# bdwsq1996/Effi-MVS-plus

Measured on AMD Instinct MI355X. Metric: ref-views/sec (cost-volume hot path: warp + cost volume + 3-D regularisation + cascaded GRU refinement), higher is better.
Workload: dtype f32 (3x3 MFMA convs: products as 3 bf16 partial products hi*hi+hi*lo+lo*hi, f32 accumulate; all else f32); 1 GPU; cfg3: DTU-shaped 1600x1184, N=5 views (S=4 sources), 3-stage cascade ndepths=48,8,8, GRU iters 3,3,3, seeded-random weights, features of the stock FPN resident in HBM; parallelism=single GPU, views_in_flight=3, arithmetic=split

## Files before the change

### effi_mvs_plus_amd/_lib.py

```python
from __future__ import annotations

import ctypes as C
import os
import threading

_HERE = os.path.dirname(os.path.abspath(__file__))
LIB_PATH = os.environ.get("EFFI_MVS_LIB") or os.path.join(_HERE, "libeffimvs_hip.so")
HEADER_PATH = os.path.join(os.path.dirname(_HERE), "include", "effi_mvs_hip.h")

_vp, _i, _l, _f = C.c_void_p, C.c_int, C.c_long, C.c_float

SIGNATURES = {
    "effi_version": [],
    "effi_set_workspace": [_i, _vp, _l],
    "effi_set_option": [C.c_char_p, _l],
    "effi_fusion_dynamic_filter_f32": [_vp, _vp, _vp, _vp, _i, _i, _i, _vp, _i, _i, _f, _i, _f, _f, _i, _vp, _vp, _vp, _vp, _vp, _vp,
                                       _vp, _vp],
    "effi_fusion_dtu_filter_f32": [_vp, _vp, _vp, _vp, _i, _i, _i, _vp, _f, _f, _i, _i, _f, _f, _vp, _vp, _vp, _vp, _vp, _vp, _vp],
    "effi_fusion_vis_filter_f32": [_vp, _vp, _i, _i, _i, _i, _f, _f, _i, _i, _vp, _vp],
    "effi_fusion_points_f32": [_i, _vp, _l, _vp, _vp, _i, _i, _i, _vp, _vp, _vp],
    "effi_fusion_dtu_reproject_f32": [_vp, _vp, _vp, _vp, _i, _i, _i, _i, _f, _f, _vp, _vp, _vp, _vp],
    "effi_compose_rel_proj_f32": [_vp, _i, _vp, _vp],
    "effi_rel_proj_f32": [_vp, _vp, _vp, _vp],
    "effi_planar_to_nhwc_f32": [_vp, _vp, _i, _i, _i, _vp],
    "effi_homo_warp_f32": [_vp, _vp, _vp, _l, _l, _i, _i, _i, _i, _vp, _vp],
    "effi_warpcorr_views_f32": [_vp, _vp, _i, _vp, _vp, _l, _l, _i, _i, _i, _i, _vp, _vp, _vp],
    "effi_warpcorr_views_tbl_f32": [_vp, _i, _vp, _vp, _l, _l, _i, _i, _i, _i, _vp, _vp, _vp],
    "effi_warpcorr_views_x3_f32": [_vp, _vp, _i, _vp, _vp, _l, _l, _i, _i, _i, _i, _vp, _vp, _i, _vp],
    "effi_warpcorr_views_x3_tbl_f32": [_vp, _i, _vp, _vp, _l, _l, _i, _i, _i, _i, _vp, _vp, _i, _vp],
    "effi_warpcorr_dyn_tbl_f32": [_vp, _i, _vp, _vp, _vp, _vp, _i, _i, _i, _i, _i, _vp, _vp, _vp],
    "effi_view_table_set": [_vp, _vp, _i, _vp],
    "effi_pixelwise_net_f32": [_vp, _vp, _i, _i, _i, _vp, _vp],
    "effi_view_aggregate_f32": [_vp, _vp, _i, _i, _i, _vp, _vp],
    "effi_warpcorr_dyn_f32": [_vp, _vp, _i, _vp, _vp, _vp, _vp, _i, _i, _i, _i, _i, _vp, _vp, _vp],
    "effi_conv3d_k3_f32": [_vp, _vp, _i, _vp, _vp, _i, _i, _i, _i, _i, _i, _i, _vp, _vp, _vp],
    "effi_deconv3d_k3s2_bf16x3_f32": [_vp, _i, _vp, _vp, _i, _i, _i, _i, _i, _vp, _vp, _vp],
    "effi_conv3d_k3s2_mfma_f32": [_vp, _i, _vp, _vp, _i, _i, _i, _i, _i, _vp, _vp],
    "effi_conv3d_k3s1_mfma_f32": [_vp, _i, _vp, _vp, _i, _i, _i, _i, _i, _vp, _vp],
    "effi_deconv3d_k3_f32": [_vp, _i, _vp, _vp, _i, _i, _i, _i, _i, _i, _vp, _vp, _vp],
    "effi_softmax_regress_conf_f32": [_vp, _vp, _l, _l, _i, _i, _vp, _vp, _vp, _i, _vp, _vp],
    "effi_vol_lookup1d_f32": [_vp, _l, _l, _i, _vp, _l, _l, _l, _i, _vp, _vp, _l, _i, _i, _vp, _vp],
    "effi_bilinear_sampler1d_f32": [_vp, _i, _i, _i, _vp, _l, _vp, _vp, _vp],
    "effi_getcost_conv1x1_f32": [_vp, _vp, _i, _i, _vp, _vp, _l, _l, _i, _vp, _l, _l, _i, _vp, _vp, _l, _i, _i, _i, _vp, _vp, _i,
                                 _i, _vp, _vp],
    "effi_getcost_f32": [_vp, _vp, _i, _i, _vp, _vp, _l, _l, _i, _vp, _l, _l, _i, _vp, _vp, _l, _i, _i, _i, _vp, _vp],
    "effi_conv2d_f32": [_vp, _vp, _i, _vp, _vp, _i, _i, _i, _i, _i, _i, _vp, _vp, _vp, _i, _vp, _vp, _vp],
    "effi_conv3d_k3s1_roll_bf16x3_f32": [_vp, _vp, _i, _vp, _vp, _i, _i, _i, _i, _i, _vp, _vp],
    "effi_conv3d_k3s1_bf16x3_f32": [_vp, _vp, _i, _vp, _vp, _i, _i, _i, _i, _i, _vp, _vp],
    "effi_vol_lookup1d_pair_f32": [_vp, _vp, _l, _l, _i, _vp, _l, _l, _l, _i, _vp, _vp, _l, _i, _i, _vp, _vp, _vp],
    "effi_conv3d_k3_pair_f32": [_vp, _vp, _vp, _vp, _vp, _vp, _vp, _vp, _i, _i, _i, _i, _i, _i, _i, _vp],
    "effi_conv3d_k3s1_roll_bf16x3_pair_f32": [_vp, _vp, _vp, _vp, _vp, _vp, _vp, _vp, _vp, _i, _i, _i, _i, _i, _i, _vp],
    "effi_csp_gen_roll_bf16x3_pair_f32": [_vp, _i, _i, _i] + [_vp] * 16 + [_vp],
    "effi_debug_poison_lds": [C.c_uint, _vp, _vp],
    "effi_debug_pk_war_probe": [_vp, _i, _i, _i, _vp],
    "effi_deconv3d_k3_pair_f32": [_vp, _vp, _vp, _vp, _vp, _vp, _vp, _vp, _i, _i, _i, _i, _i, _i, _i, _vp],
    "effi_homo_warp_bwd_f32": [_vp, _vp, _l, _l, _i, _i, _i, _i, _vp, _vp, _vp],
    "effi_warpcorr_views_bwd_f32": [_vp, _vp, _i, _vp, _vp, _l, _l, _i, _i, _i, _i, _vp, _vp, _vp, _vp],
    "effi_image_prepare_u8_f32": [_vp, _i, _i, _i, _i, _i, _vp, _vp],
    "effi_resize_linear_f32": [_vp, _i, _i, _i, _i, _i, _vp, _vp],
    "effi_encoder_inputs_f32": [_vp, _vp, _i, _vp, _vp, _l, _l, _i, _vp, _l, _l, _i, _vp, _vp, _l, _i, _i, _i, _vp, _vp, _vp, _vp,
                                _i, _vp, _vp, _vp],
    "effi_encoder_inputs_bf16x3_f32": [_vp, _vp, _i, _vp, _vp, _l, _l, _i, _vp, _l, _l, _i, _vp, _vp, _l, _i, _i, _i, _vp, _vp, _vp, _vp,
                                       _i, _vp, _vp, _vp],
    "effi_conv2d_k3_bf16x3_pair_f32": [_vp, _vp, _i, _vp, _vp, _vp, _vp, _vp, _i, _vp, _vp, _vp, _i, _i, _i, _i, _vp],
    "effi_conv2d_k3_k1_up2x_bf16x3_f32": [_vp, _vp, _i, _vp, _vp, _i, _vp, _vp, _vp, _vp, _i, _i, _i, _vp, _vp, _vp],
    "effi_conv2d_k3_k1_bf16x3_f32": [_vp, _vp, _i, _vp, _vp, _i, _i, _vp, _i, _vp, _vp, _i, _i, _i, _i, _vp, _vp],
    "effi_conv2d_k3_bf16x3_f32": [_vp, _vp, _i, _vp, _vp, _i, _i, _i, _i, _i, _vp, _vp, _vp, _i, _vp, _vp, _vp],
    "effi_conv2d_k5s2_f32": [_vp, _i, _vp, _vp, _i, _i, _i, _i, _vp, _vp],
    "effi_conv2d_k5s2_bf16x3_f32": [_vp, _i, _vp, _vp, _i, _i, _i, _i, _vp, _vp],
    "effi_conv3d_k3s2_bf16x3_f32": [_vp, _i, _vp, _vp, _i, _i, _i, _i, _i, _vp, _vp],
    "effi_conv2d_c1k7_relu_f32": [_vp, _vp, _vp, _i, _i, _i, _vp, _vp],
    "effi_conv2d_c1k7_relu_bf16x3_f32": [_vp, _vp, _vp, _i, _i, _i, _vp, _vp],
    "effi_convex_upsample2x_f32": [_vp, _vp, _vp, _i, _i, _i, _vp, _vp, _vp, _vp],
    "effi_compose_rel_proj_stages_f32": [_vp, _i, _i, _vp, _vp],
    "effi_split_tanh_relu_stages_f32": [_vp, _vp, _vp, _vp, _vp, _vp, _i, _vp],
    "effi_split_tanh_relu_f32": [_vp, _i, _i, _i, _vp, _vp, _vp],
    "effi_depth_to_inv_f32": [_vp, _vp, _i, _i, _vp, _vp],
    "effi_stage1_hypotheses_f32": [_vp, _i, _i, _vp, _vp, _vp],
    "effi_upsample_nearest_f32": [_vp, _i, _i, _i, _i, _vp, _vp],
    "effi_head_update_f32": [_vp, _vp, _vp, _vp, _i, _i, _i, _vp, _vp, _vp],
    "effi_conv2d_k3_twice_bf16x3_f32": [_vp, _i, _vp, _vp, _vp, _vp, _i, _i, _i, _vp, _vp],
    "effi_encoder_tail_bf16x3_f32": [_vp, _vp, _i, _vp, _vp, _vp, _vp, _vp, _vp, _i, _vp, _i, _vp, _vp, _i, _i, _i, _vp, _vp],
    "effi_sr_geometry": [_i, _i, _vp, _vp],
    "effi_sr_clear_border": [_vp, _vp, _vp, _vp, _vp, _vp, _i, _vp],
    "effi_sr_from_planar_f32": [_vp, _i, _i, _i, _vp, _i, _i, _vp],
    "effi_split_tanh_relu_stages_sr_f32": [_vp, _vp, _vp, _vp, _vp, _vp, _vp, _vp, _vp, _vp, _vp, _i, _vp],
    "effi_encoder_inputs_bf16x3_sr": [_vp, _vp, _i, _vp, _vp, _l, _l, _i, _vp, _l, _l, _i, _vp, _vp, _l, _i, _i, _i, _vp, _vp, _vp, _vp,
                                      _i, _vp, _vp, _i, _i, _vp],
    "effi_encoder_pair_gen_bf16x3_sr": [_vp, _vp, _i, _vp, _vp, _l, _l, _i, _vp, _l, _l, _i, _vp, _vp, _l, _i, _i, _i, _vp, _vp, _vp, _vp,
                                        _i, _vp, _vp, _vp, _vp, _vp, _vp, _i, _i, _i, _i, _vp],
    "effi_gru_zr_q_fused_bf16x3_sr": [_vp, _vp, _vp, _vp, _vp, _vp, _vp, _i, _i, _i, _i, _i, _vp, _vp, _vp],
    "effi_conv2d_k3_bf16x3_sr": [_vp, _vp, _i, _vp, _vp, _i, _i, _i, _i, _i, _i, _i, _vp, _vp, _vp, _vp, _vp],
    "effi_conv2d_k3_bf16x3_pair_sr": [_vp, _vp, _i, _vp, _vp, _vp, _vp, _vp, _i, _vp, _vp, _vp, _i, _i, _i, _i, _i, _i, _vp],
    "effi_conv2d_k3_k1_bf16x3_sr": [_vp, _vp, _i, _vp, _vp, _i, _i, _vp, _i, _vp, _vp, _i, _i, _i, _i, _i, _i, _vp, _vp, _vp],
    "effi_conv2d_k3_k1_up2x_bf16x3_sr": [_vp, _vp, _i, _vp, _vp, _i, _vp, _vp, _vp, _vp, _i, _i, _i, _i, _i, _vp, _vp, _vp],
    "effi_conv_wgrad_f32": [_vp, _vp, _i, _i, _i, _i, _i, _i, _i, _i, _i, _i, _i, _i, _i, _i, _vp, _vp],
    "effi_channel_sum_f32": [_vp, _i, _i, _l, _vp, _vp, _i, _vp],
    "effi_conv2d_k5s2_dgrad_f32": [_vp, _vp, _i, _i, _i, _i, _vp, _vp],
    "effi_bn_moment_f32": [_vp, _i, _i, _l, _vp, _i, _vp, _vp, _i, _vp],
    "effi_bn_train_fwd_f32": [_vp, _i, _i, _l, _vp, _vp, _f, _f, _vp, _vp, _vp, _i, _vp, _vp, _vp, _vp, _i, _vp],
    "effi_pack_conv2d_mfma_f32": [_vp, _vp, _i, _i, _i, _i, _vp, _vp, _vp],
    "effi_pack_conv2d_k5s2_dgrad_f32": [_vp, _i, _i, _i, _i, _vp, _vp, _vp],
    "effi_bn_apply_f32": [_vp, _i, _i, _l, _vp, _vp, _vp, _vp, _i, _vp, _vp],
    "effi_bn_bwd_f32": [_vp, _vp, _vp, _i, _i, _l, _vp, _vp, _vp, _i, _vp, _vp, _vp, _vp, _i, _vp],
    "effi_pointwise_f32": [_i, _vp, _vp, _vp, _vp, _f, _f, _l, _l, _i, _vp, _vp, _vp, _vp],
    "effi_vol_lookup1d_bwd_f32": [_vp, _l, _l, _i, _vp, _l, _l, _l, _i, _vp, _vp, _l, _i, _i, _vp, _vp],
    "effi_getcost_bwd_f32": [_vp, _vp, _i, _i, _vp, _vp, _l, _l, _i, _vp, _l, _l, _i, _vp, _vp, _l, _i, _i, _i, _vp, _vp],
    "effi_softargmin_bwd_f32": [_vp, _vp, _l, _l, _i, _i, _vp, _vp, _vp],
    "effi_view_aggregate_bwd_f32": [_vp, _vp, _i, _i, _i, _vp, _vp, _vp, _vp],
    "effi_convex_upsample2x_bwd_f32": [_vp, _vp, _i, _i, _vp, _vp, _vp, _vp, _vp],
    "effi_warpcorr_dyn_bwd_f32": [_vp, _vp, _i, _vp, _vp, _vp, _vp, _i, _i, _i, _i, _i, _vp, _vp, _vp, _vp, _vp, _vp],
}

BF16X3_ENTRIES = ("effi_conv2d_k3_bf16x3_pair_f32", "effi_conv2d_k3_bf16x3_f32", "effi_conv2d_k3_k1_bf16x3_f32",
                  "effi_conv2d_k3_k1_up2x_bf16x3_f32", "effi_conv3d_k3s1_bf16x3_f32", "effi_conv3d_k3s1_roll_bf16x3_f32",
                  "effi_conv3d_k3s1_roll_bf16x3_pair_f32", "effi_csp_gen_roll_bf16x3_pair_f32", "effi_deconv3d_k3s2_bf16x3_f32", "effi_encoder_tail_bf16x3_f32", "effi_conv2d_k3_twice_bf16x3_f32",
                  "effi_conv2d_k5s2_bf16x3_f32", "effi_conv3d_k3s2_bf16x3_f32",
                  "effi_conv2d_k3_bf16x3_sr", "effi_conv2d_k3_bf16x3_pair_sr", "effi_conv2d_k3_k1_bf16x3_sr", "effi_conv2d_k3_k1_up2x_bf16x3_sr",
                  "effi_encoder_pair_gen_bf16x3_sr", "effi_gru_zr_q_fused_bf16x3_sr")
for _n in BF16X3_ENTRIES:
    SIGNATURES[_n + "_bf16"] = SIGNATURES[_n]

NON_STATUS_SYMBOLS = ("effi_error_string", "effi_workspace_bytes", "effi_get_workspace", "effi_get_option", "effi_option_unset")

_lock = threading.Lock()
_lib = None


class EffiLibraryError(RuntimeError):
    pass


def lib():
    global _lib
    if _lib is not None:
        return _lib
    with _lock:
        if _lib is not None:
            return _lib
        if not os.path.exists(LIB_PATH):
            raise EffiLibraryError(
                f"{LIB_PATH} not found: build the gfx950 kernels first "
                "(python -c 'import __graft_entry__ as g; g.build()' or make -C effi_mvs_plus_amd/csrc). "
                "There is no CPU / eager fallback for the cost-volume path.")
        handle = C.CDLL(LIB_PATH)
        for name, argtypes in SIGNATURES.items():
            fn = getattr(handle, name)
            fn.argtypes = argtypes
            fn.restype = _i
        handle.effi_error_string.argtypes = [_i]
        handle.effi_error_string.restype = C.c_char_p
        handle.effi_workspace_bytes.argtypes = []
# ... 24 lines not shown
```

### effi_mvs_plus_amd/csrc/common.hpp

```cpp
#pragma once
#include <hip/hip_runtime.h>
#include "../../include/effi_mvs_hip.h"

#define EFFI_LAUNCH_CHECK()                                   \
    do {                                                      \
        if (hipPeekAtLastError() != hipSuccess) return EFFI_ERR_LAUNCH; \
    } while (0)

const float* effi_zero_page();

enum EffiOption {
    EFFI_OPT_WARP_LDS_KB,
    EFFI_OPT_DYN_FORM,
    EFFI_OPT_DYN_SETUP_EXACT,
    EFFI_OPT_DYN_XCHG,
    EFFI_OPT_PIXNET_MFMA,
    EFFI_OPT_FORCE_MR,
    EFFI_OPT_MR4_MIN, EFFI_OPT_MR4_NT2_MAX, EFFI_OPT_MR2_MIN,
    EFFI_OPT_WIDE_TILES,
    EFFI_OPT_ROLL_MR, EFFI_OPT_ROLL_ZT, EFFI_OPT_ROLL_RP,
    EFFI_OPT_DECONV_MR,
    EFFI_OPT_SR_WAVES,
    EFFI_OPT_ENC_GEN_MR3,
    EFFI_OPT_C3_LEAN,
// ... 64 lines not shown
__device__ __forceinline__ float effi_sigmoid_split(float x) {
#ifdef EFFI_EXACT_EPILOGUES
    return effi_sigmoid(x);
#else
    const float r = effi_rcp_refined(1.0f + effi_exp_fast(fminf(-x, 60.0f)));
    return (x != x) ? x : r;
#endif
}
__device__ __forceinline__ float effi_tanh_split(float x) {
#ifdef EFFI_EXACT_EPILOGUES
    return tanhf(x);
#else
    const float r = 1.0f - 2.0f * effi_rcp_refined(1.0f + effi_exp_fast(fminf(2.0f * x, 60.0f)));
    return (x != x) ? x : r;
#endif
}

__device__ __forceinline__ float effi_inv_to_depth(float inv, float lo, float hi) {
    const float max_depth = 1.0f / lo, min_depth = 1.0f / hi;
    const float min_disp = 1.0f / max_depth, max_disp = 1.0f / min_depth;
    float s = min_disp + (max_disp - min_disp) * inv;
    s = fmaxf(s, 1e-4f);
    return 1.0f / s;
}

__device__ __forceinline__ float effi_depth_to_inv(float depth, float lo, float hi) {
    const float max_depth = 1.0f / lo, min_depth = 1.0f / hi;
    const float min_disp = 1.0f / max_depth, max_disp = 1.0f / min_depth;
    const float den = (max_disp - min_disp) + 1e-10f;
    const float s_ = 1.0f / depth;
    return (s_ - min_disp) / den;
}

__device__ __forceinline__ float effi_lk_rcp(float b) {
#ifdef EFFI_EXACT_LOOKUP
    return 1.0f / b;
#else
    const float r0 = __builtin_amdgcn_rcpf(b);
    return fmaf(fmaf(-b, r0, 1.0f), r0, r0);
#endif
}
__device__ __forceinline__ float effi_lk_div(float a, float b, float rb) {
#ifdef EFFI_EXACT_LOOKUP
    (void)rb;
    return a / b;
#else
    const float q = a * rb;
    return fmaf(fmaf(-q, b, a), rb, q);
#endif
}

__device__ __forceinline__ void lookup1d_index(int Dp, float q_depth, float dmin, float dmax, int& x0, float& w0, float& w1) {
    const float scaled = effi_lk_rcp(q_depth);
    const float min_disp = effi_lk_rcp(dmax), max_disp = effi_lk_rcp(dmin);
    const float den = (max_disp - min_disp) + 1e-10f;
    const float disp = effi_lk_div(scaled - min_disp, den, effi_lk_rcp(den));
    const float dm1 = (float)(Dp - 1);
    const float t = disp * dm1;
    const float g = effi_lk_div(2.0f * t, dm1, effi_lk_rcp(dm1)) - 1.0f;
    float ix = ((g + 1.0f) * 0.5f) * dm1;
    ix = fminf(fmaxf(ix, -2.0f), dm1 + 2.0f);
    const float x0f = floorf(ix);
    x0 = (int)x0f;
    w1 = ix - x0f;
    w0 = (x0f + 1.0f) - ix;
}
// ... 212 lines not shown
```

### effi_mvs_plus_amd/csrc/conv2d_sr.hip

```cpp
#include "conv2d_x3.hpp"

namespace {

int fill_sr(Conv2dArgs& a, const void* const* srcs, const int* src_channels, int n_src, const void* wpack_bf16, const float* bias,
            int cout, int h, int w, int hp, int wp) {
    if (!srcs || !src_channels || n_src < 1 || n_src > EFFI_MAX_SRC || !wpack_bf16 || !bias) return EFFI_ERR_BADARG;
    if (cout < 1 || h < 1 || w < 1) return EFFI_ERR_BADARG;
    const bool wide_possible = w >= 512 || effi_option(EFFI_OPT_WIDE_TILES) == 1;
    if (hp < ((h + 15) & ~15) + 2 || wp < (wide_possible ? ((w + 63) & ~63) : ((w + 15) & ~15)) + 2) return EFFI_ERR_BADARG;
    if ((long)hp * wp * 4 >= (1L << 31)) return EFFI_ERR_UNSUPPORTED;
    a.cin = 0;
    for (int i = 0; i < EFFI_MAX_SRC; ++i) {
        a.src[i] = reinterpret_cast<const float*>((i < n_src) ? srcs[i] : srcs[0]);
        a.ch[i] = (i < n_src) ? src_channels[i] : 0;
        if (i < n_src && (!srcs[i] || src_channels[i] < 1)) return EFFI_ERR_BADARG;
        if (i < n_src && (src_channels[i] & 15)) return EFFI_ERR_UNSUPPORTED;
        if (i < n_src && (reinterpret_cast<uintptr_t>(srcs[i]) & 15)) return EFFI_ERR_BADARG;
        a.cin += a.ch[i];
    }
    if ((long)cout * hp * wp >= (1L << 31)) return EFFI_ERR_UNSUPPORTED;
    a.kgroups = (a.cin + 3) / 4;
    a.zeros = nullptr;
    a.wpack = reinterpret_cast<const float*>(wpack_bf16);
    a.bias = bias;
// ... 118 lines not shown
}

extern "C" int EFFI_FN(effi_conv2d_k3_k1_bf16x3_sr)(const void* const* srcs, const int* src_channels, int n_src, const void* wpack_bf16,
                                                    const float* bias, int cout1, int relu1, const float* extra, int c_extra,
                                                    const void* w2pack_bf16, const float* bias2, int cout2, int relu, int h, int w,
                                                    int hp, int wp, float* out, void* out_sr, effi_stream_t stream) {
    if (!w2pack_bf16 || !bias2 || (!out && !out_sr) || (out && out_sr)) return EFFI_ERR_BADARG;
    if (cout1 < 1 || cout2 < 1 || c_extra < 0 || (c_extra > 0 && !extra)) return EFFI_ERR_BADARG;
    if (cout1 > 96 || c_extra > 16 || cout2 > 96) return EFFI_ERR_UNSUPPORTED;
    if (out_sr && ((cout2 & 15) || (reinterpret_cast<uintptr_t>(out_sr) & 15))) return EFFI_ERR_BADARG;
    Conv2dArgs a;
    const int rc = fill_sr(a, srcs, src_channels, n_src, wpack_bf16, bias, cout1, h, w, hp, wp);
    if (rc != EFFI_OK) return rc;
    a.kgroups = relu1 ? 1 : 0;
    a.act = relu ? EFFI_ACT_RELU : EFFI_ACT_NONE;
    a.hd = c_extra;
    a.aux0 = c_extra ? extra : bias2;
    a.aux1 = reinterpret_cast<const float*>(w2pack_bf16);
    a.disp_range = bias2;
    a.n_range = cout2;
    a.out0 = out;
    a.out_sr = reinterpret_cast<unsigned short*>(out_sr);
    hipStream_t st = effi_s(stream);
    switch ((cout1 + 15) / 16) {
        case 1: return launch_bf16x3<1, EFFI_EPI_K1, false, true>(a, st);
        case 2: return launch_bf16x3<2, EFFI_EPI_K1, false, true>(a, st);
        case 3: return launch_bf16x3<3, EFFI_EPI_K1, false, true>(a, st);
        case 4: return launch_bf16x3<4, EFFI_EPI_K1, false, true>(a, st);
        case 6: return launch_bf16x3<6, EFFI_EPI_K1, false, true>(a, st);
        default: return EFFI_ERR_UNSUPPORTED;
    }
}

extern "C" int EFFI_FN(effi_conv2d_k3_k1_up2x_bf16x3_sr)(const void* const* srcs, const int* src_channels, int n_src,
                                                         const void* wpack_bf16, const float* bias, int cout1, const void* w2pack_bf16,
                                                         const float* bias2, const float* inv_depth, const float* disp_range,
                                                         int n_range, int h, int w, int hp, int wp, float* out_depth,
                                                         float* out_depth_inv, effi_stream_t stream) {
    if (!w2pack_bf16 || !bias2 || !inv_depth || !disp_range || n_range < 2 || !out_depth) return EFFI_ERR_BADARG;
    if (cout1 < 1 || cout1 > 96) return EFFI_ERR_UNSUPPORTED;
    Conv2dArgs a;
    const int rc = fill_sr(a, srcs, src_channels, n_src, wpack_bf16, bias, cout1, h, w, hp, wp);
    if (rc != EFFI_OK) return rc;
    a.kgroups = 1;
    a.hd = 0;
    a.aux0 = inv_depth;
    a.aux1 = reinterpret_cast<const float*>(w2pack_bf16);
    a.disp_range = bias2;
    a.n_range = 36;
    a.out0 = out_depth;
    a.out1 = out_depth_inv;
    a.zin = n_range;
    a.xptr0 = disp_range;
    hipStream_t st = effi_s(stream);
    switch ((cout1 + 15) / 16) {
        case 2: return launch_bf16x3<2, EFFI_EPI_K1UP, false, true>(a, st);
        case 4: return launch_bf16x3<4, EFFI_EPI_K1UP, false, true>(a, st);
        case 6: return launch_bf16x3<6, EFFI_EPI_K1UP, false, true>(a, st);
        default: return EFFI_ERR_UNSUPPORTED;
    }
}

#include "gru_fused.hpp"
```

### effi_mvs_plus_amd/csrc/conv2d_x3.hpp

```cpp
#pragma once
#include "common.hpp"

#ifdef EFFI_BF16_ONLY
#define EFFI_FN(name) name##_bf16
#else
#define EFFI_FN(name) name
#endif

#ifndef EFFI_ABL
#define EFFI_ABL 0
#endif
#ifndef EFFI_PIPE_FRAGS
#define EFFI_PIPE_FRAGS 0
#endif

#ifndef EFFI_EPI_BATCH
#define EFFI_EPI_BATCH 1
#endif
#ifndef EFFI_EPI_EARLY_MAX
#define EFFI_EPI_EARLY_MAX 16
#endif
#ifndef EFFI_B_EARLY
#define EFFI_B_EARLY 0
#endif
// ... 139 lines not shown
        for (int r = 0; r < 4; ++r) dst[(long)r * hw] = effi_sigmoid_split(v[r]) * (is_z ? 1.0f : hv[r]);
    } else if (EPI == EFFI_EPI_GRU_Q) {
        if (nvalid <= 0) return;
        if (SR && a.aux_q4) {
            const long oq = ((long)(co0 >> 2) * hw + pix) * 4;
            const f32x4 h4 = *reinterpret_cast<const f32x4*>(a.aux0 + oq), z4 = *reinterpret_cast<const f32x4*>(a.aux1 + oq);
            f32x4 g;
#pragma unroll
            for (int r = 0; r < 4; ++r) g[r] = (1.0f - z4[r]) * h4[r] + z4[r] * effi_tanh_split(v[r]);
            *reinterpret_cast<f32x4*>(a.out0 + oq) = g;
            effi_sr_store4(a.out_sr, a.sr_hp, a.sr_wp, co0, y, x, g);
            return;
        }
        const long o = (long)co0 * hw + pix;
        float hv[4], zv[4];
#pragma unroll
        for (int r = 0; r < 4; ++r) {
            hv[r] = a.aux0[o + (long)r * hw];
            zv[r] = a.aux1[o + (long)r * hw];
        }
        f32x4 g;
#pragma unroll
        for (int r = 0; r < 4; ++r) g[r] = (1.0f - zv[r]) * hv[r] + zv[r] * effi_tanh_split(v[r]);
#pragma unroll
        for (int r = 0; r < 4; ++r) a.out0[o + (long)r * hw] = g[r];
        if (SR) effi_sr_store4(a.out_sr, a.sr_hp, a.sr_wp, co0, y, x, g);
    }
}

typedef __bf16 bf16x8 __attribute__((ext_vector_type(8)));

#define EFFI_EPI_K1 6
#define EFFI_EPI_K1UP 8
typedef __bf16 bf16x2 __attribute__((ext_vector_type(2)));
typedef float f32x2 __attribute__((ext_vector_type(2)));

__device__ __forceinline__ void split_octet(const f32x4 (&pa)[8], int px, bf16x8& hi, bf16x8& lo) {
#pragma unroll
    for (int e = 0; e < 8; e += 2) {
        const f32x2 x = {pa[e][px], pa[e + 1][px]};
        const bf16x2 h2 = __builtin_convertvector(x, bf16x2);
        const f32x2 hf = __builtin_convertvector(h2, f32x2);
        const bf16x2 l2 = __builtin_convertvector(x - hf, bf16x2);
        hi[e] = h2[0];
        hi[e + 1] = h2[1];
        lo[e] = l2[0];
        lo[e + 1] = l2[1];
    }
}

template <int NT, int MR, int EPI, bool ZB, bool WIDE, bool SR = false, int NW = 4, bool GEN = false>
__device__ __forceinline__ void conv2d_k3_bf16x3_tile(const Conv2dArgs a, int tiles_x, int ntiles, int bid, int nbid, int bidy,
                                                      const EncGenArgs* gp = nullptr, int gmode = 0) {
    constexpr int NTHR = NW * 64;
    static_assert(!GEN || SR, "generated inputs use the split-resident LDS image");
    static_assert(NW == 4 || (SR && NW == 8), "eight waves: split-resident kernels only");
    constexpr int TR = WIDE ? NW : NW * MR, TW = WIDE ? 16 * MR : 16;
    constexpr int AR = TR + 2, AW = SR ? TW + 2 : TW + 8, AQ = AW / 4, XOFF = SR ? 0 : 3, XLEFT = 4, CCH = 16, NKS = 5;
    constexpr int MROW = WIDE ? 0 : AW * 8, MCOL = WIDE ? 16 * 8 : 0;
    constexpr int APIX = AR * AW, NITEMS = (APIX / 4) * 2;
    constexpr int APIXP = SR ? ((APIX + 15) & ~15) : APIX;
    constexpr int NPART = kHiOnly ? 1 : 2;
    constexpr int NUA = SR ? (NPART * 2 * APIXP + NTHR - 1) / NTHR : 1;
    constexpr int NBF = NKS * NT * 2 * 64;
    constexpr int NB4 = (NBF + NTHR - 1) / NTHR;
    static_assert(SR || NITEMS <= 256, "one staging item per thread");
    static_assert(!(SR && ZB), "split-resident maps are 2-D");
    static_assert(EPI != EFFI_EPI_HEAD && EPI != EFFI_EPI_ADD_UP2, "epilogue not instantiated for the split-precision kernel");
    static_assert((EPI != EFFI_EPI_K1 && EPI != EFFI_EPI_K1UP) || !ZB, "the fused 1x1 epilogue is 2-D only");
    __shared__ __attribute__((aligned(16))) unsigned short lds_ah[SR ? NUA * NTHR * 8 : APIX * CCH];
    __shared__ __attribute__((aligned(16))) unsigned short lds_al[SR ? 8 : APIX * CCH];
    __shared__ __attribute__((aligned(16))) unsigned short lds_b[NB4 * NTHR * 8];
    const unsigned short* const lds_al_rd = SR ? lds_ah + 2 * APIXP * 8 : lds_al;
    constexpr int IW7 = (AW + 7 + 1) & ~1, IH7 = AR + 7;
    __shared__ float lds_inv[GEN ? IH7 * IW7 : 1];

    const int tid = threadIdx.x, lane = tid & 63, wv = tid >> 6;
    const int li = lane & 15, lk = lane >> 4;
    const int h = a.h, w = a.w;
    const long hw = (long)h * w;
    const int tile = effi_xcd_remap(bid, nbid);
    if (tile >= ntiles) return;
    const int ty_ = tile / tiles_x;
    const int x0 = (tile - ty_ * tiles_x) * TW, y0 = ty_ * TR;
    const int zpl = ZB ? bidy : 0;

    const bool stager = tid < NITEMS;
    const int pq = stager ? tid % (APIX / 4) : 0, soct = stager ? tid / (APIX / 4) : 0;
    const int srow = pq / AQ, sqx = pq - srow * AQ;
    const int sgy = y0 - 1 + srow, sgx = x0 - XLEFT + 4 * sqx;
    const bool s_in = stager & (sgy >= 0) & (sgy < h) & (sgx >= 0) & (sgx < w);
    const int s_off = sgy * w + sgx;
    const int s_lds = (soct * APIX + srow * AW + 4 * sqx) * 8;
    const int s_nv = w - sgx;
    const bool s_part = s_nv < 4;

    f32x4 pa[SR ? NUA : 8];
    const int cin_eff = ZB ? 3 * a.cin : a.cin;
    const int nchunks = (cin_eff + CCH - 1) / CCH;
    const unsigned short* wbf = reinterpret_cast<const unsigned short*>(a.wpack);
    int goff[NUA];
    if (SR && !GEN) {
#pragma unroll
        for (int j = 0; j < NUA; ++j) {
            const int u = tid + j * NTHR;
            const int part = u / (2 * APIXP), r_ = u - part * (2 * APIXP);
            const int oct = r_ / APIXP, p = r_ - oct * APIXP;
            const int row = p / AW, col = p - row * AW;
            const bool valid = (part < NPART) & (p < APIX);
            goff[j] = valid ? ((oct * 2 + part) * a.sr_hp + (y0 + row)) * a.sr_wp + (x0 + col) : 0;
        }
    }
    auto prefetch = [&](int ch) {
        if constexpr (GEN) {
            (void)ch;
        } else if constexpr (SR) {
            const int cb = ch * CCH;
            const int c1 = cb - a.ch[0], c2 = c1 - a.ch[1];
            const float* src = (c1 < 0) ? a.src[0] : (c2 < 0 ? a.src[1] : a.src[2]);
            const int cl = (c1 < 0) ? cb : (c2 < 0 ? c1 : c2);
            const f32x4* base = reinterpret_cast<const f32x4*>(src) + (long)(cl >> 2) * ((long)a.sr_hp * a.sr_wp);
#pragma unroll
            for (int j = 0; j < NUA; ++j) pa[j] = (EFFI_ABL & 1) ? f32x4{0.0f, 0.0f, 0.0f, 0.0f} : base[goff[j]];
        } else {
        int cb = ch * CCH + soct * 8;
        const int emax = min(cin_eff - cb, 8) - 1;
        bool in = s_in & (emax >= 0);
        long zoff = 0;
        if (ZB) {
            const int dz = (cb >= a.cin) + (cb >= 2 * a.cin);
            cb -= dz * a.cin;
            const int zz = zpl + dz - 1;
            in &= (zz >= 0) & (zz < a.zcount);
            zoff = (long)zz * hw;
        }
        const int c1 = cb - a.ch[0], c2 = c1 - a.ch[1];
        const float* src = (c1 < 0) ? a.src[0] : (c2 < 0 ? a.src[1] : a.src[2]);
        const int cl = (c1 < 0) ? cb : (c2 < 0 ? c1 : c2);
        const float* base = in ? src + ((long)cl * a.cstride + zoff + s_off) : a.zeros;
        const long step = in ? a.cstride : 0;
        const float* q = base;
        if (ZB && in && s_part) {
// ... 167 lines not shown

    constexpr bool kBatchT = SR && EFFI_EPI_BATCH != 0 && !(EFFI_ABL & 24) &&
                             (EPI == EFFI_EPI_PLAIN || EPI == EFFI_EPI_GRU_ZR || EPI == EFFI_EPI_GRU_Q);
    constexpr int NZ = (EPI == EFFI_EPI_GRU_ZR) ? NT / 2 : 0;
    constexpr int NH = !kBatchT ? 0 : (EPI == EFFI_EPI_GRU_ZR ? NT - NZ : (EPI == EFFI_EPI_GRU_Q ? NT : 0));
    constexpr int NZQ = (kBatchT && EPI == EFFI_EPI_GRU_Q) ? NT : 0;
    constexpr bool kStateEarly = MR * (NH + NZQ) * 4 <= EFFI_EPI_EARLY_MAX;
    const bool ebatch = kBatchT && (EPI == EFFI_EPI_PLAIN || a.aux_q4);
    f32x4 eb[kBatchT ? NT : 1], eh[MR][NH > 0 ? NH : 1], ez[MR][NZQ > 0 ? NZQ : 1];
    unsigned eqb[MR];
    bool einside[MR];
    auto epi_issue_bias = [&]() {
        if (!ebatch) return;
#pragma unroll
        for (int n = 0; n < NT; ++n) eb[n] = *reinterpret_cast<const f32x4*>(a.bias + n * 16 + 4 * lk);
#pragma unroll
        for (int m = 0; m < MR; ++m) {
            const int x = x0 + li + (WIDE ? 16 * m : 0), y = y0 + (WIDE ? wv : wv * MR + m);
            einside[m] = (y < h) & (x < w);
            eqb[m] = ((unsigned)lk * (unsigned)hw + (einside[m] ? (unsigned)(y * w + x) : 0u)) * 4u;
        }
    };
    auto epi_issue_state = [&]() {
        if (!ebatch) return;
#pragma unroll
        for (int m = 0; m < MR; ++m) {
#pragma unroll
            for (int j = 0; j < NH; ++j) eh[m][j] = *reinterpret_cast<const f32x4*>(a.aux0 + (size_t)(eqb[m] + (unsigned)j * 16u * (unsigned)hw));
#pragma unroll
            for (int j = 0; j < NZQ; ++j) ez[m][j] = *reinterpret_cast<const f32x4*>(a.aux1 + (size_t)(eqb[m] + (unsigned)j * 16u * (unsigned)hw));
        }
    };

    constexpr bool kK1 = (EPI == EFFI_EPI_K1 || EPI == EFFI_EPI_K1UP) && !(EFFI_ABL & 24) && EFFI_EPI_BATCH != 0;
    f32x4 kb[kK1 ? NT : 1], kex[kK1 ? MR : 1];
    if constexpr (kK1) {
#pragma unroll
        for (int n = 0; n < NT; ++n) kb[n] = *reinterpret_cast<const f32x4*>(a.bias + n * 16 + 4 * lk);
#pragma unroll
        for (int m = 0; m < MR; ++m) kex[m] = f32x4{0.0f, 0.0f, 0.0f, 0.0f};
        if (EPI == EFFI_EPI_K1 && a.hd > 0) {
#pragma unroll
            for (int m = 0; m < MR; ++m) {
                const int x = x0 + li + (WIDE ? 16 * m : 0), y = y0 + (WIDE ? wv : wv * MR + m);
                const unsigned pix = ((y < h) & (x < w)) ? (unsigned)(y * w + x) : 0u;
#pragma unroll
                for (int r = 0; r < 4; ++r) {
                    const int c = 4 * lk + r;
                    const float t_ = a.aux0[(size_t)((unsigned)min(c, a.hd - 1) * (unsigned)hw + pix)];
                    kex[m][r] = (c < a.hd) ? t_ : 0.0f;
                }
            }
        }
    }

    constexpr bool kBiasQ = !kBatchT && !kK1 && !(EFFI_ABL & 24) && EFFI_EPI_BATCH != 0;
    f32x4 gb[kBiasQ ? NT : 1];
    if constexpr (kBiasQ) {
#pragma unroll
        for (int n = 0; n < NT; ++n) gb[n] = *reinterpret_cast<const f32x4*>(a.bias + n * 16 + 4 * lk);
    }

    prefetch(0);
    epi_issue_bias();
    if (kStateEarly) epi_issue_state();
    stash(0);
    __syncthreads();
// ... 58 lines not shown
                    }
                }
                if (PIPE) {
                    __builtin_amdgcn_sched_barrier(0);
                    if (s_ + 1 < NKS) load_b(s_ + 1, n);
                }
            }
        }
        if (ch + 1 < nchunks) {
            __syncthreads();
            stash(ch + 1);
            __syncthreads();
        }
    }

    if (EFFI_ABL & 24) {
#pragma unroll
        for (int m = 0; m < MR; ++m) {
            const int x = x0 + li + (WIDE ? 16 * m : 0), y = y0 + (WIDE ? wv : wv * MR + m);
            if (y >= h || x >= w) continue;
#pragma unroll
            for (int n = 0; n < NT; ++n)
#pragma unroll
                for (int r = 0; r < 4; ++r) {
                    if (EFFI_ABL & 16) {
                        if (acc[m][n][r] == 1.2345e38f) a.out0[0] = 1.0f;
                    } else if (n * 16 + 4 * lk + r < min(a.cout, a.hd > 0 ? a.hd : a.cout)) {
                        a.out0[(long)(n * 16 + 4 * lk + r) * hw + (long)y * w + x] = acc[m][n][r];
                    }
                }
        }
        return;
    }
    if (EPI == EFFI_EPI_K1 || EPI == EFFI_EPI_K1UP) {
        const unsigned short* w2 = reinterpret_cast<const unsigned short*>(a.aux1);
        const int nt2 = (a.n_range + 15) >> 4;
        const bool relu1 = a.kgroups != 0;
        bf16x4 xh[MR][NT + 1], xl[MR][NT + 1];
        bool inside[MR];
        long pixm[MR];
        f32x4 ex[MR];
#pragma unroll
        for (int m = 0; m < MR; ++m) {
            const int x = x0 + li + (WIDE ? 16 * m : 0);
            const int y = y0 + (WIDE ? wv : wv * MR + m);
            inside[m] = (y < h) & (x < w);
            pixm[m] = inside[m] ? (long)y * w + x : 0;
            if constexpr (kK1) {
                ex[m] = kex[m];
            } else {
#pragma unroll
                for (int r = 0; r < 4; ++r) {
                    const int c = 4 * lk + r;
                    ex[m][r] = (c < a.hd) ? a.aux0[(long)c * hw + pixm[m]] : 0.0f;
                }
            }
        }
#pragma unroll
        for (int m = 0; m < MR; ++m) {
#pragma unroll
            for (int n = 0; n <= NT; ++n) {
                f32x4 vf;
#pragma unroll
                for (int r = 0; r < 4; ++r)
                    vf[r] = (n < NT) ? acc[m][n][r] + (kK1 ? kb[n < NT ? n : 0][r] : a.bias[n * 16 + 4 * lk + r]) : (inside[m] ? ex[m][r] : 0.0f);
                if (relu1 && n < NT) {
#pragma unroll
                    for (int r = 0; r < 4; ++r) vf[r] = fmaxf(vf[r], 0.0f);
                }
                xh[m][n] = __builtin_convertvector(vf, bf16x4);
                xl[m][n] = __builtin_convertvector(vf - __builtin_convertvector(xh[m][n], f32x4), bf16x4);
            }
        }
        if constexpr (EPI == EFFI_EPI_K1UP) {
            f32x4 om[MR][3];
#pragma unroll
            for (int t = 0; t < 3; ++t) {
                bf16x4 wh[NT + 1], wl[NT + 1];
#pragma unroll
// ... 32 lines not shown
                    const int yy = y + k / 3 - 1, xx = x + k % 3 - 1;
                    const bool ok = (yy >= 0) & (yy < h) & (xx >= 0) & (xx < w);
                    nbv[k] = ok ? a.aux0[ok ? (long)yy * w + xx : 0] : 0.0f;
                }
                float mx = v[0];
#pragma unroll
                for (int k = 1; k < 9; ++k) mx = fmaxf(mx, v[k]);
                float e[9], sm = 0.0f;
#pragma unroll
                for (int k = 0; k < 9; ++k) {
#ifdef EFFI_EXACT_EPILOGUES
                    e[k] = expf(v[k] - mx);
#else
                    e[k] = effi_exp_fast(v[k] - mx);
#endif
                    sm = sm + e[k];
                }
                float ac = 0.0f;
#ifdef EFFI_EXACT_EPILOGUES
#pragma unroll
                for (int k = 0; k < 9; ++k) ac = ac + (e[k] / sm) * nbv[k];
#else
                const float rsm = effi_rcp_refined(sm);
#pragma unroll
                for (int k = 0; k < 9; ++k) ac = ac + (e[k] * rsm) * nbv[k];
#endif
                const long o = (long)(2 * y + (lk >> 1)) * W2 + 2 * x + (lk & 1);
                const float dep = effi_inv_to_depth(ac, lo, hi);
                a.out0[o] = dep;
                if (a.out1) a.out1[o] = effi_depth_to_inv(dep, lo, hi);
            }
            return;
        }
        for (int t = 0; t < nt2; ++t) {
            bf16x4 wh[NT + 1], wl[NT + 1];
#pragma unroll
            for (int n = 0; n <= NT; ++n) {
                const long f = ((long)(t * (NT + 1) + n) * 2) * 64 + lane;
                wh[n] = *reinterpret_cast<const bf16x4*>(w2 + f * 4);
                wl[n] = *reinterpret_cast<const bf16x4*>(w2 + (f + 64) * 4);
            }
            const int co = t * 16 + 4 * lk;
            float b2[4];
#pragma unroll
            for (int r = 0; r < 4; ++r) b2[r] = a.disp_range[co + r];
#pragma unroll
            for (int m = 0; m < MR; ++m) {
                f32x4 o = {0.0f, 0.0f, 0.0f, 0.0f};
#pragma unroll
                for (int n = 0; n <= NT; ++n) {
                    o = __builtin_amdgcn_mfma_f32_16x16x16bf16_1k(wh[n], xh[m][n], o, 0, 0, 0);
                    if (!kHiOnly) {
                        o = __builtin_amdgcn_mfma_f32_16x16x16bf16_1k(wl[n], xh[m][n], o, 0, 0, 0);
                        o = __builtin_amdgcn_mfma_f32_16x16x16bf16_1k(wh[n], xl[m][n], o, 0, 0, 0);
                    }
                }
                if (inside[m]) {
                    f32x4 vo;
#pragma unroll
                    for (int r = 0; r < 4; ++r) {
                        float v = o[r] + b2[r];
                        if (a.act == EFFI_ACT_RELU) v = fmaxf(v, 0.0f);
                        vo[r] = v;
                    }
                    if (SR && a.out_sr) {
                        effi_sr_store4(a.out_sr, a.sr_hp, a.sr_wp, co, y0 + (WIDE ? wv : wv * MR + m), x0 + li + (WIDE ? 16 * m : 0), vo);
                    } else {
#pragma unroll
                        for (int r = 0; r < 4; ++r)
                            if (co + r < a.n_range) a.out0[(long)(co + r) * hw + pixm[m]] = vo[r];
                    }
                }
            }
        }
        return;
    }
    if constexpr (kBatchT) if (ebatch) {
        if (!kStateEarly) epi_issue_state();
        const unsigned plane = (unsigned)a.sr_hp * (unsigned)a.sr_wp;
#pragma unroll
        for (int m = 0; m < MR; ++m) {
            if (!einside[m]) continue;
            const int x = x0 + li + (WIDE ? 16 * m : 0), y = y0 + (WIDE ? wv : wv * MR + m);
            const unsigned ub = (unsigned)lk * plane + (unsigned)(y + 1) * (unsigned)a.sr_wp + (unsigned)(x + 1);
#pragma unroll
            for (int n = 0; n < NT; ++n) {
                f32x4 v;
#pragma unroll
                for (int r = 0; r < 4; ++r) v[r] = acc[m][n][r] + eb[n][r];
// ... 11 lines not shown
#pragma unroll
                        for (int r = 0; r < 4; ++r) dst[(long)r * a.ostride] = v[r];
                    }
                } else if constexpr (EPI == EFFI_EPI_GRU_ZR) {
                    f32x4 g;
                    if (n < NZ) {
#pragma unroll
                        for (int r = 0; r < 4; ++r) g[r] = effi_sigmoid_split(v[r]) * 1.0f;
                        *reinterpret_cast<f32x4*>(a.out0 + (size_t)(eqb[m] + (unsigned)n * 16u * (unsigned)hw)) = g;
                    } else {
#pragma unroll
                        for (int r = 0; r < 4; ++r) g[r] = effi_sigmoid_split(v[r]) * eh[m][n >= NZ ? n - NZ : 0][r];
                        effi_sr_store4_at(a.out_sr, ub + (unsigned)(4 * (n - NZ)) * plane, lk & 1, g);
                    }
                } else {
                    f32x4 g;
#pragma unroll
                    for (int r = 0; r < 4; ++r) g[r] = (1.0f - ez[m][n][r]) * eh[m][n][r] + ez[m][n][r] * effi_tanh_split(v[r]);
                    *reinterpret_cast<f32x4*>(a.out0 + (size_t)(eqb[m] + (unsigned)n * 16u * (unsigned)hw)) = g;
                    effi_sr_store4_at(a.out_sr, ub + (unsigned)(4 * n) * plane, lk & 1, g);
                }
            }
        }
        return;
    }
#pragma unroll
    for (int m = 0; m < MR; ++m) {
        const int x = x0 + li + (WIDE ? 16 * m : 0);
        const int y = y0 + (WIDE ? wv : wv * MR + m);
        if (y >= h || x >= w) continue;
        const long pix = (long)y * w + x;
#pragma unroll
        for (int n = 0; n < NT; ++n)
            conv_epilogue_store_t<((EPI == EFFI_EPI_K1 || EPI == EFFI_EPI_K1UP) ? EFFI_EPI_PLAIN : EPI), SR>(a, acc[m][n], n * 16 + 4 * lk, pix, hw, zpl, y, x,
                                                                                                          kBiasQ ? &gb[n] : nullptr);
    }
}

template <int NT, int MR, int EPI, bool ZB = false, bool WIDE = false, bool SR = false, int NW = 4>
__global__ __launch_bounds__(NW * 64) void conv2d_k3_bf16x3_kernel(const Conv2dArgs a, int tiles_x, int ntiles) {
#ifdef EFFI_STAGGER
    if (SR && gridDim.x > 512) {
        const int slot = (blockIdx.x >> 8) % 3;
        for (int i = 0; i < slot * EFFI_STAGGER; ++i) __builtin_amdgcn_s_sleep(127);
    }
#endif
    conv2d_k3_bf16x3_tile<NT, MR, EPI, ZB, WIDE, SR, NW>(a, tiles_x, ntiles, blockIdx.x, gridDim.x, blockIdx.y);
}

template <int NT, int MR, bool WIDE, bool SR = false, int NW = 4>
__global__ __launch_bounds__(NW * 64) void conv2d_k3_bf16x3_pair_kernel(const Conv2dArgs a0, const Conv2dArgs a1, int tiles_x, int ntiles) {
    if (blockIdx.y == 0) conv2d_k3_bf16x3_tile<NT, MR, EFFI_EPI_PLAIN, false, WIDE, SR, NW>(a0, tiles_x, ntiles, blockIdx.x, gridDim.x, 0);
    else conv2d_k3_bf16x3_tile<NT, MR, EFFI_EPI_PLAIN, false, WIDE, SR, NW>(a1, tiles_x, ntiles, blockIdx.x, gridDim.x, 0);
}

template <int NT, int MR, bool WIDE>
__global__ __launch_bounds__(256) void conv2d_k3_bf16x3_encgen_pair_kernel(const Conv2dArgs a0, const Conv2dArgs a1, const EncGenArgs g,
                                                                           int tiles_x, int ntiles) {
    conv2d_k3_bf16x3_tile<NT, MR, EFFI_EPI_PLAIN, false, WIDE, true, 4, true>(blockIdx.y == 0 ? a0 : a1, tiles_x, ntiles, blockIdx.x, gridDim.x, 0, &g,
                                                                             (int)blockIdx.y);
}

static long effi_opt_or(int id, long dflt) {
    const long v = effi_option(id);
    return v == EFFI_OPT_UNSET ? dflt : v;
}
static long effi_mr4_min() { return effi_opt_or(EFFI_OPT_MR4_MIN, 400); }
// ... 8 lines not shown
    if (t4 >= effi_mr4_min() && !(NT == 2 && t4 >= effi_mr4_nt2_max())) mr = 4;
    else if (t2 >= effi_mr2_min()) mr = 2;
    else mr = 1;
    const long force = effi_opt_or(EFFI_OPT_FORCE_MR, 0);
    if (force) mr = (int)force;
    const long wide_env = effi_opt_or(EFFI_OPT_WIDE_TILES, -1);
    const bool wide = wide_env >= 0 ? wide_env != 0 : (mr == 4 && a.w >= 512 && !ZB);
    if (wide) {
        const int tiles_x = effi_cdiv(a.w, 16 * mr), ntiles = tiles_x * effi_cdiv(a.h, 4);
        const dim3 grid(ntiles, (unsigned)planes);
        if (mr == 4) hipLaunchKernelGGL((conv2d_k3_bf16x3_kernel<NT, 4, EPI, ZB, true, SR>), grid, dim3(256), 0, st, a, tiles_x, ntiles);
        else if (mr == 2) hipLaunchKernelGGL((conv2d_k3_bf16x3_kernel<NT, 2, EPI, ZB, true, SR>), grid, dim3(256), 0, st, a, tiles_x, ntiles);
        else hipLaunchKernelGGL((conv2d_k3_bf16x3_kernel<NT, 1, EPI, ZB, true, SR>), grid, dim3(256), 0, st, a, tiles_x, ntiles);
        return hipPeekAtLastError() == hipSuccess ? EFFI_OK : EFFI_ERR_LAUNCH;
    }
    if constexpr (SR) {
        const long srw = effi_option(EFFI_OPT_SR_WAVES);
        if ((srw == 8 && mr <= 2) || (srw == EFFI_OPT_UNSET && mr == 1 && NT >= 6)) {
            const int tiles_x = (int)cols, ntiles = tiles_x * effi_cdiv(a.h, 8 * mr);
            const dim3 grid(ntiles, 1);
            if (mr == 2) hipLaunchKernelGGL((conv2d_k3_bf16x3_kernel<NT, 2, EPI, false, false, true, 8>), grid, dim3(512), 0, st, a, tiles_x, ntiles);
            else hipLaunchKernelGGL((conv2d_k3_bf16x3_kernel<NT, 1, EPI, false, false, true, 8>), grid, dim3(512), 0, st, a, tiles_x, ntiles);
            return hipPeekAtLastError() == hipSuccess ? EFFI_OK : EFFI_ERR_LAUNCH;
        }
    }
    const int tiles_x = (int)cols, ntiles = tiles_x * effi_cdiv(a.h, 4 * mr);
    const dim3 grid(ntiles, (unsigned)planes);
    if (mr == 4) hipLaunchKernelGGL((conv2d_k3_bf16x3_kernel<NT, 4, EPI, ZB, false, SR>), grid, dim3(256), 0, st, a, tiles_x, ntiles);
    else if (mr == 2) hipLaunchKernelGGL((conv2d_k3_bf16x3_kernel<NT, 2, EPI, ZB, false, SR>), grid, dim3(256), 0, st, a, tiles_x, ntiles);
    else hipLaunchKernelGGL((conv2d_k3_bf16x3_kernel<NT, 1, EPI, ZB, false, SR>), grid, dim3(256), 0, st, a, tiles_x, ntiles);
    return hipPeekAtLastError() == hipSuccess ? EFFI_OK : EFFI_ERR_LAUNCH;
}

template <int EPI, bool SR = false>
static int dispatch_bf16x3(const Conv2dArgs& a, int nt, hipStream_t st) {
    switch (nt) {
        case 1: return launch_bf16x3<1, EPI, false, SR>(a, st);
        case 2: return launch_bf16x3<2, EPI, false, SR>(a, st);
        case 3: return launch_bf16x3<3, EPI, false, SR>(a, st);
        case 4: return launch_bf16x3<4, EPI, false, SR>(a, st);
        case 6: return launch_bf16x3<6, EPI, false, SR>(a, st);
        default: return EFFI_ERR_UNSUPPORTED;
    }
}

template <int NT, bool SR = false>
static int launch_bf16x3_pair(const Conv2dArgs& a0, const Conv2dArgs& a1, hipStream_t st) {
    const long cols = effi_cdiv(a0.w, 16);
    const long t4 = cols * effi_cdiv(a0.h, 16) * 2, t2 = cols * effi_cdiv(a0.h, 8) * 2;
    int mr;
    if (t4 >= effi_mr4_min() && !(NT == 2 && t4 >= effi_mr4_nt2_max())) mr = 4;
    else if (t2 >= effi_mr2_min()) mr = 2;
    else mr = 1;
    const long force = effi_opt_or(EFFI_OPT_FORCE_MR, 0);
    if (force) mr = (int)force;
    if (mr == 4 && a0.w >= 512) {
        const int tiles_x = effi_cdiv(a0.w, 64), ntiles = tiles_x * effi_cdiv(a0.h, 4);
        hipLaunchKernelGGL((conv2d_k3_bf16x3_pair_kernel<NT, 4, true, SR>), dim3(ntiles, 2), dim3(256), 0, st, a0, a1, tiles_x, ntiles);
        return hipPeekAtLastError() == hipSuccess ? EFFI_OK : EFFI_ERR_LAUNCH;
    }
    if constexpr (SR) {
        if (effi_option(EFFI_OPT_SR_WAVES) == 8 && mr <= 2) {
            const int tiles_x = (int)cols, ntiles = tiles_x * effi_cdiv(a0.h, 8 * mr);
            const dim3 grid(ntiles, 2);
            if (mr == 2) hipLaunchKernelGGL((conv2d_k3_bf16x3_pair_kernel<NT, 2, false, true, 8>), grid, dim3(512), 0, st, a0, a1, tiles_x, ntiles);
            else hipLaunchKernelGGL((conv2d_k3_bf16x3_pair_kernel<NT, 1, false, true, 8>), grid, dim3(512), 0, st, a0, a1, tiles_x, ntiles);
// ... 33 lines not shown
```

### effi_mvs_plus_amd/csrc/proj.hip

```cpp
#include "common.hpp"

namespace {

__device__ void compose_k_rt(const float* pair, double P[4][4]) {
    const float* E = pair;
    const float* K = pair + 16;
    for (int r = 0; r < 3; ++r)
        for (int c = 0; c < 4; ++c) {
            double s = 0.0;
            for (int k = 0; k < 3; ++k) s += (double)K[r * 4 + k] * (double)E[k * 4 + c];
            P[r][c] = s;
        }
    for (int c = 0; c < 4; ++c) P[3][c] = (double)E[12 + c];
}

__device__ void load4x4(const float* m, double P[4][4]) {
    for (int r = 0; r < 4; ++r)
        for (int c = 0; c < 4; ++c) P[r][c] = (double)m[r * 4 + c];
}

__device__ void invert4x4(const double A[4][4], double inv[4][4]) {
    double M[4][8];
    for (int r = 0; r < 4; ++r)
        for (int c = 0; c < 4; ++c) {
// ... 15 lines not shown
            if (r == col) continue;
            const double f = M[r][col];
            for (int c = 0; c < 8; ++c) M[r][c] -= f * M[col][c];
        }
    }
    for (int r = 0; r < 4; ++r)
        for (int c = 0; c < 4; ++c) inv[r][c] = M[r][c + 4];
}

__device__ void write_rt(const double S[4][4], const double Rinv[4][4], float* rt) {
    double M[3][4];
    for (int r = 0; r < 3; ++r)
        for (int c = 0; c < 4; ++c) {
            double s = 0.0;
            for (int k = 0; k < 4; ++k) s += S[r][k] * Rinv[k][c];
            M[r][c] = s;
        }
    for (int r = 0; r < 3; ++r)
        for (int c = 0; c < 3; ++c) rt[r * 3 + c] = (float)M[r][c];
    for (int r = 0; r < 3; ++r) rt[9 + r] = (float)M[r][3];
}

__global__ void compose_rel_proj_kernel(const float* __restrict__ pairs, int n_views, float* __restrict__ rt) {
    const int v = blockIdx.x * blockDim.x + threadIdx.x;
    if (v >= n_views - 1) return;
    double R[4][4], Rinv[4][4], S[4][4];
    compose_k_rt(pairs, R);
    invert4x4(R, Rinv);
    compose_k_rt(pairs + (long)(v + 1) * 32, S);
    write_rt(S, Rinv, rt + v * 12);
}

struct PairList { const float* p[4]; };
__global__ void compose_rel_proj_stages_kernel(PairList pl, int n_views, float* __restrict__ rt_all) {
    const int v = threadIdx.x;
    if (v >= n_views - 1) return;
    const float* pairs = pl.p[0];
#pragma unroll
    for (int j = 1; j < 4; ++j)
        if ((int)blockIdx.x == j) pairs = pl.p[j];
    double R[4][4], Rinv[4][4], S[4][4];
    compose_k_rt(pairs, R);
    invert4x4(R, Rinv);
    compose_k_rt(pairs + (long)(v + 1) * 32, S);
    write_rt(S, Rinv, rt_all + ((long)blockIdx.x * (n_views - 1) + v) * 12);
}

__global__ void rel_proj_kernel(const float* __restrict__ src, const float* __restrict__ ref, float* __restrict__ rt) {
    if (threadIdx.x != 0 || blockIdx.x != 0) return;
    double R[4][4], Rinv[4][4], S[4][4];
    load4x4(ref, R);
    invert4x4(R, Rinv);
    load4x4(src, S);
    write_rt(S, Rinv, rt);
}

}

extern "C" int effi_compose_rel_proj_f32(const float* pairs, int n_views, float* rt_out, effi_stream_t stream) {
    if (!pairs || !rt_out || n_views < 2 || n_views > EFFI_MAX_VIEWS + 1) return EFFI_ERR_BADARG;
    hipLaunchKernelGGL(compose_rel_proj_kernel, dim3(1), dim3(64), 0, effi_s(stream), pairs, n_views, rt_out);
    EFFI_LAUNCH_CHECK();
    return EFFI_OK;
}

extern "C" int effi_compose_rel_proj_stages_f32(const float* const* pairs, int n_stages, int n_views, float* rt_out,
                                                effi_stream_t stream) {
    if (!pairs || !rt_out || n_stages < 1 || n_stages > 4 || n_views < 2 || n_views > EFFI_MAX_VIEWS + 1) return EFFI_ERR_BADARG;
    PairList pl;
    for (int k = 0; k < 4; ++k) {
        pl.p[k] = pairs[k < n_stages ? k : 0];
        if (!pl.p[k]) return EFFI_ERR_BADARG;
    }
    hipLaunchKernelGGL(compose_rel_proj_stages_kernel, dim3(n_stages), dim3(64), 0, effi_s(stream), pl, n_views, rt_out);
    EFFI_LAUNCH_CHECK();
    return EFFI_OK;
}

extern "C" int effi_rel_proj_f32(const float* src_proj, const float* ref_proj, float* rt_out, effi_stream_t stream) {
    if (!src_proj || !ref_proj || !rt_out) return EFFI_ERR_BADARG;
    hipLaunchKernelGGL(rel_proj_kernel, dim3(1), dim3(64), 0, effi_s(stream), src_proj, ref_proj, rt_out);
    EFFI_LAUNCH_CHECK();
    return EFFI_OK;
}
```

### effi_mvs_plus_amd/csrc/volume_ops.hip

```cpp
#include <cstdint>
#include "common.hpp"

namespace {

constexpr int TPB = 256;

__global__ __launch_bounds__(TPB) void planar_to_nhwc_kernel(EffiPtrList srcs, EffiOutList dsts, int C, int HW) {
    extern __shared__ __attribute__((aligned(16))) float tile[];
    const float* __restrict__ src = srcs.p[blockIdx.y];
    float* __restrict__ dst = dsts.p[blockIdx.y];
    const long p0 = (long)blockIdx.x * 64;
    const int n = C * 64;
    for (int e = threadIdx.x; e < n; e += TPB) {
        const int c = e >> 6, p = e & 63;
        const long gp = p0 + p;
        tile[c * 65 + p] = (gp < HW) ? src[(long)c * HW + gp] : 0.0f;
    }
    __syncthreads();
    for (int e = threadIdx.x; e < n; e += TPB) {
        const int p = e / C, c = e - p * C;
        const long gp = p0 + p;
        if (gp < HW) dst[gp * C + c] = tile[c * 65 + p];
    }
}
// ... 38 lines not shown
    for (int j = 1; j < 4; ++j)
        if (k == j) { ctx = a.ctx[j]; hidden = a.hidden[j]; inp = a.inp[j]; nh = a.nh[j]; n = a.n[j]; b0 = a.first[j]; }
    const long i = 4 * ((long)(blockIdx.x - b0) * TPB + threadIdx.x);
    if (a.vec4) {
        if (i >= n) return;
        const float4 v = *reinterpret_cast<const float4*>(ctx + i);
        if (i < nh) *reinterpret_cast<float4*>(hidden + i) = make_float4(tanhf(v.x), tanhf(v.y), tanhf(v.z), tanhf(v.w));
        else *reinterpret_cast<float4*>(inp + (i - nh)) = make_float4(fmaxf(v.x, 0.0f), fmaxf(v.y, 0.0f), fmaxf(v.z, 0.0f), fmaxf(v.w, 0.0f));
        return;
    }
#pragma unroll
    for (int e = 0; e < 4; ++e) {
        if (i + e >= n) break;
        const float v = ctx[i + e];
        if (i + e < nh) hidden[i + e] = tanhf(v);
        else inp[i + e - nh] = fmaxf(v, 0.0f);
    }
}

__global__ void depth_to_inv_kernel(const float* __restrict__ depth, const float* __restrict__ disp_range,
                                    int n_range, int n, float* __restrict__ inv) {
    const float lo = disp_range[0], hi = disp_range[n_range - 1];
    const float max_depth = 1.0f / lo, min_depth = 1.0f / hi;
    const float min_disp = 1.0f / max_depth, max_disp = 1.0f / min_depth;
    const float den = (max_disp - min_disp) + 1e-10f;
    for (int i = blockIdx.x * TPB + threadIdx.x; i < n; i += gridDim.x * TPB) {
        const float s = 1.0f / depth[i];
        inv[i] = (s - min_disp) / den;
    }
}

__global__ void stage1_hypotheses_kernel(const float* __restrict__ disp_range, int n_range, int D,
                                         float* __restrict__ depths, float* __restrict__ intervals) {
    const float lo = disp_range[0], hi = disp_range[n_range - 1];
    const float step = (hi - lo) / (float)(D - 1);
    for (int d = threadIdx.x; d < D; d += blockDim.x) {
        const float s = lo + (float)d * step;
        depths[d] = 1.0f / s;
    }
    if (threadIdx.x < 3) {
        const float base = (hi - lo) / (float)n_range;
        const float ratio = (threadIdx.x == 0) ? 4.0f : (threadIdx.x == 1 ? 2.0f : 1.0f);
        intervals[threadIdx.x] = base * ratio;
    } else if (threadIdx.x == 3) {
        intervals[3] = 1.0f / hi;
    } else if (threadIdx.x == 4) {
        intervals[4] = 1.0f / lo;
    }
}

__global__ void upsample_nearest_kernel(const float* __restrict__ in, int C, int h, int w, int f,
                                        float* __restrict__ out) {
    const int W = w * f, H = h * f;
    const long n = (long)C * H * W;
    for (long i = (long)blockIdx.x * TPB + threadIdx.x; i < n; i += (long)gridDim.x * TPB) {
        const int x = (int)(i % W);
        const long t = i / W;
        const int y = (int)(t % H);
        const int c = (int)(t / H);
        out[i] = in[((long)c * h + y / f) * w + x / f];
    }
}

__global__ __launch_bounds__(TPB) void head_update_kernel(const float* __restrict__ s9, const float* __restrict__ bias2,
                                                          const float* __restrict__ inv, const float* __restrict__ disp_range,
                                                          int n_range, int h, int w, float* __restrict__ out_inv,
                                                          float* __restrict__ out_depth) {
    const int wq = w >> 2;
    const long q = (long)blockIdx.x * TPB + threadIdx.x;
    if (q >= (long)h * wq) return;
    const int y = (int)(q / wq), x = (int)(q - (long)y * wq) * 4;
    const long hw = (long)h * w;
    float acc[4] = {0.0f, 0.0f, 0.0f, 0.0f};
#pragma unroll
    for (int ky = 0; ky < 3; ++ky) {
        const int yy = y + ky - 1;
        if (yy < 0 || yy >= h) continue;
        const float* row = s9 + (long)yy * w + x;
#pragma unroll
        for (int kx = 0; kx < 3; ++kx) {
            const float* pl = row + (long)(ky * 3 + kx) * hw;
// ... 20 lines not shown
    *reinterpret_cast<float4*>(out_depth + pix) = d;
}

__global__ void view_aggregate_kernel(const float* __restrict__ sim_views, const float* __restrict__ weights,
                                      int S, int D, int hw, float* __restrict__ out) {
    const int p = blockIdx.x * TPB + threadIdx.x;
    if (p >= hw) return;
    const int d0 = blockIdx.y * 8;
    if (!weights) {
        for (int d = d0; d < min(D, d0 + 8); ++d) {
            float acc = 0.0f;
            for (int v = 0; v < S; ++v) acc = acc + sim_views[((long)v * D + d) * hw + p];
            out[(long)d * hw + p] = acc / (float)S;
        }
        return;
    }
    float wv[EFFI_MAX_VIEWS];
    float wsum = 0.0f;
#pragma unroll
    for (int v = 0; v < EFFI_MAX_VIEWS; ++v) {
        wv[v] = (v < S) ? weights[(long)v * hw + p] : 0.0f;
        if (v < S) wsum = wsum + wv[v];
    }
    const float den = wsum + 1e-6f;
    for (int d = d0; d < min(D, d0 + 8); ++d) {
        float acc = 0.0f;
#pragma unroll
        for (int v = 0; v < EFFI_MAX_VIEWS; ++v)
            if (v < S) acc = acc + sim_views[((long)v * D + d) * hw + p] * wv[v];
        out[(long)d * hw + p] = acc / den;
    }
}

__global__ void softmax_regress_conf_kernel(const float* __restrict__ logits, const float* __restrict__ depth,
                                            long dds, long dps, int D, int hw,
                                            float* __restrict__ out_depth, float* __restrict__ out_conf,
                                            const float* __restrict__ disp_range, int n_range, float* __restrict__ out_dinv) {
    const int p = blockIdx.x * blockDim.x + threadIdx.x;
    if (p >= hw) return;
    float m = -INFINITY;
    for (int d = 0; d < D; ++d) m = fmaxf(m, logits[(long)d * hw + p]);
    float sum = 0.0f;
    for (int d = 0; d < D; ++d) sum = sum + expf(logits[(long)d * hw + p] - m);
    float dep = 0.0f, idxf = 0.0f;
    for (int d = 0; d < D; ++d) {
        const float pr = expf(logits[(long)d * hw + p] - m) / sum;
        dep = dep + pr * depth[d * dds + p * dps];
        idxf = idxf + pr * (float)d;
    }
    int idx = (int)idxf;
    idx = max(0, min(D - 1, idx));
    float s4 = 0.0f;
    for (int k = idx - 1; k <= idx + 2; ++k) {
        const float pr = (k >= 0 && k < D) ? expf(logits[(long)k * hw + p] - m) / sum : 0.0f;
        s4 = s4 + pr;
    }
    out_depth[p] = dep;
    out_conf[p] = 4.0f * (s4 / 4.0f);
    if (out_dinv) out_dinv[p] = effi_depth_to_inv(dep, disp_range[0], disp_range[n_range - 1]);
}

template <int DT>
__global__ __launch_bounds__(64) void softmax_regress_conf_reg_kernel(const float* __restrict__ logits, const float* __restrict__ depth,
                                                                      long dds, long dps, int hw, float* __restrict__ out_depth,
                                                                      float* __restrict__ out_conf, const float* __restrict__ disp_range,
                                                                      int n_range, float* __restrict__ out_dinv) {
    const int p = blockIdx.x * 64 + threadIdx.x;
    if (p >= hw) return;
    float e[DT], dv[DT];
#pragma unroll
    for (int d = 0; d < DT; ++d) e[d] = logits[(long)d * hw + p];
#pragma unroll
    for (int d = 0; d < DT; ++d) dv[d] = depth[d * dds + p * dps];
    float m = -INFINITY;
#pragma unroll
    for (int d = 0; d < DT; ++d) m = fmaxf(m, e[d]);
    float sum = 0.0f;
#pragma unroll
    for (int d = 0; d < DT; ++d) {
        e[d] = expf(e[d] - m);
        sum = sum + e[d];
    }
    float dep = 0.0f, idxf = 0.0f;
#pragma unroll
    for (int d = 0; d < DT; ++d) {
        e[d] = e[d] / sum;
        dep = dep + e[d] * dv[d];
        idxf = idxf + e[d] * (float)d;
    }
    int idx = (int)idxf;
    idx = max(0, min(DT - 1, idx));
    float s4 = 0.0f;
#pragma unroll
    for (int d = 0; d < DT; ++d) {
        const bool in = (d >= idx - 1) & (d <= idx + 2);
        s4 = in ? s4 + e[d] : s4;
    }
    out_depth[p] = dep;
    out_conf[p] = 4.0f * (s4 / 4.0f);
    if (out_dinv) out_dinv[p] = effi_depth_to_inv(dep, disp_range[0], disp_range[n_range - 1]);
}

__device__ __forceinline__ float lookup1d(const float* __restrict__ vol, long dstride, int Dp,
                                          float q_depth, float dmin, float dmax) {
    int x0;
    float w0, w1;
    lookup1d_index(Dp, q_depth, dmin, dmax, x0, w0, w1);
    return lookup1d_fetch(vol, dstride, Dp, x0, w0, w1);
}

__global__ void bilinear_sampler1d_kernel(const float* __restrict__ img, int C, int W, const float* __restrict__ coords, long nq,
                                          long total, float* __restrict__ out, float* __restrict__ mask) {
    const long i = (long)blockIdx.x * TPB + threadIdx.x;
    if (i >= total) return;
    const long n = i / nq, q = i - n * nq;
    const float xp = coords[2 * i], yp = coords[2 * i + 1];
    const float wm1 = (float)(W - 1);
    const float g = 2.0f * xp / wm1 - 1.0f;
    float ix = ((g + 1.0f) / 2.0f) * wm1;
    ix = fminf(fmaxf(ix, -2.0f), wm1 + 2.0f);
    const float x0f = floorf(ix);
    const int x0 = (int)x0f;
    const float w1 = ix - x0f, w0 = (x0f + 1.0f) - ix;
    const float* row = img + n * (long)C * W;
    for (int c = 0; c < C; ++c) out[(n * C + c) * nq + q] = lookup1d_fetch(row + (long)c * W, 1, W, x0, w0, w1);
    if (mask) mask[i] = ((g > -1.0f) & (yp > -1.0f) & (g < 1.0f) & (yp < 1.0f)) ? 1.0f : 0.0f;
}

__global__ void vol_lookup1d_kernel(const float* __restrict__ vol, long vds, long vps, int Dp,
                                    const float* __restrict__ query, long qds, long qys, long qxs, int nq,
                                    const float* __restrict__ dmin, const float* __restrict__ dmax, long rps,
                                    int h, int w, float* __restrict__ out, const float* __restrict__ vol_b,
                                    float* __restrict__ out_b) {
// ... 222 lines not shown
}

extern "C" int effi_upsample_nearest_f32(const float* in, int C, int h, int w, int f, float* out,
                                         effi_stream_t stream) {
    if (!in || !out || C < 1 || h < 1 || w < 1 || f < 1) return EFFI_ERR_BADARG;
    const long n = (long)C * h * f * w * f;
    hipLaunchKernelGGL(upsample_nearest_kernel, dim3(min(effi_cdiv(n, TPB), 8192)), dim3(TPB), 0, effi_s(stream),
                       in, C, h, w, f, out);
    EFFI_LAUNCH_CHECK();
    return EFFI_OK;
}

extern "C" int effi_head_update_f32(const float* partial9, const float* bias2, const float* inv_depth, const float* disp_range,
                                    int n_range, int h, int w, float* out_inv, float* out_depth, effi_stream_t stream) {
    if (!partial9 || !bias2 || !inv_depth || !disp_range || n_range < 2 || !out_inv || !out_depth || h < 1 || w < 1)
        return EFFI_ERR_BADARG;
    if (w & 3) return EFFI_ERR_UNSUPPORTED;
    const long n = (long)h * (w >> 2);
    hipLaunchKernelGGL(head_update_kernel, dim3((unsigned)effi_cdiv(n, TPB)), dim3(TPB), 0, effi_s(stream), partial9, bias2, inv_depth,
                       disp_range, n_range, h, w, out_inv, out_depth);
    EFFI_LAUNCH_CHECK();
    return EFFI_OK;
}

extern "C" int effi_view_aggregate_f32(const float* sim_views, const float* weights, int S, int D, int hw,
                                       float* out, effi_stream_t stream) {
    if (!sim_views || !out || S < 1 || S > EFFI_MAX_VIEWS || D < 1 || hw < 1) return EFFI_ERR_BADARG;
    hipLaunchKernelGGL(view_aggregate_kernel, dim3(effi_cdiv(hw, TPB), effi_cdiv(D, 8)), dim3(TPB), 0, effi_s(stream),
                       sim_views, weights, S, D, hw, out);
    EFFI_LAUNCH_CHECK();
    return EFFI_OK;
}

extern "C" int effi_softmax_regress_conf_f32(const float* logits, const float* depth, long dds, long dps, int D,
                                             int hw, float* out_depth, float* out_conf, const float* disp_range, int n_range,
                                             float* out_depth_inv, effi_stream_t stream) {
    if (!logits || !depth || !out_depth || !out_conf || D < 1 || hw < 1) return EFFI_ERR_BADARG;
    if (out_depth_inv && (!disp_range || n_range < 2)) return EFFI_ERR_BADARG;
    const dim3 grid(effi_cdiv(hw, 64));
    hipStream_t st = effi_s(stream);
#define EFFI_SM(DT)                                                                                                      \
    hipLaunchKernelGGL(softmax_regress_conf_reg_kernel<DT>, grid, dim3(64), 0, st, logits, depth, dds, dps, hw, out_depth, \
                       out_conf, disp_range, n_range, out_depth_inv)
    switch (D) {
        case 8: EFFI_SM(8); break;
        case 16: EFFI_SM(16); break;
        case 32: EFFI_SM(32); break;
        case 48: EFFI_SM(48); break;
        case 64: EFFI_SM(64); break;
        case 96: EFFI_SM(96); break;
        default:
            hipLaunchKernelGGL(softmax_regress_conf_kernel, grid, dim3(64), 0, st, logits, depth, dds, dps, D, hw, out_depth, out_conf,
                               disp_range, n_range, out_depth_inv);
    }
#undef EFFI_SM
    EFFI_LAUNCH_CHECK();
    return EFFI_OK;
}

extern "C" int effi_vol_lookup1d_f32(const float* vol, long vds, long vps, int Dp, const float* query, long qds,
                                     long qys, long qxs, int nq, const float* dmin, const float* dmax, long rps,
                                     int h, int w, float* out, effi_stream_t stream) {
    if (!vol || !query || !dmin || !dmax || !out || Dp < 2 || nq < 1 || h < 1 || w < 1) return EFFI_ERR_BADARG;
    hipLaunchKernelGGL(vol_lookup1d_kernel, dim3(effi_cdiv((long)h * w, TPB)), dim3(TPB), 0, effi_s(stream), vol, vds,
                       vps, Dp, query, qds, qys, qxs, nq, dmin, dmax, rps, h, w, out, nullptr, nullptr);
    EFFI_LAUNCH_CHECK();
    return EFFI_OK;
}

extern "C" int effi_bilinear_sampler1d_f32(const float* img, int N, int C, int W, const float* coords, long nq, float* out,
                                           float* mask, effi_stream_t stream) {
    if (!img || !coords || !out || N < 1 || C < 1 || W < 1 || nq < 1) return EFFI_ERR_BADARG;
    const long total = (long)N * nq;
    hipLaunchKernelGGL(bilinear_sampler1d_kernel, dim3(effi_cdiv(total, TPB)), dim3(TPB), 0, effi_s(stream), img, C, W, coords, nq,
                       total, out, mask);
    EFFI_LAUNCH_CHECK();
    return EFFI_OK;
}

extern "C" int effi_vol_lookup1d_pair_f32(const float* vol_a, const float* vol_b, long vds, long vps, int Dp, const float* query,
                                          long qds, long qys, long qxs, int nq, const float* dmin, const float* dmax, long rps,
                                          int h, int w, float* out_a, float* out_b, effi_stream_t stream) {
    if (!vol_a || !vol_b || !query || !dmin || !dmax || !out_a || !out_b || Dp < 2 || nq < 1 || h < 1 || w < 1) return EFFI_ERR_BADARG;
    hipLaunchKernelGGL(vol_lookup1d_kernel, dim3(effi_cdiv((long)h * w, TPB), 2), dim3(TPB), 0, effi_s(stream), vol_a, vds,
                       vps, Dp, query, qds, qys, qxs, nq, dmin, dmax, rps, h, w, out_a, vol_b, out_b);
    EFFI_LAUNCH_CHECK();
    return EFFI_OK;
}

extern "C" int effi_getcost_f32(const float* inv_depth, const float* disp_range, int n_range, int input_is_depth,
// ... 77 lines not shown
                                       int w, const float* weight_c1, const float* bias_c1, const float* weight_d1,
                                       const float* bias_d1, int cout, float* out_c1, float* out_d1, effi_stream_t stream) {
    return encoder_inputs_launch(false, inv_depth, disp_range, n_range, interval, cur_vol, cds, cps, Dcur, reg_vol, rds, rps, Dreg, dmin,
                                 dmax, range_ps, nq, h, w, weight_c1, bias_c1, weight_d1, bias_d1, cout, out_c1, out_d1, stream);
}

extern "C" int effi_encoder_inputs_bf16x3_f32(const float* inv_depth, const float* disp_range, int n_range, const float* interval,
                                              const float* cur_vol, long cds, long cps, int Dcur, const float* reg_vol, long rds,
                                              long rps, int Dreg, const float* dmin, const float* dmax, long range_ps, int nq, int h,
                                              int w, const float* weight_c1, const float* bias_c1, const float* weight_d1,
                                              const float* bias_d1, int cout, float* out_c1, float* out_d1, effi_stream_t stream) {
    return encoder_inputs_launch(true, inv_depth, disp_range, n_range, interval, cur_vol, cds, cps, Dcur, reg_vol, rds, rps, Dreg, dmin,
                                 dmax, range_ps, nq, h, w, weight_c1, bias_c1, weight_d1, bias_d1, cout, out_c1, out_d1, stream);
}

extern "C" int effi_encoder_inputs_bf16x3_sr(const float* inv_depth, const float* disp_range, int n_range, const float* interval,
                                             const float* cur_vol, long cds, long cps, int Dcur, const float* reg_vol, long rds,
                                             long rps, int Dreg, const float* dmin, const float* dmax, long range_ps, int nq, int h,
                                             int w, const float* weight_c1, const float* bias_c1, const float* weight_d1,
                                             const float* bias_d1, int cout, void* sr_c1, void* sr_d1, int hp, int wp,
                                             effi_stream_t stream) {
    if (!sr_c1 || !sr_d1) return EFFI_ERR_BADARG;
    return encoder_inputs_launch(true, inv_depth, disp_range, n_range, interval, cur_vol, cds, cps, Dcur, reg_vol, rds, rps, Dreg, dmin,
                                 dmax, range_ps, nq, h, w, weight_c1, bias_c1, weight_d1, bias_d1, cout, nullptr, nullptr, stream,
                                 sr_c1, sr_d1, hp, wp);
}

namespace {
struct SrMaps {
    unsigned short* base[4];
    int planes[4], h[4], w[4], hp[4], wp[4];
    int first[5];
};
__global__ __launch_bounds__(TPB) void sr_clear_border_kernel(SrMaps a) {
    int k = 0;
#pragma unroll
    for (int j = 1; j < 4; ++j) k += ((int)blockIdx.x >= a.first[j]) ? 1 : 0;
    unsigned short* base = a.base[0];
    int planes = a.planes[0], h = a.h[0], w = a.w[0], hp = a.hp[0], wp = a.wp[0], b0 = a.first[0];
#pragma unroll
    for (int j = 1; j < 4; ++j)
        if (k == j) { base = a.base[j]; planes = a.planes[j]; h = a.h[j]; w = a.w[j]; hp = a.hp[j]; wp = a.wp[j]; b0 = a.first[j]; }
    const int rowpart = (hp - h) * wp, per_plane = rowpart + h * (wp - w);
    const long i = (long)(blockIdx.x - b0) * TPB + threadIdx.x;
    if (i >= (long)planes * per_plane) return;
    const int pl = (int)(i / per_plane), r = (int)(i - (long)pl * per_plane);
    int y, x;
    if (r < rowpart) {
        const int ry = r / wp;
        x = r - ry * wp;
        y = ry == 0 ? 0 : h + ry;
    } else {
        const int q = r - rowpart, ry = q / (wp - w), cx = q - ry * (wp - w);
        y = 1 + ry;
        x = cx == 0 ? 0 : w + cx;
    }
    *reinterpret_cast<float4*>(base + (((long)pl * hp + y) * wp + x) * 8) = make_float4(0.0f, 0.0f, 0.0f, 0.0f);
}

__global__ __launch_bounds__(TPB) void sr_from_planar_kernel(const float* __restrict__ in, int C, int h, int w, unsigned short* __restrict__ sr,
                                                             int hp, int wp) {
    const long hw = (long)h * w, i = (long)blockIdx.x * TPB + threadIdx.x;
    if (i >= (long)(C >> 3) * hw) return;
    const int o = (int)(i / hw);
    const long p = i - (long)o * hw;
    const int y = (int)(p / w), x = (int)(p - (long)y * w);
    float v[8];
#pragma unroll
    for (int e = 0; e < 8; ++e) v[e] = in[(long)(8 * o + e) * hw + p];
    effi_sr_store8(sr, hp, wp, 8 * o, y, x, v);
}

struct SplitStagesSr {
    const float* ctx[4];
    float* hidden[4];
    float* inp[4];
    unsigned short* hidden_sr[4];
    int hd[4], cd[4], h[4], w[4], hp[4], wp[4], q4[4];
    int first[5];
};
__global__ __launch_bounds__(TPB) void split_tanh_relu_stages_sr_kernel(SplitStagesSr a) {
    int k = 0;
#pragma unroll
    for (int j = 1; j < 4; ++j) k += ((int)blockIdx.x >= a.first[j]) ? 1 : 0;
    const float* __restrict__ ctx = a.ctx[0];
    float* __restrict__ hidden = a.hidden[0];
    float* __restrict__ inp = a.inp[0];
    unsigned short* __restrict__ hsr = a.hidden_sr[0];
    int hd = a.hd[0], cd = a.cd[0], h = a.h[0], w = a.w[0], hp = a.hp[0], wp = a.wp[0], b0 = a.first[0], q4 = a.q4[0];
#pragma unroll
    for (int j = 1; j < 4; ++j)
        if (k == j) {
            ctx = a.ctx[j]; hidden = a.hidden[j]; inp = a.inp[j]; hsr = a.hidden_sr[j];
            hd = a.hd[j]; cd = a.cd[j]; h = a.h[j]; w = a.w[j]; hp = a.hp[j]; wp = a.wp[j]; b0 = a.first[j]; q4 = a.q4[j];
        }
    const long hw = (long)h * w, n_h = (long)(hd >> 3) * hw, n_i = (long)(cd >> 2) * hw;
    const long i = (long)(blockIdx.x - b0) * TPB + threadIdx.x;
    if (i < n_h) {
        const int o = (int)(i / hw);
        const long p = i - (long)o * hw;
        const int y = (int)(p / w), x = (int)(p - (long)y * w);
        float v[8];
#pragma unroll
        for (int e = 0; e < 8; ++e) v[e] = tanhf(ctx[(long)(8 * o + e) * hw + p]);
        if (q4) {
            *reinterpret_cast<float4*>(hidden + ((long)(2 * o) * hw + p) * 4) = make_float4(v[0], v[1], v[2], v[3]);
            *reinterpret_cast<float4*>(hidden + ((long)(2 * o + 1) * hw + p) * 4) = make_float4(v[4], v[5], v[6], v[7]);
        } else {
#pragma unroll
            for (int e = 0; e < 8; ++e) hidden[(long)(8 * o + e) * hw + p] = v[e];
        }
        effi_sr_store8(hsr, hp, wp, 8 * o, y, x, v);
    } else if (i < n_h + n_i) {
        const long q = i - n_h;
        const int c4 = (int)(q / hw);
        const long p = q - (long)c4 * hw;
#pragma unroll
        for (int e = 0; e < 4; ++e) inp[(long)(4 * c4 + e) * hw + p] = fmaxf(ctx[(long)(hd + 4 * c4 + e) * hw + p], 0.0f);
    }
}
}

extern "C" int effi_sr_geometry(int h, int w, int* hp, int* wp) {
    if (h < 1 || w < 1 || !hp || !wp) return EFFI_ERR_BADARG;
    *hp = ((h + 15) & ~15) + 2;
    *wp = (w >= 512 ? ((w + 63) & ~63) : ((w + 15) & ~15)) + 2;
    return EFFI_OK;
}

extern "C" int effi_sr_clear_border(void* const* maps, const int* planes, const int* h, const int* w, const int* hp, const int* wp,
                                    int n_groups, effi_stream_t stream) {
    if (!maps || !planes || !h || !w || !hp || !wp || n_groups < 1 || n_groups > 4) return EFFI_ERR_BADARG;
    SrMaps a;
    int blocks = 0;
    for (int k = 0; k < 4; ++k) {
        const int j = k < n_groups ? k : 0;
        if (!maps[j] || planes[j] < 1 || h[j] < 1 || w[j] < 1 || hp[j] < h[j] + 2 || wp[j] < w[j] + 2 || (reinterpret_cast<uintptr_t>(maps[j]) & 15))
            return EFFI_ERR_BADARG;
        a.base[k] = reinterpret_cast<unsigned short*>(maps[j]);
        a.planes[k] = planes[j]; a.h[k] = h[j]; a.w[k] = w[j]; a.hp[k] = hp[j]; a.wp[k] = wp[j];
        a.first[k] = blocks;
        if (k < n_groups) blocks += effi_cdiv((long)planes[j] * ((long)(hp[j] - h[j]) * wp[j] + (long)h[j] * (wp[j] - w[j])), TPB);
    }
    a.first[4] = blocks;
    hipLaunchKernelGGL(sr_clear_border_kernel, dim3(blocks), dim3(TPB), 0, effi_s(stream), a);
    EFFI_LAUNCH_CHECK();
    return EFFI_OK;
}

extern "C" int effi_sr_from_planar_f32(const float* in, int channels, int h, int w, void* sr, int hp, int wp, effi_stream_t stream) {
    if (!in || !sr || channels < 8 || (channels & 7) || h < 1 || w < 1 || hp < h + 2 || wp < w + 2 || (reinterpret_cast<uintptr_t>(sr) & 15))
        return EFFI_ERR_BADARG;
    hipLaunchKernelGGL(sr_from_planar_kernel, dim3(effi_cdiv((long)(channels >> 3) * h * w, TPB)), dim3(TPB), 0, effi_s(stream), in,
                       channels, h, w, reinterpret_cast<unsigned short*>(sr), hp, wp);
    EFFI_LAUNCH_CHECK();
    return EFFI_OK;
}

extern "C" int effi_split_tanh_relu_stages_sr_f32(const float* const* ctx, const int* hd, const int* cd, const int* h, const int* w,
                                                  float* const* hidden, void* const* hidden_sr, const int* hp, const int* wp,
                                                  float* const* inp, const int* hidden_q4, int n_stages, effi_stream_t stream) {
    if (!ctx || !hd || !cd || !h || !w || !hidden || !hidden_sr || !hp || !wp || !inp || n_stages < 1 || n_stages > 4) return EFFI_ERR_BADARG;
    SplitStagesSr a;
    int blocks = 0;
    for (int k = 0; k < 4; ++k) {
        const int j = k < n_stages ? k : 0;
        if (!ctx[j] || !hidden[j] || !hidden_sr[j] || !inp[j] || hd[j] < 8 || cd[j] < 4 || h[j] < 1 || w[j] < 1) return EFFI_ERR_BADARG;
        if ((hd[j] & 7) || (cd[j] & 3)) return EFFI_ERR_UNSUPPORTED;
        if (hp[j] < h[j] + 2 || wp[j] < w[j] + 2 || (reinterpret_cast<uintptr_t>(hidden_sr[j]) & 15)) return EFFI_ERR_BADARG;
        a.ctx[k] = ctx[j]; a.hidden[k] = hidden[j]; a.inp[k] = inp[j]; a.hidden_sr[k] = reinterpret_cast<unsigned short*>(hidden_sr[j]);
        a.hd[k] = hd[j]; a.cd[k] = cd[j]; a.h[k] = h[j]; a.w[k] = w[j]; a.hp[k] = hp[j]; a.wp[k] = wp[j];
        a.q4[k] = hidden_q4 ? hidden_q4[j] : 0;
        if (a.q4[k] && (reinterpret_cast<uintptr_t>(hidden[j]) & 15)) return EFFI_ERR_BADARG;
        a.first[k] = blocks;
        if (k < n_stages) blocks += effi_cdiv((long)h[j] * w[j] * ((hd[j] >> 3) + (cd[j] >> 2)), TPB);
    }
    a.first[4] = blocks;
    hipLaunchKernelGGL(split_tanh_relu_stages_sr_kernel, dim3(blocks), dim3(TPB), 0, effi_s(stream), a);
    EFFI_LAUNCH_CHECK();
    return EFFI_OK;
}

namespace {
template <int COUT>
__global__ __launch_bounds__(TPB) void conv2d_c1k7_relu_x3_kernel(const float* __restrict__ in, const float* __restrict__ wgt,
                                                                  const float* __restrict__ bias, int h, int w, float* __restrict__ out) {
    effi_c1k7_relu_tile_x3<COUT>(in, wgt, bias, h, w, out, blockIdx.x, blockIdx.y);
}
}

extern "C" int effi_conv2d_c1k7_relu_bf16x3_f32(const float* in, const float* weight, const float* bias, int cout, int h, int w,
                                                float* out, effi_stream_t stream) {
    if (!in || !weight || !bias || !out || h < 1 || w < 1) return EFFI_ERR_BADARG;
    const dim3 grid(effi_cdiv(w, EFFI_C1K7_TX), effi_cdiv(h, EFFI_C1K7_TY));
    hipStream_t st = effi_s(stream);
    switch (cout) {
        case 16: hipLaunchKernelGGL(conv2d_c1k7_relu_x3_kernel<16>, grid, dim3(TPB), 0, st, in, weight, bias, h, w, out); break;
        case 32: hipLaunchKernelGGL(conv2d_c1k7_relu_x3_kernel<32>, grid, dim3(TPB), 0, st, in, weight, bias, h, w, out); break;
        case 48: hipLaunchKernelGGL(conv2d_c1k7_relu_x3_kernel<48>, grid, dim3(TPB), 0, st, in, weight, bias, h, w, out); break;
        default: return EFFI_ERR_UNSUPPORTED;
    }
    EFFI_LAUNCH_CHECK();
    return EFFI_OK;
}

extern "C" int effi_convex_upsample2x_f32(const float* inv_depth, const float* mask, const float* disp_range,
                                          int n_range, int h, int w, float* out_inv, float* out_depth,
                                          float* out_depth_inv, effi_stream_t stream) {
    if (!inv_depth || !mask || (!out_inv && !out_depth) || h < 1 || w < 1) return EFFI_ERR_BADARG;
    if (out_depth && (!disp_range || n_range < 2)) return EFFI_ERR_BADARG;
    if (out_depth_inv && !out_depth) return EFFI_ERR_BADARG;
    hipLaunchKernelGGL(convex_upsample2x_kernel, dim3(effi_cdiv((long)h * w, TPB)), dim3(TPB), 0, effi_s(stream),
                       inv_depth, mask, disp_range, n_range, h, w, out_inv, out_depth, out_depth_inv);
// ... 4 lines not shown
```

### effi_mvs_plus_amd/models/Effi_MVS_plus.py

```python
from __future__ import annotations

from functools import partial

import torch
import torch.nn as nn

from .. import ops, packing
from .module import (ConvBnReLU, CostRegNet_2_sample_FPN3D_Fast, P_1to8_FeatureNet_Fast, _require_eval,
                     cost_up_small, mvs_loss)
from .update import BasicUpdateBlock

Align_Corners_Range = False


def _stack(ts):
    return ts[0].unsqueeze(0) if len(ts) == 1 else torch.stack(ts)


def disp_to_depth(disp, min_depth, max_depth):
    lo, hi = 1 / max_depth, 1 / min_depth
    scaled = (lo + (hi - lo) * disp).clamp(min=1e-4)
    return scaled, 1 / scaled


# ... 218 lines not shown
        self.cdim = 32
        self.feat_ratio = [2, 2, 2]
        self.G = 1
        self.cost_dim_stage = [32, 16, 8]
        self.feature_in_channel = [8, 16, 32, 64]
        self.context_in_channel = [4, 8, 16, 32]
        if list(depth_interals_ratio) != [4, 2, 1] or not inverse or not stage_channel:
            raise NotImplementedError("Effi_MVS_plus: HIP path covers the shipped configuration "
                                      "(depth_interals_ratio=[4,2,1], inverse=True, stage_channel=True)")

        self.PixelwiseNet = PixelwiseNet2d()
        self.feature = P_1to8_FeatureNet_Fast(base_channels=4, in_channel=self.feature_in_channel,
                                              out_channel=self.cost_dim_stage, stage_channel=self.stage_channel)
        self.feature.channels_last_outputs = True
        self.cnet_depth = P_1to8_FeatureNet_Fast(base_channels=4, in_channel=self.context_in_channel,
                                                 out_channel=self.context_feature, stage_channel=self.stage_channel)
        blocks = [BasicUpdateBlock(hidden_dim=self.hdim_stage[s], cost_dim=self.G * self.CostNum,
                                   ratio=self.feat_ratio[s], context_dim=self.cdim_stage[s], UpMask=True,
                                   Inverse=self.inverse, cost_num=self.cost_num) for s in range(3)]
        self.update_block_depth1, self.update_block_depth2, self.update_block_depth3 = blocks
        self.update_block = nn.ModuleList(blocks)
        self.depthnet = DepthNet()
        self.CSP_R1 = cost_up_small(in_channels=self.G, base_channels=8)
        self.CSP_R2 = cost_up_small(in_channels=self.G, base_channels=8)
        self.CSP_R = nn.ModuleList([self.CSP_R1, self.CSP_R2])
        self.CSP_C1 = cost_up_small(in_channels=self.G, base_channels=8)
        self.CSP_C2 = cost_up_small(in_channels=self.G, base_channels=8)
        self.CSP_C = nn.ModuleList([self.CSP_C1, self.CSP_C2])
        self.cost_regularization = CostRegNet_2_sample_FPN3D_Fast(in_channels=self.G, base_channels=8)

    def _hot_single(self, feats, ctx, pairs, disp_range, want_intermediates=False):
        D1 = self.depth_stage_nums[0]
        ops.mark("begin")
        hyp, misc = ops.stage1_hypotheses(disp_range, D1)
        g_min, g_max = misc[3:4], misc[4:5]
        preds, inter = [], {}
        conf = None
        weights = reg_vol = cur_vol = None
        lo_prev, hi_prev = g_min, g_max

        keys = ["stage{}".format(s + 1) for s in range(self.num_stage)]
        if self.num_stage <= 4:
            rts = ops.compose_rel_proj_stages([pairs[k].contiguous() for k in keys])
        else:
            rts = [ops.compose_rel_proj(pairs[k]) for k in keys]

        table = feats if isinstance(feats, ops.ViewTable) else None

        def geometry(s):
            if table is not None:
                return (), rts[s], table.shapes[s]
            maps = [f[keys[s]] for f in feats]
            return ops.to_nhwc(maps), rts[s], maps[0].shape

        sr_maps = None
        use_sr = (ops.uses_sr() and self.num_stage <= 4 and self.CostNum == 3
                  and all(hd in (16, 32, 48) for hd in self.hdim_stage[:self.num_stage])
                  and all(ctx[k].shape[-1] % 4 == 0 for k in keys))

        state_q4 = [False] * self.num_stage

        def all_states():
            nonlocal sr_maps, state_q4
            cs = [ctx[k].contiguous() for k in keys]
            if use_sr:
                nm = BasicUpdateBlock.N_SR_MAPS
                sr_maps = [ops.sr_alloc(nm, self.hdim_stage[s], cs[s].shape[1], cs[s].shape[2], cs[s].device, clear=False)
                           for s in range(self.num_stage)]
                ops.sr_clear_border(sr_maps)
                state_q4 = [self.update_block[s].state_q4_ok(not want_intermediates) and ops.uses_sr(cs[s].shape[1] * cs[s].shape[2])
                            for s in range(self.num_stage)]
                return dict(enumerate(ops.split_tanh_relu_stages_sr(cs, self.hdim_stage[:self.num_stage], self.cdim_stage[:self.num_stage],
                                                                    [m[-1] for m in sr_maps], q4=state_q4)))
            if self.num_stage <= 4:
                return dict(enumerate(ops.split_tanh_relu_stages(cs, self.hdim_stage[:self.num_stage], self.cdim_stage[:self.num_stage])))
            return {s: ops.split_tanh_relu(cs[s], self.hdim_stage[s], self.cdim_stage[s]) for s in range(self.num_stage)}

        geo = {0: geometry(0)}
        with ops.Branch() as prep_branch:
            st = all_states()
            for s in range(1, self.num_stage):
                geo[s] = geometry(s)
        prep_joined = False
        tail_branch = None
        inv_next = None
        for s in range(self.num_stage):
            if s > 0:
                ops.mark("stage{}".format(s))
            nhwc, rt, (_, h, w) = geo[s]
            if s == 0:
                if table is not None:
                    sim_views, entropy = ops.warpcorr_views_tbl(table, 0, rt, hyp, D1, x3=bool(ops.option("warp_x3")))
                else:
                    sim_views, entropy = ops.warpcorr_views(nhwc[0], nhwc[1:], rt, hyp, D1, x3=bool(ops.option("warp_x3")))
                weights = self.PixelwiseNet.run(entropy)
                cur_vol = ops.view_aggregate(sim_views, weights)
                reg_vol = self.cost_regularization.run(cur_vol.unsqueeze(0))[0][0]
                depth, c, inv_next = ops.softmax_regress_conf(reg_vol, hyp, disp_range)
                with ops.Branch() as tail_branch:
                    conf = ops.upsample_nearest(c.unsqueeze(0), 4)[0]
                preds.append(depth)
                lo_cur, hi_cur = g_min, g_max
            else:
                D = self.depth_stage_nums[s]
                if table is not None:
                    sim, samples = ops.warpcorr_dyn_tbl(table, s, rt, preds[-1], misc[s:s + 1], weights, D)
                else:
                    sim, samples = ops.warpcorr_dyn(nhwc[0], nhwc[1:], rt, preds[-1], misc[s:s + 1], weights, D)
                x = sim.unsqueeze(0)
                csp_r, csp_c = self.CSP_R[s - 1], self.CSP_C[s - 1]
                if cur_vol.shape == reg_vol.shape and cur_vol.dim() == 3 and cost_up_small.pairable(csp_r, csp_c, x, w // 2):
                    prior, prior_c = ops.vol_lookup1d_pair(reg_vol, cur_vol, samples, lo_prev, hi_prev, h // 2, w // 2)
                    (reg_new, _), (cur_new, _) = cost_up_small.run_pair(csp_r, csp_c, x, prior.unsqueeze(0), prior_c.unsqueeze(0))
                    reg_vol, cur_vol = reg_new[0], cur_new[0]
                else:
                    with ops.Branch() as br:
                        prior_c = ops.vol_lookup1d(cur_vol, samples, lo_prev, hi_prev, h // 2, w // 2)
                        cur_new = csp_c.run(x, prior_c.unsqueeze(0))[0][0]
                    prior = ops.vol_lookup1d(reg_vol, samples, lo_prev, hi_prev, h // 2, w // 2)
                    reg_vol = csp_r.run(x, prior.unsqueeze(0))[0][0]
                    br.join(cur_new)
                    cur_vol = cur_new
                lo_cur, hi_cur = samples[D - 1], samples[0]
            if want_intermediates:
                inter["view_weights"] = weights
                inter["reg_volume{}".format(s + 1)] = reg_vol
                inter["cur_volume{}".format(s + 1)] = cur_vol
            if not prep_joined:
                prep_branch.join(*[t_ for k in st for t_ in st[k]], *[t_ for k in range(1, self.num_stage) for t_ in (list(geo[k][0]) + [geo[k][1]])])
                prep_joined = True
            hidden, inp = st[s]
            inv_cur = (inv_next if inv_next is not None else ops.depth_to_inv(preds[-1], disp_range)).unsqueeze(0)
            cur_c, reg_c, lo_c, hi_c, itv = cur_vol, reg_vol, lo_cur, hi_cur, misc[s:s + 1]
# ... 89 lines not shown
```

### effi_mvs_plus_amd/models/update.py

```python
from __future__ import annotations

import functools

import torch
import torch.nn as nn

from .. import ops, packing
from .module import _require_eval


def _pack(cache, conv, scale=1.0):
    return cache.get([conv.weight, conv.bias], lambda: packing.pack_conv2d(conv.weight, conv.bias, scale))


def _unbatched(t):
    return [t[i].contiguous() for i in range(t.shape[0])]


def _stack(ts):
    return ts[0].unsqueeze(0) if len(ts) == 1 else torch.stack(ts)


class DepthHead(nn.Module):

# ... 187 lines not shown
        w, b = _pack(self._m2, self.mask[2], scale=0.25)
        return ops.conv2d([hid], w, b, self.mask[2].out_channels, 1, act=ops.ACT_NONE)

    def mask_upsample_fusable(self, net):
        c1, c2 = self.mask[0].out_channels, self.mask[2].out_channels
        return (ops.uses_split() and net.shape[-1] % 4 == 0 and c1 in (32, 64, 96) and c2 == 36
                and self.mask[0].in_channels % 8 == 0)

    def run_mask_upsample(self, net, inv_depth, disp_range):
        w, b = _pack(self._m0, self.mask[0])
        c1 = self.mask[0].out_channels
        w2, b2 = self._m2u.get([self.mask[2].weight, self.mask[2].bias],
                               lambda: packing.pack_mask_taps_per_lane(self.mask[2].weight, self.mask[2].bias, c1, scale=0.25))
        return ops.conv2d_k3_k1_up2x([net], w.wx, b, c1, w2, b2, inv_depth, disp_range)

    N_SR_MAPS = 5

    def _sr_structure_ok(self, hd):
        e = self.encoder
        cmix, cd = e.convd.out_channels, e.convc.in_channels - e.convd.out_channels
        c1m = self.mask[0].out_channels
        return (hd in (16, 32, 48) and e.convd1.in_channels == 1 and cmix <= 48 and 0 <= cd <= 16 and e.convc.out_channels == hd
                and self.depth_head.conv1.out_channels == hd and self.depth_head.conv1.in_channels == hd
                and self.depth_head.conv2.out_channels == 1 and (not self.UpMask or (c1m in (32, 64, 96) and self.mask[2].out_channels == 36)))

    def sr_fusable(self, net, lookup):
        return (ops.uses_sr(net.shape[-1] * net.shape[-2]) and net.shape[-1] % 4 == 0 and getattr(lookup, "encoder_inputs_sr", None) is not None
                and self._sr_structure_ok(net.shape[0]))

    def state_q4_ok(self, fuse_upsample):
        return (bool(ops.option("state_q4")) and fuse_upsample and self.UpMask and not ops.option("gru_fused")
                and self._sr_structure_ok(self.depth_head.conv1.in_channels))

    def run_fused_sr(self, net, lookup, inv_depth, context, seq_len, disp_range, fuse_upsample=False, maps=None, net_sr_ready=False,
                     net_owned=False, net_q4=False):
        hd = net.shape[0]
        h, w = net.shape[-2:]
        dev = net.device
        if maps is None:
            maps = ops.sr_alloc(self.N_SR_MAPS, hd, h, w, dev)
        A, B, Cm, Dm, Hm = maps
        if net_q4 and not (net_sr_ready and net_owned and self.state_q4_ok(fuse_upsample)):
            raise ValueError("run_fused_sr: a Q4 state needs net_sr_ready, net_owned and the fused mask head")
        q4 = net_q4
        if not net_sr_ready:
            ops.sr_from_planar(net, out=Hm)
        gru_fused = hd <= 16 * ops.option("gru_fused")
        zh_buf = torch.empty(9 if gru_fused else max(hd, 9), h, w, device=dev, dtype=torch.float32)
        z_buf, head_buf = (None if gru_fused else zh_buf[:hd]), zh_buf[:9]
        h_own = net if net_owned else None
        e = self.encoder
        wc1, bc1 = e.convc1_raw()
        w7, b7 = e.conv7_packed()
        wd2, bd2 = _pack(e._caches["d2"], e.convd2)
        wc2, bc2 = _pack(e._caches["c2"], e.convc2)
        wd, bd = _pack(e._caches["d"], e.convd)
        cmix, cd = e.convd.out_channels, context.shape[0]
        wca, bca = e._caches["c_after"].get([e.convc.weight, e.convc.bias],
                                            lambda: packing.pack_conv1x1_after(e.convc.weight, e.convc.bias, cmix, cd))
        wzr, bzr = self.depth_gru._packed_zr()
        wq, bq = _pack(self.depth_gru._cq, self.depth_gru.convq)
        dh = self.depth_head
        wh1, bh1 = _pack(dh._c1, dh.conv1)
        wh2, bh2 = dh._c2t.get([dh.conv2.weight], lambda: packing.pack_head_taps(dh.conv2.weight, hd))
        inv_list, mask_list, depth_list = [], [], []
        gen_pair = ops.option("enc_gen") != 0 and getattr(lookup, "encoder_pair_sr", None) is not None
        H_first = Hm
        h_pp = [None, net if net_owned else None]
        for i in range(seq_len):
            if gen_pair:
                lookup.encoder_pair_sr(inv_depth, wc1, bc1, w7, b7, hd, wc2.wx, bc2, Cm, wd2.wx, bd2, Dm)
            else:
                lookup.encoder_inputs_sr(inv_depth, wc1, bc1, w7, b7, hd, A, B)
                ops.conv2d_k3_pair_sr([A], wc2.wx, bc2, Cm, [B], wd2.wx, bd2, Dm, hd, act=ops.ACT_RELU)
            ops.conv2d_k3_k1_sr([Cm, Dm], wd.wx, bd, cmix, context, wca, bca, hd, relu=True, out_sr=A)
            if gru_fused:
                h_next = h_pp[i % 2]
                if h_next is None or h_next.data_ptr() == net.data_ptr():
                    h_next = h_pp[i % 2] = torch.empty(hd, h, w, device=dev, dtype=torch.float32)
                H_next = B if Hm is not B else H_first
                net, _ = ops.gru_zr_q_fused_sr(Hm, A, net, wzr.wx, bzr, wq.wx, bq, h_next, H_next)
                Hm = H_next
            else:
                z, _ = ops.conv2d_k3_sr([Hm, A], wzr.wx, bzr, 2 * hd, epilogue=ops.EPI_GRU_ZR, aux0=net, out0=z_buf, out_sr=B, q4=q4)
                if h_own is None:
                    h_own = torch.empty(hd, h, w, device=dev, dtype=torch.float32)
                net, _ = ops.conv2d_k3_sr([B, A], wq.wx, bq, hd, epilogue=ops.EPI_GRU_Q, aux0=net, aux1=z, out0=h_own, out_sr=Hm, q4=q4)
            want_mask = self.UpMask and i == seq_len - 1
            fused_up = want_mask and fuse_upsample
            if want_mask and not fused_up:
                with ops.Branch() as br:
                    mask = self.run_mask(net)
            part = ops.conv2d_k3_k1_sr([Hm], wh1.wx, bh1, hd, None, wh2, bh2, 9, relu=False, relu1=True, out=head_buf)
            inv_depth, depth = ops.head_update(part, dh.conv2.bias, inv_depth, disp_range)
            if fused_up:
                wm, bm = _pack(self._m0, self.mask[0])
                c1 = self.mask[0].out_channels
                w2, b2 = self._m2u.get([self.mask[2].weight, self.mask[2].bias],
                                       lambda: packing.pack_mask_taps_per_lane(self.mask[2].weight, self.mask[2].bias, c1, scale=0.25))
                mask = ops.conv2d_k3_k1_up2x_sr([Hm], wm.wx, bm, c1, w2, b2, inv_depth, disp_range)
            elif want_mask:
                br.join(mask)
            inv_list.append(inv_depth)
            depth_list.append(depth)
            mask_list.append(mask if want_mask else inv_depth)
        return net, mask_list, inv_list, depth_list

    def run_fused(self, net, lookup, inv_depth, context, seq_len, disp_range, fuse_upsample=False, sr_maps=None, net_sr_ready=False,
                  net_owned=False, net_q4=False):
        if self.sr_fusable(net, lookup):
            return self.run_fused_sr(net, lookup, inv_depth, context, seq_len, disp_range, fuse_upsample, sr_maps, net_sr_ready, net_owned, net_q4)
        if net_q4:
            raise ValueError("run_fused: a Q4 state was passed but the block does not take the split-resident path")
        hd = net.shape[0]
        h, w = net.shape[-2:]
        dev = net.device
        mk = lambda c: torch.empty(c, h, w, device=dev, dtype=torch.float32)
        bufs = {"cor1": mk(hd), "cor2": mk(hd), "dfm1": mk(hd), "dfm2": mk(hd)}
        bufs["enc"] = bufs["cor1"]
        bufs["enc_tail"] = bufs["dfm2"]
        z_buf, rh_buf, head_buf, cost_buf = bufs["dfm1"], bufs["cor2"], bufs["dfm2"], None
        h_bufs = [mk(hd), mk(hd)]
        inv_list, mask_list, depth_list = [], [], []
        fuse_c1 = getattr(lookup, "conv1x1", None) is not None and hd % 8 == 0
        fuse_in = fuse_c1 and getattr(lookup, "encoder_inputs", None) is not None and hd in (16, 32, 48)
        for i in range(seq_len):
            if fuse_c1:
# ... 67 lines not shown
```

### effi_mvs_plus_amd/ops.py

```python
from __future__ import annotations

import ctypes as C
import functools
import os
import threading

import weakref

import torch

from . import _lib
from ._lib import EffiLibraryError, check

ACT_NONE, ACT_RELU, ACT_SIGMOID, ACT_TANH = 0, 1, 2, 3
EPI_PLAIN, EPI_GRU_ZR, EPI_GRU_Q, EPI_HEAD, EPI_ADD_UP2, EPI_NHWC = 0, 1, 2, 3, 4, 5
EPI_ADD_SHUF2, EPI_NHWC_ADD_SHUF2 = 9, 10
MAX_VIEWS = 12


class KernelProfile:

    def __init__(self, keys=None):
        self.keys = None if keys is None else set(keys)
        self.records = []
# ... 21 lines not shown
            d["flops"] += work.get("flops", 0.0)
            d["bytes"] += work.get("bytes", 0.0)
        return out


_PROF = None

PRECISIONS = ("split", "fp32", "bf16")
_PRECISION = os.environ.get("EFFI_MVS_PRECISION", "split")
if _PRECISION not in PRECISIONS:
    raise ValueError(f"EFFI_MVS_PRECISION must be one of {PRECISIONS}, got {_PRECISION!r}")


def set_precision(mode):
    global _PRECISION
    if mode not in PRECISIONS:
        raise ValueError(f"precision must be one of {PRECISIONS}, got {mode!r}")
    _PRECISION = mode


def get_precision():
    return _PRECISION


def uses_split():
    return _PRECISION in ("split", "bf16")


def _x3(name):
    return getattr(_lib.lib(), name + "_bf16" if _PRECISION == "bf16" else name)


_PY_OPTION_DEFAULTS = {"warp_x3": 0, "state_q4": 1, "c1k7_mfma": 1, "k5s2_split": 1, "roll": 1, "conv3d_unaligned_split": 1, "conv3d_s2_split": 1, "fpn_conv0_fused": 1,
                       "fpn_split_head": 1, "csp_pair": 1, "head_taps": 1, "enc_tail": 0, "enc_gen": 1, "reduce_chunk": 2048, "gru_fused": 0, "csp_gen": 0}
_PY_OPTS = {k: int(os.environ.get("EFFI_" + k.upper(), v)) for k, v in _PY_OPTION_DEFAULTS.items()}
LIB_OPTIONS = ("warp_lds_kb", "dyn_form", "dyn_setup_exact", "dyn_xchg", "pixnet_mfma", "force_mr", "mr4_min", "mr4_nt2_max", "mr2_min",
               "wide_tiles", "roll_mr", "roll_zt", "roll_rp", "deconv_mr", "sr_waves", "enc_gen_mr3", "c3_lean", "dyn_win")


def option(name):
    return _PY_OPTS[name]


def get_option(name):
    if name in _PY_OPTS:
        return _PY_OPTS[name]
    if name not in LIB_OPTIONS:
        raise KeyError(name)
    L = _lib.lib()
    v = L.effi_get_option(name.encode())
    return None if v == L.effi_option_unset() else int(v)


def set_option(name, value):
    before = get_option(name)
    if name in _PY_OPTS:
        _PY_OPTS[name] = _PY_OPTION_DEFAULTS[name] if value is None else int(value)
    else:
        L = _lib.lib()
        check(L.effi_set_option(name.encode(), L.effi_option_unset() if value is None else int(value)), "effi_set_option")
    return before


class options:

    def __init__(self, **kw):
        self.kw, self.before = kw, {}
# ... 164 lines not shown
        _MARKS.append((name, ev))


def _stream():
    return C.c_void_p(torch._C._cuda_getCurrentRawStream(torch._C._cuda_getDevice()))


def _ptr_array(tensors):
    return (C.c_void_p * len(tensors))(*[t.data_ptr() for t in tensors])


def _int_array(vals):
    return (C.c_int * len(vals))(*vals)


def compose_rel_proj(pairs: torch.Tensor) -> torch.Tensor:
    _t(pairs, "pairs")
    n = pairs.shape[0]
    rt = torch.empty(n - 1, 12, device=pairs.device, dtype=torch.float32)
    check(_lib.lib().effi_compose_rel_proj_f32(_p(pairs), n, _p(rt), _stream()), "effi_compose_rel_proj_f32")
    return rt


def compose_rel_proj_stages(pairs_list):
    for p_ in pairs_list:
        _t(p_, "pairs")
    n = pairs_list[0].shape[0]
    if len(pairs_list) > 4 or any(p_.shape[0] != n for p_ in pairs_list):
        raise ValueError("compose_rel_proj_stages: up to 4 stages with the same number of views")
    rt = torch.empty(len(pairs_list), n - 1, 12, device=pairs_list[0].device, dtype=torch.float32)
    check(_lib.lib().effi_compose_rel_proj_stages_f32(_ptr_array(pairs_list), len(pairs_list), n, _p(rt), _stream()),
          "effi_compose_rel_proj_stages_f32")
    return [rt[k] for k in range(len(pairs_list))]


def rel_proj(src_proj: torch.Tensor, ref_proj: torch.Tensor) -> torch.Tensor:
    _t(src_proj, "src_proj"), _t(ref_proj, "ref_proj")
    rt = torch.empty(12, device=src_proj.device, dtype=torch.float32)
    check(_lib.lib().effi_rel_proj_f32(_p(src_proj), _p(ref_proj), _p(rt), _stream()), "effi_rel_proj_f32")
    return rt


def to_nhwc(feats):
    out, todo_src, todo_dst = [None] * len(feats), [], []
    for i, f in enumerate(feats):
        _t(f, "feature", contiguous=False)
        C_, h, w = f.shape
        if f.permute(1, 2, 0).is_contiguous() and C_ > 1:
            out[i] = f.permute(1, 2, 0)
        else:
            if not f.is_contiguous():
                raise ValueError("feature map must be planar-contiguous or channels-last")
            d = torch.empty(h, w, C_, device=f.device, dtype=torch.float32)
            out[i] = d
            todo_src.append(f)
            todo_dst.append(d)
    if todo_src:
        C_, h, w = todo_src[0].shape
        for k in range(0, len(todo_src), MAX_VIEWS + 1):
            s, d = todo_src[k:k + MAX_VIEWS + 1], todo_dst[k:k + MAX_VIEWS + 1]
            check(_lib.lib().effi_planar_to_nhwc_f32(_ptr_array(s), _ptr_array(d), len(s), C_, h * w, _stream()),
                  "effi_planar_to_nhwc_f32")
    return out


def _depth_strides(depth: torch.Tensor, D, h, w):
# ... 389 lines not shown
    work = lambda: {"flops": 0.0, "bytes": 4.0 * h * w * (1 + V + 1 + 1 + (3 if want_points else 0)) + 3.0 * h * w}
    check(_call("fusion_dtu_filter", work, _lib.lib().effi_fusion_dtu_filter_f32, _p(ref_depth), _p(src_depths), _p(ref_cam), _p(src_cams),
                V, h, w, _p(conf), float(conf_threshold), float(conf_keep), int(s), int(e), float(dist_base), float(diff_base), _p(scratch),
                _p(out["depth"]), _p(out["photo_mask"]), _p(out["geo_mask"]), _p(out["mask"]), _p(out["points"]), _stream()),
          "effi_fusion_dtu_filter_f32")
    return out


def image_prepare(img_u8, dst_h, dst_w, out=None):
    if not isinstance(img_u8, torch.Tensor) or img_u8.dtype != torch.uint8 or not img_u8.is_contiguous():
        raise TypeError("image_prepare: contiguous uint8 tensor [h,w,c] expected")
    if img_u8.dim() == 2:
        img_u8 = img_u8.unsqueeze(-1)
    if not img_u8.is_cuda:
        raise _lib.EffiLibraryError("effi_image_prepare_u8_f32 needs a tensor on the GPU (there is no CPU fallback)")
    h, w, c = img_u8.shape
    if out is None:
        out = torch.empty(c, dst_h, dst_w, device=img_u8.device, dtype=torch.float32)
    work = lambda: {"flops": 0.0, "bytes": 1.0 * h * w * c + 4.0 * c * dst_h * dst_w}
    check(_call("image_prepare", work, _lib.lib().effi_image_prepare_u8_f32, C.c_void_p(img_u8.data_ptr()), h, w, c, dst_h, dst_w,
                _p(out), _stream()), "effi_image_prepare_u8_f32")
    return out


def resize_planar(x, dst_h, dst_w, out=None):
    _t(x, "image")
    c, h, w = x.shape
    if out is None:
        out = torch.empty(c, dst_h, dst_w, device=x.device, dtype=torch.float32)
    check(_lib.lib().effi_resize_linear_f32(_p(x), c, h, w, dst_h, dst_w, _p(out), _stream()), "effi_resize_linear_f32")
    return out


def softmax_regress_conf(logits, depth, disp_range=None):
    D, h, w = logits.shape
    _t(logits, "logits"), _t(depth, "depth", contiguous=False)
    depth, dds, dps = _depth_strides(depth, D, h, w)
    od = torch.empty(h, w, device=logits.device, dtype=torch.float32)
    oc = torch.empty(h, w, device=logits.device, dtype=torch.float32)
    oi, n_range = None, 0
    if disp_range is not None:
        _t(disp_range, "disp_range")
        oi, n_range = torch.empty(h, w, device=logits.device, dtype=torch.float32), disp_range.numel()
    check(_lib.lib().effi_softmax_regress_conf_f32(_p(logits), _p(depth), dds, dps, D, h * w, _p(od), _p(oc), _p(disp_range), n_range,
                                                    _p(oi), _stream()), "effi_softmax_regress_conf_f32")
    return (od, oc) if disp_range is None else (od, oc, oi)


def _vol_strides(vol, h, w):
    _t(vol, "volume", contiguous=False)
    if vol.dim() == 3:
        if not vol.is_contiguous():
            vol = vol.contiguous()
        return vol, h * w, 1, vol.shape[0]
    if vol.dim() == 4 and vol.shape[0] == h * w:
        return vol, vol.stride(3), vol.stride(0), vol.shape[3]
    raise ValueError(f"unsupported volume shape {tuple(vol.shape)}")


def _range_ptr(r, h, w):
    _t(r, "range", contiguous=False)
    if r.numel() == 1:
        return r.reshape(1), 0
    if r.numel() == h * w:
        return r.reshape(h, w).contiguous(), 1
    raise ValueError(f"depth range with {r.numel()} elements does not match {h}x{w}")


def vol_lookup1d(vol, query, dmin, dmax, h, w):
    vol, vds, vps, Dp = _vol_strides(vol, h, w)
    _t(query, "query")
    nq, qh, qw = query.shape
    if (qh, qw) == (h, w):
        qys, qxs = qw, 1
    elif (qh // 2, qw // 2) == (h, w):
        qys, qxs = 2 * qw, 2
# ... 280 lines not shown
        self.t, self.channels, self.h, self.w = t, channels, h, w
        self.hp, self.wp = t.shape[2], t.shape[3]

    def parts(self):
        v = self.t[:, :, 1:self.h + 1, 1:self.w + 1, :].float()
        v = v.permute(1, 0, 4, 2, 3).reshape(2, self.channels, self.h, self.w)
        return v[0], v[1]


def sr_alloc(n_maps, channels, h, w, device, clear=True):
    if channels % 8:
        raise ValueError("SR maps hold whole octets of channels")
    hp, wp = sr_geometry(h, w)
    block = torch.empty(n_maps, channels // 8, 2, hp, wp, 8, device=device, dtype=torch.bfloat16)
    maps = [SRMap(block[i], channels, h, w) for i in range(n_maps)]
    if clear:
        sr_clear_border([maps])
    return maps


def _sr(m, name):
    if not isinstance(m, SRMap):
        raise TypeError(f"{name}: expected an SRMap")
    t_ = m.t
    if not t_.is_cuda:
        raise EffiLibraryError(f"{name}: CPU tensor passed to the HIP path (no CPU fallback exists)")
    if t_.device.index != torch._C._cuda_getDevice():
        raise EffiLibraryError(f"{name}: map lives on cuda:{t_.device.index} but the current device is cuda:{torch._C._cuda_getDevice()}")
    if t_.dtype != torch.bfloat16 or not t_.is_contiguous():
        raise ValueError(f"{name}: SR maps are contiguous bf16 tensors")
    return m


def sr_clear_border(groups):
    if not 1 <= len(groups) <= 4:
        raise ValueError("sr_clear_border: 1..4 groups")
    firsts = [_sr(g[0], "SR map") for g in groups]
    planes = [2 * (g[0].channels // 8) * len(g) for g in groups]
    for g in groups:
        step = g[0].t.numel() * 2
        if any(m.t.data_ptr() != g[0].t.data_ptr() + i * step for i, m in enumerate(g)):
            raise ValueError("sr_clear_border: a group must be consecutive maps of one sr_alloc block")
    check(_lib.lib().effi_sr_clear_border(_ptr_array([m.t for m in firsts]), _int_array(planes), _int_array([m.h for m in firsts]),
                                           _int_array([m.w for m in firsts]), _int_array([m.hp for m in firsts]),
                                           _int_array([m.wp for m in firsts]), len(groups), _stream()), "effi_sr_clear_border")


def sr_from_planar(x, out=None):
    _t(x, "map")
    Cc, h, w = x.shape
    if out is None:
        out = sr_alloc(1, Cc, h, w, x.device)[0]
    check(_lib.lib().effi_sr_from_planar_f32(_p(x), Cc, h, w, _p(_sr(out, "SR map").t), out.hp, out.wp, _stream()), "effi_sr_from_planar_f32")
    return out


def split_tanh_relu_stages_sr(ctxs, hds, cds, hidden_srs, q4=None):
    outs = []
    for c_, hd, cd, m in zip(ctxs, hds, cds, hidden_srs):
        _t(c_, "context"), _sr(m, "hidden SR map")
        _, h, w = c_.shape
        if (m.channels, m.h, m.w) != (hd, h, w):
            raise ValueError("split_tanh_relu_stages_sr: SR map does not match the hidden state")
        outs.append((torch.empty(hd, h, w, device=c_.device, dtype=torch.float32),
                     torch.empty(cd, h, w, device=c_.device, dtype=torch.float32)))
    if len(ctxs) > 4:
        raise ValueError("split_tanh_relu_stages_sr: up to 4 stages")
    check(_lib.lib().effi_split_tanh_relu_stages_sr_f32(
        _ptr_array(ctxs), _int_array(list(hds)), _int_array(list(cds)), _int_array([c_.shape[1] for c_ in ctxs]),
        _int_array([c_.shape[2] for c_ in ctxs]), _ptr_array([o[0] for o in outs]), _ptr_array([m.t for m in hidden_srs]),
        _int_array([m.hp for m in hidden_srs]), _int_array([m.wp for m in hidden_srs]), _ptr_array([o[1] for o in outs]),
        _int_array([int(bool(v)) for v in (q4 if q4 is not None else [0] * len(ctxs))]), len(ctxs),
        _stream()), "effi_split_tanh_relu_stages_sr_f32")
    return outs


def encoder_inputs_sr(x, disp_range, interval, cur_vol, reg_vol, dmin, dmax, nq, h, w, weight_c1, bias_c1, weight_d1, bias_d1, cout,
                      out_c1, out_d1):
    _t(x, "inv_depth"), _t(interval, "interval"), _t(disp_range, "disp_range")
    for t_ in (weight_c1, bias_c1, weight_d1, bias_d1):
        _t(t_, "encoder weights")
    _sr(out_c1, "out_c1"), _sr(out_d1, "out_d1")
    cur_vol, cds, cps, Dc = _vol_strides(cur_vol, h, w)
    reg_vol, rds, rps, Dr = _vol_strides(reg_vol, h, w)
    dmin_t, gps = _range_ptr(dmin, h, w)
    dmax_t, gps2 = _range_ptr(dmax, h, w)
    if gps != gps2:
        raise ValueError("depth_min / depth_max must both be global or both per-pixel")
    if (out_c1.channels, out_c1.h, out_c1.w) != (cout, h, w) or (out_d1.channels, out_d1.h, out_d1.w) != (cout, h, w):
        raise ValueError("encoder_inputs_sr: output maps must be [cout,h,w]")
    work = lambda: {"flops": 2.0 * h * w * (2 * nq + 49) * cout, "bytes": 4.0 * h * w * (2 * cout + 1 + Dc + Dr)}
    check(_call("encoder_inputs", work, _lib.lib().effi_encoder_inputs_bf16x3_sr, _p(x), _p(disp_range), disp_range.numel(),
                _p(interval), _p(cur_vol), cds, cps, Dc, _p(reg_vol), rds, rps, Dr, _p(dmin_t), _p(dmax_t), gps, nq, h, w,
                _p(weight_c1), _p(bias_c1), _p(weight_d1), _p(bias_d1), cout, _p(out_c1.t), _p(out_d1.t), out_c1.hp, out_c1.wp,
                _stream()), "effi_encoder_inputs_bf16x3_sr")
    return out_c1, out_d1


def encoder_pair_gen_sr(x, disp_range, interval, cur_vol, reg_vol, dmin, dmax, nq, h, w, weight_c1, bias_c1, weight_d1, bias_d1, hd,
                        wpack_c2, bias_c2, out_c2, wpack_d2, bias_d2, out_d2, cout, act=ACT_RELU):
# ... 83 lines not shown
def conv2d_k3_pair_sr(srcs_a, wpack_a, bias_a, out_a, srcs_b, wpack_b, bias_b, out_b, cout, act=ACT_NONE):
    g = _sr_srcs(list(srcs_a) + list(srcs_b) + [out_a, out_b])
    h, w = g.h, g.w
    cin = sum(m.channels for m in srcs_a) + sum(m.channels for m in srcs_b)
    work = lambda: {"flops": 2.0 * h * w * cin * cout * 9, "bytes": 4.0 * h * w * (cin + 2 * cout)}
    check(_call(f"conv2d_k3x3_pair_nt{(cout + 15) // 16}", work, _x3("effi_conv2d_k3_bf16x3_pair_sr"), _ptr_array([m.t for m in srcs_a]),
                _int_array([m.channels for m in srcs_a]), len(srcs_a), _p(wpack_a), _p(bias_a), _p(out_a.t),
                _ptr_array([m.t for m in srcs_b]), _int_array([m.channels for m in srcs_b]), len(srcs_b), _p(wpack_b), _p(bias_b),
                _p(out_b.t), cout, h, w, g.hp, g.wp, act, _stream()), "effi_conv2d_k3_bf16x3_pair_sr")
    return out_a, out_b


def conv2d_k3_k1_sr(srcs, wpack, bias, cout1, extra, w2pack, bias2, cout2, relu=True, relu1=False, out=None, out_sr=None):
    g = _sr_srcs(srcs)
    h, w = g.h, g.w
    c_extra = 0
    if extra is not None:
        _t(extra, "extra channels")
        c_extra = extra.shape[0]
    if out_sr is None and out is None:
        out = torch.empty(cout2, h, w, device=g.t.device, dtype=torch.float32)
    if out_sr is not None:
        _sr(out_sr, "out_sr")
        if (out_sr.channels, out_sr.h, out_sr.w) != (cout2, h, w):
            raise ValueError("conv2d_k3_k1_sr: output map does not match")
    cin = sum(m.channels for m in srcs)
    work = lambda: {"flops": 2.0 * h * w * (cin * cout1 * 9 + (cout1 + c_extra) * cout2),
                    "bytes": 4.0 * h * w * (cin + c_extra + cout2)}
    check(_call(f"conv2d_k3k1_nt{(cout1 + 15) // 16}", work, _x3("effi_conv2d_k3_k1_bf16x3_sr"), _ptr_array([m.t for m in srcs]),
                _int_array([m.channels for m in srcs]), len(srcs), _p(wpack), _p(bias), cout1, int(relu1), _p(extra), c_extra,
                _p(w2pack), _p(bias2), cout2, int(relu), h, w, g.hp, g.wp, _p(None if out_sr is not None else out),
                _p(out_sr.t if out_sr is not None else None), _stream()), "effi_conv2d_k3_k1_bf16x3_sr")
    return out_sr if out_sr is not None else out


def conv2d_k3_k1_up2x_sr(srcs, wpack, bias, cout1, w2pack, bias2, inv_depth, disp_range, want_depth_inv=True):
    g = _sr_srcs(srcs)
    _t(inv_depth, "inv_depth"), _t(disp_range, "disp_range")
    h, w = g.h, g.w
    dev = g.t.device
    out_depth = torch.empty(2 * h, 2 * w, device=dev, dtype=torch.float32)
    out_dinv = torch.empty(2 * h, 2 * w, device=dev, dtype=torch.float32) if want_depth_inv else None
    cin = sum(m.channels for m in srcs)
    work = lambda: {"flops": 2.0 * h * w * (cin * cout1 * 9 + cout1 * 36), "bytes": 4.0 * h * w * (cin + 1 + 8)}
    check(_call(f"conv2d_k3k1up_nt{(cout1 + 15) // 16}", work, _x3("effi_conv2d_k3_k1_up2x_bf16x3_sr"), _ptr_array([m.t for m in srcs]),
                _int_array([m.channels for m in srcs]), len(srcs), _p(wpack), _p(bias), cout1, _p(w2pack), _p(bias2), _p(inv_depth),
                _p(disp_range), disp_range.numel(), h, w, g.hp, g.wp, _p(out_depth), _p(out_dinv), _stream()),
          "effi_conv2d_k3_k1_up2x_bf16x3_sr")
    return out_depth, out_dinv


def conv2d_k3_k1_x3(srcs, wpack, bias, cout1, extra, w2pack, bias2, cout2, relu=True, out=None, relu1=False):
    for s in srcs:
        _t(s, "conv2d input")
    h, w = srcs[0].shape[-2:]
    c_extra = 0
    if extra is not None:
        _t(extra, "extra channels")
        c_extra = extra.shape[0]
    if out is None:
        out = torch.empty(cout2, h, w, device=srcs[0].device, dtype=torch.float32)
    cin = sum(s.shape[0] for s in srcs)
    work = lambda: {"flops": 2.0 * h * w * (cin * cout1 * 9 + (cout1 + c_extra) * cout2),
                    "bytes": 4.0 * h * w * (cin + c_extra + cout2)}
    check(_call(f"conv2d_k3k1_nt{(cout1 + 15) // 16}", work, _x3("effi_conv2d_k3_k1_bf16x3_f32"), _ptr_array(srcs),
                _int_array([s.shape[0] for s in srcs]), len(srcs), _p(wpack), _p(bias), cout1, int(relu1), _p(extra), c_extra,
# ... 404 lines not shown
```

### include/effi_mvs_hip.h

```cpp
#ifndef EFFI_MVS_HIP_H
#define EFFI_MVS_HIP_H

#ifdef __cplusplus
extern "C" {
#endif

#define EFFI_OK               0
#define EFFI_ERR_BADARG      -1
#define EFFI_ERR_UNSUPPORTED -2
#define EFFI_ERR_LAUNCH      -3
#define EFFI_ERR_WORKSPACE   -4

#define EFFI_MAX_VIEWS 12
#define EFFI_MAX_SRC    3
#define EFFI_VIEW_TABLE_ROW (EFFI_MAX_VIEWS + 2)
#define EFFI_VIEW_TABLE_MAX 64

typedef void* effi_stream_t;

#define EFFI_ACT_NONE    0
#define EFFI_ACT_RELU    1
#define EFFI_ACT_SIGMOID 2
#define EFFI_ACT_TANH    3
#define EFFI_EPI_PLAIN   0
#define EFFI_EPI_GRU_ZR  1
#define EFFI_EPI_GRU_Q   2
#define EFFI_EPI_Q4      0x100
#define EFFI_EPI_HEAD    3
#define EFFI_EPI_NHWC    5
#define EFFI_EPI_ADD_SHUF2 9
#define EFFI_EPI_NHWC_ADD_SHUF2 10
#define EFFI_EPI_ADD_UP2 4

int effi_version(void);
const char* effi_error_string(int code);

#define EFFI_MAX_DEVICES 64
long effi_workspace_bytes(void);
int effi_set_workspace(int device, void* workspace, long bytes);
const void* effi_get_workspace(int device);

int effi_compose_rel_proj_f32(const float* pairs, int n_views, float* rt_out, effi_stream_t stream);
int effi_compose_rel_proj_stages_f32(const float* const* pairs, int n_stages, int n_views, float* rt_out,
                                     effi_stream_t stream);
int effi_rel_proj_f32(const float* src_proj, const float* ref_proj, float* rt_out, effi_stream_t stream);

int effi_planar_to_nhwc_f32(const float* const* srcs, float* const* dsts, int n, int C, int HW,
                            effi_stream_t stream);

int effi_homo_warp_f32(const float* src_nhwc, const float* rt, const float* depth, long depth_dstride,
                       long depth_pstride, int C, int h, int w, int D, float* out, effi_stream_t stream);

int effi_warpcorr_views_f32(const float* ref_nhwc, const float* const* src_nhwc, int S, const float* rt,
                            const float* depth, long depth_dstride, long depth_pstride,
                            int C, int h, int w, int D, float* sim_views, float* entropy,
                            effi_stream_t stream);

int effi_warpcorr_views_tbl_f32(const float* const* view_table_dev, int S, const float* rt, const float* depth,
                                long depth_dstride, long depth_pstride, int C, int h, int w, int D, float* sim_views,
                                float* entropy, effi_stream_t stream);
int effi_view_table_set(const void** table_dev, const void* const* ptrs, int n, effi_stream_t stream);

int effi_pixelwise_net_f32(const float* entropy, const float* params, int n, int h, int w, float* weight,
                           effi_stream_t stream);

int effi_view_aggregate_f32(const float* sim_views, const float* weights, int S, int D, int hw, float* out,
                            effi_stream_t stream);

int effi_warpcorr_dyn_f32(const float* ref_nhwc, const float* const* src_nhwc, int S, const float* rt,
                          const float* cur_depth, const float* interval, const float* view_w, int vw_shift,
                          int C, int h, int w, int D, float* sim, float* samples, effi_stream_t stream);

int effi_warpcorr_dyn_tbl_f32(const float* const* view_table_dev, int S, const float* rt, const float* cur_depth,
                              const float* interval, const float* view_w, int vw_shift, int C, int h, int w, int D,
                              float* sim, float* samples, effi_stream_t stream);

int effi_conv3d_k3_f32(const float* const* srcs, const int* src_channels, int n_src,
                       const float* weight, const float* bias, int cout,
// ... 10 lines not shown
int effi_conv2d_k3_bf16x3_pair_f32(const float* const* srcs_a, const int* src_channels_a, int n_src_a, const void* wpack_a,
                                   const float* bias_a, float* out_a, const float* const* srcs_b,
                                   const int* src_channels_b, int n_src_b, const void* wpack_b, const float* bias_b,
                                   float* out_b, int cout, int h, int w, int act, effi_stream_t stream);
int effi_conv2d_k5s2_bf16x3_f32(const float* in, int cin, const void* wpack_bf16, const float* bias, int cout, int hin, int win,
                                int act, float* out, effi_stream_t stream);
int effi_conv3d_k3s2_bf16x3_f32(const float* in, int cin, const void* wpack_bf16, const float* bias, int cout, int D, int h, int w,
                                int relu, float* out, effi_stream_t stream);
int effi_conv2d_k3_twice_bf16x3_f32(const float* in, int cin, const void* w1_bf16, const float* bias1, const void* w2_bf16,
                                    const float* bias2, int cout, int h, int w, float* out, effi_stream_t stream);
int effi_encoder_tail_bf16x3_f32(const float* cor1, const float* dfm1, int hd, const void* wc2_bf16, const float* bias_c2,
                                 const void* wd2_bf16, const float* bias_d2, const void* wd_bf16, const float* bias_d, int cmix,
                                 const float* extra, int c_extra, const void* w2pack_bf16, const float* bias2, int cout2, int h,
                                 int w, float* out, effi_stream_t stream);
int effi_conv2d_k3_k1_up2x_bf16x3_f32(const float* const* srcs, const int* src_channels, int n_src, const void* wpack_bf16,
                                      const float* bias, int cout1, const void* w2pack_bf16, const float* bias2,
                                      const float* inv_depth, const float* disp_range, int n_range, int h, int w,
                                      float* out_depth, float* out_depth_inv, effi_stream_t stream);
int effi_conv3d_k3s1_bf16x3_f32(const float* const* srcs, const int* src_channels, int n_src, const void* wpack_bf16,
                                const float* bias, int cout, int D, int h, int w, int relu, float* out,
                                effi_stream_t stream);
int effi_conv3d_k3s1_roll_bf16x3_f32(const float* const* srcs, const int* src_channels, int n_src, const void* wpack_bf16,
                                     const float* bias, int cout, int D, int h, int w, int relu, float* out,
                                     effi_stream_t stream);
int effi_deconv3d_k3_f32(const float* in, int cin, const float* weight, const float* bias, int cout,
                         int D, int h, int w, int sz, int relu, const float* skip,
                         float* out, effi_stream_t stream);
int effi_deconv3d_k3s2_bf16x3_f32(const float* in, int cin, const void* wpack_bf16, const float* bias, int cout,
                                  int D, int h, int w, int relu, const float* skip, float* out, effi_stream_t stream);

int effi_softmax_regress_conf_f32(const float* logits, const float* depth, long depth_dstride,
                                  long depth_pstride, int D, int hw, float* out_depth, float* out_conf,
                                  const float* disp_range, int n_range, float* out_depth_inv, effi_stream_t stream);

int effi_vol_lookup1d_f32(const float* vol, long vol_dstride, long vol_pstride, int Dp,
                          const float* query, long q_dstride, long q_ystride, long q_xstride, int nq,
                          const float* dmin, const float* dmax, long range_pstride,
                          int h, int w, float* out, effi_stream_t stream);

int effi_bilinear_sampler1d_f32(const float* img, int N, int C, int W, const float* coords, long nq, float* out, float* mask,
                                effi_stream_t stream);

int effi_getcost_f32(const float* inv_depth, const float* disp_range, int n_range, int input_is_depth,
                     const float* interval,
                     const float* cur_vol, long cur_dstride, long cur_pstride, int Dcur,
                     const float* reg_vol, long reg_dstride, long reg_pstride, int Dreg,
                     const float* dmin, const float* dmax, long range_pstride, int nq,
                     int h, int w, float* cost, effi_stream_t stream);

int effi_getcost_conv1x1_f32(const float* inv_depth, const float* disp_range, int n_range, int input_is_depth,
                             const float* interval,
                             const float* cur_vol, long cur_dstride, long cur_pstride, int Dcur,
                             const float* reg_vol, long reg_dstride, long reg_pstride, int Dreg,
                             const float* dmin, const float* dmax, long range_pstride, int nq,
                             int h, int w, const float* weight, const float* bias, int cout, int relu,
                             float* out, effi_stream_t stream);

int effi_encoder_inputs_f32(const float* inv_depth, const float* disp_range, int n_range, const float* interval,
                            const float* cur_vol, long cur_dstride, long cur_pstride, int Dcur,
                            const float* reg_vol, long reg_dstride, long reg_pstride, int Dreg,
                            const float* dmin, const float* dmax, long range_pstride, int nq, int h, int w,
                            const float* weight_c1, const float* bias_c1, const float* weight_d1, const float* bias_d1,
                            int cout, float* out_c1, float* out_d1, effi_stream_t stream);
int effi_encoder_inputs_bf16x3_f32(const float* inv_depth, const float* disp_range, int n_range, const float* interval,
                            const float* cur_vol, long cur_dstride, long cur_pstride, int Dcur,
                            const float* reg_vol, long reg_dstride, long reg_pstride, int Dreg,
// ... 175 lines not shown
int effi_conv3d_k3s1_bf16x3_f32_bf16(const float* const* srcs, const int* src_channels, int n_src, const void* wpack_bf16,
                                const float* bias, int cout, int D, int h, int w, int relu, float* out,
                                effi_stream_t stream);
int effi_conv3d_k3s1_roll_bf16x3_f32_bf16(const float* const* srcs, const int* src_channels, int n_src, const void* wpack_bf16,
                                     const float* bias, int cout, int D, int h, int w, int relu, float* out,
                                     effi_stream_t stream);
int effi_conv3d_k3s1_roll_bf16x3_pair_f32_bf16(const float* const* srcs_a, const void* wpack_a, const float* bias_a, float* out_a,
                                          const float* const* srcs_b, const void* wpack_b, const float* bias_b, float* out_b,
                                          const int* src_channels, int n_src, int cout, int D, int h, int w, int relu,
                                          effi_stream_t stream);
int effi_csp_gen_roll_bf16x3_pair_f32_bf16(const float* x, int D, int H, int W, const float* prior_a, const float* w0_a, const float* b0_a,
                                      const float* wc_a, const float* bc_a, const void* w1_a, const float* b1_a, float* out_a,
                                      const float* prior_b, const float* w0_b, const float* b0_b, const float* wc_b, const float* bc_b,
                                      const void* w1_b, const float* b1_b, float* out_b, effi_stream_t stream);
int effi_deconv3d_k3s2_bf16x3_f32_bf16(const float* in, int cin, const void* wpack_bf16, const float* bias, int cout,
                                  int D, int h, int w, int relu, const float* skip, float* out, effi_stream_t stream);

int effi_fusion_dtu_filter_f32(const float* ref_depth, const float* src_depths, const float* ref_cam, const float* src_cams, int n_src,
                               int h, int w, const float* confidence, float conf_threshold, float conf_keep, int s, int e,
                               float dist_base, float diff_base, float* mats_scratch, float* out_depth, unsigned char* out_photo_mask,
                               unsigned char* out_geo_mask, unsigned char* out_final_mask, float* out_points, effi_stream_t stream);

int effi_set_option(const char* name, long value);
long effi_get_option(const char* name);
long effi_option_unset(void);

int effi_sr_geometry(int h, int w, int* hp, int* wp);
int effi_sr_clear_border(void* const* maps, const int* planes, const int* h, const int* w, const int* hp, const int* wp, int n_groups,
                         effi_stream_t stream);
int effi_sr_from_planar_f32(const float* in, int channels, int h, int w, void* sr, int hp, int wp, effi_stream_t stream);
int effi_split_tanh_relu_stages_sr_f32(const float* const* ctx, const int* hd, const int* cd, const int* h, const int* w,
                                       float* const* hidden, void* const* hidden_sr, const int* hp, const int* wp, float* const* inp,
                                       const int* hidden_q4, int n_stages, effi_stream_t stream);
int effi_encoder_inputs_bf16x3_sr(const float* inv_depth, const float* disp_range, int n_range, const float* interval,
                                  const float* cur_vol, long cds, long cps, int Dcur, const float* reg_vol, long rds, long rps,
                                  int Dreg, const float* dmin, const float* dmax, long range_ps, int nq, int h, int w,
                                  const float* weight_c1, const float* bias_c1, const float* weight_d1, const float* bias_d1,
                                  int cout, void* sr_c1, void* sr_d1, int hp, int wp, effi_stream_t stream);
int effi_encoder_pair_gen_bf16x3_sr(const float* inv_depth, const float* disp_range, int n_range, const float* interval,
                                    const float* cur_vol, long cds, long cps, int Dcur, const float* reg_vol, long rds, long rps,
                                    int Dreg, const float* dmin, const float* dmax, long range_ps, int nq, int h, int w,
                                    const float* weight_c1, const float* bias_c1, const float* weight_d1, const float* bias_d1, int hd,
                                    const void* wpack_c2, const float* bias_c2, void* out_sr_c2, const void* wpack_d2,
                                    const float* bias_d2, void* out_sr_d2, int cout, int hp, int wp, int act, effi_stream_t stream);
int effi_conv2d_k3_bf16x3_sr(const void* const* srcs, const int* src_channels, int n_src, const void* wpack_bf16, const float* bias,
                             int cout, int h, int w, int hp, int wp, int epilogue, int act, const float* aux0, const float* aux1,
                             float* out0, void* out_sr, effi_stream_t stream);
int effi_conv2d_k3_bf16x3_pair_sr(const void* const* srcs_a, const int* src_channels_a, int n_src_a, const void* wpack_a,
                                  const float* bias_a, void* out_sr_a, const void* const* srcs_b, const int* src_channels_b,
                                  int n_src_b, const void* wpack_b, const float* bias_b, void* out_sr_b, int cout, int h, int w,
                                  int hp, int wp, int act, effi_stream_t stream);
int effi_conv2d_k3_k1_bf16x3_sr(const void* const* srcs, const int* src_channels, int n_src, const void* wpack_bf16, const float* bias,
                                int cout1, int relu1, const float* extra, int c_extra, const void* w2pack_bf16, const float* bias2,
                                int cout2, int relu, int h, int w, int hp, int wp, float* out, void* out_sr, effi_stream_t stream);
int effi_conv2d_k3_k1_up2x_bf16x3_sr(const void* const* srcs, const int* src_channels, int n_src, const void* wpack_bf16,
                                     const float* bias, int cout1, const void* w2pack_bf16, const float* bias2, const float* inv_depth,
                                     const float* disp_range, int n_range, int h, int w, int hp, int wp, float* out_depth,
                                     float* out_depth_inv, effi_stream_t stream);
int effi_gru_zr_q_fused_bf16x3_sr(const void* H_in, const void* X, const float* h_in, const void* wzr_pack, const float* bias_zr,
                                  const void* wq_pack, const float* bias_q, int hd, int h, int w, int hp, int wp, float* h_out,
                                  void* H_out, effi_stream_t stream);
int effi_conv2d_k3_bf16x3_sr_bf16(const void* const* srcs, const int* src_channels, int n_src, const void* wpack_bf16, const float* bias,
                                  int cout, int h, int w, int hp, int wp, int epilogue, int act, const float* aux0, const float* aux1,
                                  float* out0, void* out_sr, effi_stream_t stream);
int effi_conv2d_k3_bf16x3_pair_sr_bf16(const void* const* srcs_a, const int* src_channels_a, int n_src_a, const void* wpack_a,
                                       const float* bias_a, void* out_sr_a, const void* const* srcs_b, const int* src_channels_b,
                                       int n_src_b, const void* wpack_b, const float* bias_b, void* out_sr_b, int cout, int h, int w,
                                       int hp, int wp, int act, effi_stream_t stream);
int effi_conv2d_k3_k1_bf16x3_sr_bf16(const void* const* srcs, const int* src_channels, int n_src, const void* wpack_bf16,
                                     const float* bias, int cout1, int relu1, const float* extra, int c_extra, const void* w2pack_bf16,
                                     const float* bias2, int cout2, int relu, int h, int w, int hp, int wp, float* out, void* out_sr,
                                     effi_stream_t stream);
int effi_conv2d_k3_k1_up2x_bf16x3_sr_bf16(const void* const* srcs, const int* src_channels, int n_src, const void* wpack_bf16,
                                          const float* bias, int cout1, const void* w2pack_bf16, const float* bias2,
                                          const float* inv_depth, const float* disp_range, int n_range, int h, int w, int hp, int wp,
                                          float* out_depth, float* out_depth_inv, effi_stream_t stream);
int effi_gru_zr_q_fused_bf16x3_sr_bf16(const void* H_in, const void* X, const float* h_in, const void* wzr_pack, const float* bias_zr,
                                       const void* wq_pack, const float* bias_q, int hd, int h, int w, int hp, int wp, float* h_out,
                                       void* H_out, effi_stream_t stream);
int effi_encoder_pair_gen_bf16x3_sr_bf16(const float* inv_depth, const float* disp_range, int n_range, const float* interval,
                                         const float* cur_vol, long cds, long cps, int Dcur, const float* reg_vol, long rds, long rps,
                                         int Dreg, const float* dmin, const float* dmax, long range_ps, int nq, int h, int w,
                                         const float* weight_c1, const float* bias_c1, const float* weight_d1, const float* bias_d1,
                                         int hd, const void* wpack_c2, const float* bias_c2, void* out_sr_c2, const void* wpack_d2,
                                         const float* bias_d2, void* out_sr_d2, int cout, int hp, int wp, int act, effi_stream_t stream);

#ifdef __cplusplus
}
#endif
#endif
```

Baseline: 631.4 views/s.

## Fuse depth head into one launch and merge cascade setup and SR-clear kernels

```diff
diff --git a/effi_mvs_plus_amd/_lib.py b/effi_mvs_plus_amd/_lib.py
--- a/effi_mvs_plus_amd/_lib.py
+++ b/effi_mvs_plus_amd/_lib.py
@@ -39,6 +39,7 @@
     "effi_conv3d_k3s1_mfma_f32": [_vp, _i, _vp, _vp, _i, _i, _i, _i, _i, _vp, _vp],
     "effi_deconv3d_k3_f32": [_vp, _i, _vp, _vp, _i, _i, _i, _i, _i, _i, _vp, _vp, _vp],
     "effi_softmax_regress_conf_f32": [_vp, _vp, _l, _l, _i, _i, _vp, _vp, _vp, _i, _vp, _vp],
+    "effi_softmax_regress_conf_up_f32": [_vp, _vp, _l, _l, _i, _i, _i, _vp, _vp, _vp, _i, _vp, _vp, _i, _vp],
     "effi_vol_lookup1d_f32": [_vp, _l, _l, _i, _vp, _l, _l, _l, _i, _vp, _vp, _l, _i, _i, _vp, _vp],
     "effi_bilinear_sampler1d_f32": [_vp, _i, _i, _i, _vp, _l, _vp, _vp, _vp],
     "effi_getcost_conv1x1_f32": [_vp, _vp, _i, _i, _vp, _vp, _l, _l, _i, _vp, _l, _l, _i, _vp, _vp, _l, _i, _i, _i, _vp, _vp, _i,
@@ -73,6 +74,7 @@
     "effi_conv2d_c1k7_relu_bf16x3_f32": [_vp, _vp, _vp, _i, _i, _i, _vp, _vp],
     "effi_convex_upsample2x_f32": [_vp, _vp, _vp, _i, _i, _i, _vp, _vp, _vp, _vp],
     "effi_compose_rel_proj_stages_f32": [_vp, _i, _i, _vp, _vp],
+    "effi_cascade_setup_f32": [_vp, _i, _i, _vp, _vp, _vp, _i, _i, _vp, _vp],
     "effi_split_tanh_relu_stages_f32": [_vp, _vp, _vp, _vp, _vp, _vp, _i, _vp],
     "effi_split_tanh_relu_f32": [_vp, _i, _i, _i, _vp, _vp, _vp],
     "effi_depth_to_inv_f32": [_vp, _vp, _i, _i, _vp, _vp],
@@ -85,6 +87,8 @@
     "effi_sr_clear_border": [_vp, _vp, _vp, _vp, _vp, _vp, _i, _vp],
     "effi_sr_from_planar_f32": [_vp, _i, _i, _i, _vp, _i, _i, _vp],
     "effi_split_tanh_relu_stages_sr_f32": [_vp, _vp, _vp, _vp, _vp, _vp, _vp, _vp, _vp, _vp, _vp, _i, _vp],
+    "effi_split_tanh_relu_stages_sr_clear_f32": [_vp, _vp, _vp, _vp, _vp, _vp, _vp, _vp, _vp, _vp, _vp, _vp, _vp, _i, _vp],
+    "effi_depth_head_bf16x3_sr": [_vp, _vp, _i, _vp, _vp, _i, _vp, _vp, _vp, _vp, _vp, _i, _i, _i, _i, _i, _i, _vp, _vp, _vp],
     "effi_encoder_inputs_bf16x3_sr": [_vp, _vp, _i, _vp, _vp, _l, _l, _i, _vp, _l, _l, _i, _vp, _vp, _l, _i, _i, _i, _vp, _vp, _vp, _vp,
                                       _i, _vp, _vp, _i, _i, _vp],
     "effi_encoder_pair_gen_bf16x3_sr": [_vp, _vp, _i, _vp, _vp, _l, _l, _i, _vp, _l, _l, _i, _vp, _vp, _l, _i, _i, _i, _vp, _vp, _vp, _vp,
@@ -117,7 +121,7 @@
                   "effi_conv3d_k3s1_roll_bf16x3_pair_f32", "effi_csp_gen_roll_bf16x3_pair_f32", "effi_deconv3d_k3s2_bf16x3_f32", "effi_encoder_tail_bf16x3_f32", "effi_conv2d_k3_twice_bf16x3_f32",
                   "effi_conv2d_k5s2_bf16x3_f32", "effi_conv3d_k3s2_bf16x3_f32",
                   "effi_conv2d_k3_bf16x3_sr", "effi_conv2d_k3_bf16x3_pair_sr", "effi_conv2d_k3_k1_bf16x3_sr", "effi_conv2d_k3_k1_up2x_bf16x3_sr",
-                  "effi_encoder_pair_gen_bf16x3_sr", "effi_gru_zr_q_fused_bf16x3_sr")
+                  "effi_encoder_pair_gen_bf16x3_sr", "effi_gru_zr_q_fused_bf16x3_sr", "effi_depth_head_bf16x3_sr")
 for _n in BF16X3_ENTRIES:
     SIGNATURES[_n + "_bf16"] = SIGNATURES[_n]
 
diff --git a/effi_mvs_plus_amd/csrc/common.hpp b/effi_mvs_plus_amd/csrc/common.hpp
--- a/effi_mvs_plus_amd/csrc/common.hpp
+++ b/effi_mvs_plus_amd/csrc/common.hpp
@@ -120,6 +120,25 @@
     return (s_ - min_disp) / den;
 }
 
+__device__ __forceinline__ void effi_stage1_hypotheses_block(const float* __restrict__ disp_range, int n_range, int D,
+                                                             float* __restrict__ depths, float* __restrict__ intervals) {
+    const float lo = disp_range[0], hi = disp_range[n_range - 1];
+    const float step = (hi - lo) / (float)(D - 1);
+    for (int d = threadIdx.x; d < D; d += blockDim.x) {
+        const float s = lo + (float)d * step;
+        depths[d] = 1.0f / s;
+    }
+    if (threadIdx.x < 3) {
+        const float base = (hi - lo) / (float)n_range;
+        const float ratio = (threadIdx.x == 0) ? 4.0f : (threadIdx.x == 1 ? 2.0f : 1.0f);
+        intervals[threadIdx.x] = base * ratio;
+    } else if (threadIdx.x == 3) {
+        intervals[3] = 1.0f / hi;
+    } else if (threadIdx.x == 4) {
+        intervals[4] = 1.0f / lo;
+    }
+}
+
 __device__ __forceinline__ float effi_lk_rcp(float b) {
 #ifdef EFFI_EXACT_LOOKUP
     return 1.0f / b;
diff --git a/effi_mvs_plus_amd/csrc/conv2d_sr.hip b/effi_mvs_plus_amd/csrc/conv2d_sr.hip
--- a/effi_mvs_plus_amd/csrc/conv2d_sr.hip
+++ b/effi_mvs_plus_amd/csrc/conv2d_sr.hip
@@ -174,6 +174,36 @@
     }
 }
 
+extern "C" int EFFI_FN(effi_depth_head_bf16x3_sr)(const void* const* srcs, const int* src_channels, int n_src, const void* wpack_bf16,
+                                                  const float* bias, int cout1, const void* w2pack_bf16, const float* bias2_taps,
+                                                  const float* bias2, const float* inv_depth, const float* disp_range, int n_range,
+                                                  int h, int w, int hp, int wp, int tile, float* out_inv, float* out_depth,
+                                                  effi_stream_t stream) {
+    if (!w2pack_bf16 || !bias2_taps || !bias2 || !inv_depth || !disp_range || n_range < 2 || !out_inv || !out_depth) return EFFI_ERR_BADARG;
+    if (cout1 < 1 || cout1 > 48) return EFFI_ERR_UNSUPPORTED;
+    Conv2dArgs a;
+    const int rc = fill_sr(a, srcs, src_channels, n_src, wpack_bf16, bias, cout1, h, w, hp, wp);
+    if (rc != EFFI_OK) return rc;
+    a.kgroups = 1;
+    a.hd = 0;
+    a.aux0 = inv_depth;
+    a.aux1 = reinterpret_cast<const float*>(w2pack_bf16);
+    a.disp_range = bias2_taps;
+    a.n_range = 9;
+    a.zeros = bias2;
+    a.out0 = out_inv;
+    a.out1 = out_depth;
+    a.zin = n_range;
+    a.xptr0 = disp_range;
+    hipStream_t st = effi_s(stream);
+    switch ((cout1 + 15) / 16) {
+        case 1: return launch_bf16x3_head<1>(a, tile, st);
+        case 2: return launch_bf16x3_head<2>(a, tile, st);
+        case 3: return launch_bf16x3_head<3>(a, tile, st);
+        default: return EFFI_ERR_UNSUPPORTED;
+    }
+}
+
 extern "C" int EFFI_FN(effi_conv2d_k3_k1_up2x_bf16x3_sr)(const void* const* srcs, const int* src_channels, int n_src,
                                                          const void* wpack_bf16, const float* bias, int cout1, const void* w2pack_bf16,
                                                          const float* bias2, const float* inv_depth, const float* disp_range,
diff --git a/effi_mvs_plus_amd/csrc/conv2d_x3.hpp b/effi_mvs_plus_amd/csrc/conv2d_x3.hpp
--- a/effi_mvs_plus_amd/csrc/conv2d_x3.hpp
+++ b/effi_mvs_plus_amd/csrc/conv2d_x3.hpp
@@ -195,6 +195,7 @@
 
 #define EFFI_EPI_K1 6
 #define EFFI_EPI_K1UP 8
+#define EFFI_EPI_K1HEAD 7
 typedef __bf16 bf16x2 __attribute__((ext_vector_type(2)));
 typedef float f32x2 __attribute__((ext_vector_type(2)));
 
@@ -230,7 +231,9 @@
     static_assert(SR || NITEMS <= 256, "one staging item per thread");
     static_assert(!(SR && ZB), "split-resident maps are 2-D");
     static_assert(EPI != EFFI_EPI_HEAD && EPI != EFFI_EPI_ADD_UP2, "epilogue not instantiated for the split-precision kernel");
-    static_assert((EPI != EFFI_EPI_K1 && EPI != EFFI_EPI_K1UP) || !ZB, "the fused 1x1 epilogue is 2-D only");
+    static_assert((EPI != EFFI_EPI_K1 && EPI != EFFI_EPI_K1UP && EPI != EFFI_EPI_K1HEAD) || !ZB, "the fused 1x1 epilogue is 2-D only");
+    constexpr bool kHead = EPI == EFFI_EPI_K1HEAD;
+    static_assert(!kHead || (SR && !WIDE && !GEN), "the one-launch depth head reads split-resident maps on 16-column tiles");
     __shared__ __attribute__((aligned(16))) unsigned short lds_ah[SR ? NUA * NTHR * 8 : APIX * CCH];
     __shared__ __attribute__((aligned(16))) unsigned short lds_al[SR ? 8 : APIX * CCH];
     __shared__ __attribute__((aligned(16))) unsigned short lds_b[NB4 * NTHR * 8];
@@ -245,7 +248,7 @@
     const int tile = effi_xcd_remap(bid, nbid);
     if (tile >= ntiles) return;
     const int ty_ = tile / tiles_x;
-    const int x0 = (tile - ty_ * tiles_x) * TW, y0 = ty_ * TR;
+    const int x0 = kHead ? (tile - ty_ * tiles_x) * (TW - 2) - 1 : (tile - ty_ * tiles_x) * TW, y0 = kHead ? ty_ * (TR - 2) - 1 : ty_ * TR;
     const int zpl = ZB ? bidy : 0;
 
     const bool stager = tid < NITEMS;
@@ -270,7 +273,8 @@
             const int part = u / (2 * APIXP), r_ = u - part * (2 * APIXP);
             const int oct = r_ / APIXP, p = r_ - oct * APIXP;
             const int row = p / AW, col = p - row * AW;
-            const bool valid = (part < NPART) & (p < APIX);
+            bool valid = (part < NPART) & (p < APIX);
+            if (kHead) valid &= (y0 + row >= 0) & (y0 + row < a.sr_hp) & (x0 + col >= 0) & (x0 + col < a.sr_wp);
             goff[j] = valid ? ((oct * 2 + part) * a.sr_hp + (y0 + row)) * a.sr_wp + (x0 + col) : 0;
         }
     }
@@ -504,7 +508,7 @@
         }
     };
 
-    constexpr bool kK1 = (EPI == EFFI_EPI_K1 || EPI == EFFI_EPI_K1UP) && !(EFFI_ABL & 24) && EFFI_EPI_BATCH != 0;
+    constexpr bool kK1 = (EPI == EFFI_EPI_K1 || EPI == EFFI_EPI_K1UP || kHead) && !(EFFI_ABL & 24) && EFFI_EPI_BATCH != 0;
     f32x4 kb[kK1 ? NT : 1], kex[kK1 ? MR : 1];
     if constexpr (kK1) {
 #pragma unroll
@@ -629,7 +633,7 @@
         }
         return;
     }
-    if (EPI == EFFI_EPI_K1 || EPI == EFFI_EPI_K1UP) {
+    if (EPI == EFFI_EPI_K1 || EPI == EFFI_EPI_K1UP || kHead) {
         const unsigned short* w2 = reinterpret_cast<const unsigned short*>(a.aux1);
         const int nt2 = (a.n_range + 15) >> 4;
         const bool relu1 = a.kgroups != 0;
@@ -641,7 +645,7 @@
         for (int m = 0; m < MR; ++m) {
             const int x = x0 + li + (WIDE ? 16 * m : 0);
             const int y = y0 + (WIDE ? wv : wv * MR + m);
-            inside[m] = (y < h) & (x < w);
+            inside[m] = (y < h) & (x < w) & (!kHead || ((y >= 0) & (x >= 0)));
             pixm[m] = inside[m] ? (long)y * w + x : 0;
             if constexpr (kK1) {
                 ex[m] = kex[m];
@@ -740,18 +744,21 @@
             }
             return;
         }
-        for (int t = 0; t < nt2; ++t) {
+        if constexpr (kHead) {
+            constexpr int TPIX = TR * TW;
+            static_assert(9 * TPIX * 4 <= (int)sizeof(lds_ah), "the tap planes fit the A image");
+            float* taps = reinterpret_cast<float*>(lds_ah);
             bf16x4 wh[NT + 1], wl[NT + 1];
 #pragma unroll
             for (int n = 0; n <= NT; ++n) {
-                const long f = ((long)(t * (NT + 1) + n) * 2) * 64 + lane;
+                const long f = ((long)n * 2) * 64 + lane;
                 wh[n] = *reinterpret_cast<const bf16x4*>(w2 + f * 4);
                 wl[n] = *reinterpret_cast<const bf16x4*>(w2 + (f + 64) * 4);
             }
-            const int co = t * 16 + 4 * lk;
             float b2[4];
 #pragma unroll
-            for (int r = 0; r < 4; ++r) b2[r] = a.disp_range[co + r];
+            for (int r = 0; r < 4; ++r) b2[r] = a.disp_range[4 * lk + r];
+            __syncthreads();
 #pragma unroll
             for (int m = 0; m < MR; ++m) {
                 f32x4 o = {0.0f, 0.0f, 0.0f, 0.0f};
@@ -763,6 +770,59 @@
                         o = __builtin_amdgcn_mfma_f32_16x16x16bf16_1k(wh[n], xl[m][n], o, 0, 0, 0);
                     }
                 }
+#pragma unroll
+                for (int r = 0; r < 4; ++r)
+                    if (4 * lk + r < 9) taps[(4 * lk + r) * TPIX + (wv * MR + m) * TW + li] = o[r] + b2[r];
+            }
+            __syncthreads();
+            const float b = a.zeros[0], lo = a.xptr0[0], hi = a.xptr0[a.zin - 1];
+            constexpr int IR = TR - 2, IC = TW - 2;
+            for (int p = tid; p < IR * IC; p += NTHR) {
+                const int iy = p / IC, ix = p - iy * IC;
+                const int y = y0 + 1 + iy, x = x0 + 1 + ix;
+                if (y >= h || x >= w) continue;
+                float s = 0.0f;
+#pragma unroll
+                for (int ky = 0; ky < 3; ++ky) {
+                    const int yy = y + ky - 1;
+                    if (yy < 0 || yy >= h) continue;
+#pragma unroll
+                    for (int kx = 0; kx < 3; ++kx) {
+                        const int xx = x + kx - 1;
+                        const float t_ = taps[(ky * 3 + kx) * TPIX + (iy + ky) * TW + ix + kx];
+                        s = s + ((xx >= 0 && xx < w) ? t_ : 0.0f);
+                    }
+                }
+                const long pix = (long)y * w + x;
+                const float o = a.aux0[pix] + tanhf(s + b);
+                a.out0[pix] = o;
+                a.out1[pix] = effi_inv_to_depth(o, lo, hi);
+            }
+            return;
+        }
+        for (int t = 0; t < nt2; ++t) {
+            bf16x4 wh[NT + 1], wl[NT + 1];
+#pragma unroll
+            for (int n = 0; n <= NT; ++n) {
+                const long f = ((long)(t * (NT + 1) + n) * 2) * 64 + lane;
+                wh[n] = *reinterpret_cast<const bf16x4*>(w2 + f * 4);
+                wl[n] = *reinterpret_cast<const bf16x4*>(w2 + (f + 64) * 4);
+            }
+            const int co = t * 16 + 4 * lk;
+            float b2[4];
+#pragma unroll
+            for (int r = 0; r < 4; ++r) b2[r] = a.disp_range[co + r];
+#pragma unroll
+            for (int m = 0; m < MR; ++m) {
+                f32x4 o = {0.0f, 0.0f, 0.0f, 0.0f};
+#pragma unroll
+                for (int n = 0; n <= NT; ++n) {
+                    o = __builtin_amdgcn_mfma_f32_16x16x16bf16_1k(wh[n], xh[m][n], o, 0, 0, 0);
+                    if (!kHiOnly) {
+                        o = __builtin_amdgcn_mfma_f32_16x16x16bf16_1k(wl[n], xh[m][n], o, 0, 0, 0);
+                        o = __builtin_amdgcn_mfma_f32_16x16x16bf16_1k(wh[n], xl[m][n], o, 0, 0, 0);
+                    }
+                }
                 if (inside[m]) {
                     f32x4 vo;
 #pragma unroll
@@ -840,7 +900,7 @@
         const long pix = (long)y * w + x;
 #pragma unroll
         for (int n = 0; n < NT; ++n)
-            conv_epilogue_store_t<((EPI == EFFI_EPI_K1 || EPI == EFFI_EPI_K1UP) ? EFFI_EPI_PLAIN : EPI), SR>(a, acc[m][n], n * 16 + 4 * lk, pix, hw, zpl, y, x,
+            conv_epilogue_store_t<((EPI == EFFI_EPI_K1 || EPI == EFFI_EPI_K1UP || EPI == EFFI_EPI_K1HEAD) ? EFFI_EPI_PLAIN : EPI), SR>(a, acc[m][n], n * 16 + 4 * lk, pix, hw, zpl, y, x,
                                                                                                           kBiasQ ? &gb[n] : nullptr);
     }
 }
@@ -915,6 +975,18 @@
     return hipPeekAtLastError() == hipSuccess ? EFFI_OK : EFFI_ERR_LAUNCH;
 }
 
+template <int NT>
+static int launch_bf16x3_head(const Conv2dArgs& a, int tile, hipStream_t st) {
+    const int tr = tile == 2 ? 8 : 16;
+    const int tiles_x = effi_cdiv(a.w, 14), ntiles = tiles_x * effi_cdiv(a.h, tr - 2);
+    const dim3 grid(ntiles, 1);
+    if (tile == 2) hipLaunchKernelGGL((conv2d_k3_bf16x3_kernel<NT, 2, EFFI_EPI_K1HEAD, false, false, true, 4>), grid, dim3(256), 0, st, a, tiles_x, ntiles);
+    else if (tile == 4) hipLaunchKernelGGL((conv2d_k3_bf16x3_kernel<NT, 4, EFFI_EPI_K1HEAD, false, false, true, 4>), grid, dim3(256), 0, st, a, tiles_x, ntiles);
+    else if (tile == 8) hipLaunchKernelGGL((conv2d_k3_bf16x3_kernel<NT, 2, EFFI_EPI_K1HEAD, false, false, true, 8>), grid, dim3(512), 0, st, a, tiles_x, ntiles);
+    else return EFFI_ERR_BADARG;
+    return hipPeekAtLastError() == hipSuccess ? EFFI_OK : EFFI_ERR_LAUNCH;
+}
+
 template <int EPI, bool SR = false>
 static int dispatch_bf16x3(const Conv2dArgs& a, int nt, hipStream_t st) {
     switch (nt) {
diff --git a/effi_mvs_plus_amd/csrc/proj.hip b/effi_mvs_plus_amd/csrc/proj.hip
--- a/effi_mvs_plus_amd/csrc/proj.hip
+++ b/effi_mvs_plus_amd/csrc/proj.hip
@@ -71,18 +71,27 @@
 }
 
 struct PairList { const float* p[4]; };
-__global__ void compose_rel_proj_stages_kernel(PairList pl, int n_views, float* __restrict__ rt_all) {
+__device__ __forceinline__ void compose_rel_proj_stage(const PairList& pl, int stage, int n_views, float* __restrict__ rt_all) {
     const int v = threadIdx.x;
     if (v >= n_views - 1) return;
     const float* pairs = pl.p[0];
 #pragma unroll
     for (int j = 1; j < 4; ++j)
-        if ((int)blockIdx.x == j) pairs = pl.p[j];
+        if (stage == j) pairs = pl.p[j];
     double R[4][4], Rinv[4][4], S[4][4];
     compose_k_rt(pairs, R);
     invert4x4(R, Rinv);
     compose_k_rt(pairs + (long)(v + 1) * 32, S);
-    write_rt(S, Rinv, rt_all + ((long)blockIdx.x * (n_views - 1) + v) * 12);
+    write_rt(S, Rinv, rt_all + ((long)stage * (n_views - 1) + v) * 12);
+}
+__global__ void compose_rel_proj_stages_kernel(PairList pl, int n_views, float* __restrict__ rt_all) {
+    compose_rel_proj_stage(pl, (int)blockIdx.x, n_views, rt_all);
+}
+
+__global__ void cascade_setup_kernel(const float* __restrict__ disp_range, int n_range, int D, float* __restrict__ depths,
+                                     float* __restrict__ intervals, PairList pl, int n_views, float* __restrict__ rt_all) {
+    if (blockIdx.x == 0) effi_stage1_hypotheses_block(disp_range, n_range, D, depths, intervals);
+    else compose_rel_proj_stage(pl, (int)blockIdx.x - 1, n_views, rt_all);
 }
 
 __global__ void rel_proj_kernel(const float* __restrict__ src, const float* __restrict__ ref, float* __restrict__ rt) {
@@ -116,6 +125,21 @@
     return EFFI_OK;
 }
 
+extern "C" int effi_cascade_setup_f32(const float* disp_range, int n_range, int D, float* depths, float* intervals,
+                                      const float* const* pairs, int n_stages, int n_views, float* rt_out, effi_stream_t stream) {
+    if (!disp_range || !depths || !intervals || n_range < 2 || D < 2) return EFFI_ERR_BADARG;
+    if (!pairs || !rt_out || n_stages < 1 || n_stages > 4 || n_views < 2 || n_views > EFFI_MAX_VIEWS + 1) return EFFI_ERR_BADARG;
+    PairList pl;
+    for (int k = 0; k < 4; ++k) {
+        pl.p[k] = pairs[k < n_stages ? k : 0];
+        if (!pl.p[k]) return EFFI_ERR_BADARG;
+    }
+    hipLaunchKernelGGL(cascade_setup_kernel, dim3(1 + n_stages), dim3(128), 0, effi_s(stream), disp_range, n_range, D, depths, intervals, pl,
+                       n_views, rt_out);
+    EFFI_LAUNCH_CHECK();
+    return EFFI_OK;
+}
+
 extern "C" int effi_rel_proj_f32(const float* src_proj, const float* ref_proj, float* rt_out, effi_stream_t stream) {
     if (!src_proj || !ref_proj || !rt_out) return EFFI_ERR_BADARG;
     hipLaunchKernelGGL(rel_proj_kernel, dim3(1), dim3(64), 0, effi_s(stream), src_proj, ref_proj, rt_out);
diff --git a/effi_mvs_plus_amd/csrc/volume_ops.hip b/effi_mvs_plus_amd/csrc/volume_ops.hip
--- a/effi_mvs_plus_amd/csrc/volume_ops.hip
+++ b/effi_mvs_plus_amd/csrc/volume_ops.hip
@@ -94,21 +94,7 @@
 
 __global__ void stage1_hypotheses_kernel(const float* __restrict__ disp_range, int n_range, int D,
                                          float* __restrict__ depths, float* __restrict__ intervals) {
-    const float lo = disp_range[0], hi = disp_range[n_range - 1];
-    const float step = (hi - lo) / (float)(D - 1);
-    for (int d = threadIdx.x; d < D; d += blockDim.x) {
-        const float s = lo + (float)d * step;
-        depths[d] = 1.0f / s;
-    }
-    if (threadIdx.x < 3) {
-        const float base = (hi - lo) / (float)n_range;
-        const float ratio = (threadIdx.x == 0) ? 4.0f : (threadIdx.x == 1 ? 2.0f : 1.0f);
-        intervals[threadIdx.x] = base * ratio;
-    } else if (threadIdx.x == 3) {
-        intervals[3] = 1.0f / hi;
-    } else if (threadIdx.x == 4) {
-        intervals[4] = 1.0f / lo;
-    }
+    effi_stage1_hypotheses_block(disp_range, n_range, D, depths, intervals);
 }
 
 __global__ void upsample_nearest_kernel(const float* __restrict__ in, int C, int h, int w, int f,
@@ -195,10 +181,24 @@
     }
 }
 
+__device__ __forceinline__ void conf_store_up(float* __restrict__ out_up, float conf, int p, int w, int f) {
+    const int y = p / w, x = p - y * w;
+    float* dst = out_up + ((long)y * f) * ((long)w * f) + (long)x * f;
+    if (f == 4) {
+        const float4 v = make_float4(conf, conf, conf, conf);
+#pragma unroll
+        for (int j = 0; j < 4; ++j) *reinterpret_cast<float4*>(dst + (long)j * w * 4) = v;
+        return;
+    }
+    for (int j = 0; j < f; ++j)
+        for (int i = 0; i < f; ++i) dst[(long)j * w * f + i] = conf;
+}
+
 __global__ void softmax_regress_conf_kernel(const float* __restrict__ logits, const float* __restrict__ depth,
                                             long dds, long dps, int D, int hw,
                                             float* __restrict__ out_depth, float* __restrict__ out_conf,
-                                            const float* __restrict__ disp_range, int n_range, float* __restrict__ out_dinv) {
+                                            const float* __restrict__ disp_range, int n_range, float* __restrict__ out_dinv,
+                                            float* __restrict__ out_conf_up, int w, int f) {
     const int p = blockIdx.x * blockDim.x + threadIdx.x;
     if (p >= hw) return;
     float m = -INFINITY;
@@ -219,15 +219,18 @@
         s4 = s4 + pr;
     }
     out_depth[p] = dep;
-    out_conf[p] = 4.0f * (s4 / 4.0f);
+    const float conf = 4.0f * (s4 / 4.0f);
+    out_conf[p] = conf;
     if (out_dinv) out_dinv[p] = effi_depth_to_inv(dep, disp_range[0], disp_range[n_range - 1]);
+    if (out_conf_up) conf_store_up(out_conf_up, conf, p, w, f);
 }
 
 template <int DT>
 __global__ __launch_bounds__(64) void softmax_regress_conf_reg_kernel(const float* __restrict__ logits, const float* __restrict__ depth,
                                                                       long dds, long dps, int hw, float* __restrict__ out_depth,
                                                                       float* __restrict__ out_conf, const float* __restrict__ disp_range,
-                                                                      int n_range, float* __restrict__ out_dinv) {
+                                                                      int n_range, float* __restrict__ out_dinv,
+                                                                      float* __restrict__ out_conf_up, int w, int f) {
     const int p = blockIdx.x * 64 + threadIdx.x;
     if (p >= hw) return;
     float e[DT], dv[DT];
@@ -260,8 +263,10 @@
         s4 = in ? s4 + e[d] : s4;
     }
     out_depth[p] = dep;
-    out_conf[p] = 4.0f * (s4 / 4.0f);
+    const float conf = 4.0f * (s4 / 4.0f);
+    out_conf[p] = conf;
     if (out_dinv) out_dinv[p] = effi_depth_to_inv(dep, disp_range[0], disp_range[n_range - 1]);
+    if (out_conf_up) conf_store_up(out_conf_up, conf, p, w, f);
 }
 
 __device__ __forceinline__ float lookup1d(const float* __restrict__ vol, long dstride, int Dp,
@@ -550,16 +555,18 @@
     return EFFI_OK;
 }
 
-extern "C" int effi_softmax_regress_conf_f32(const float* logits, const float* depth, long dds, long dps, int D,
-                                             int hw, float* out_depth, float* out_conf, const float* disp_range, int n_range,
-                                             float* out_depth_inv, effi_stream_t stream) {
+static int softmax_regress_conf_launch(const float* logits, const float* depth, long dds, long dps, int D, int hw, float* out_depth,
+                                       float* out_conf, const float* disp_range, int n_range, float* out_depth_inv,
+                                       float* out_conf_up, int w, int f, effi_stream_t stream) {
     if (!logits || !depth || !out_depth || !out_conf || D < 1 || hw < 1) return EFFI_ERR_BADARG;
     if (out_depth_inv && (!disp_range || n_range < 2)) return EFFI_ERR_BADARG;
+    if (out_conf_up && (w < 1 || f < 1 || hw % w != 0)) return EFFI_ERR_BADARG;
+    if (out_conf_up && f == 4 && (reinterpret_cast<uintptr_t>(out_conf_up) & 15)) return EFFI_ERR_BADARG;
     const dim3 grid(effi_cdiv(hw, 64));
     hipStream_t st = effi_s(stream);
 #define EFFI_SM(DT)                                                                                                      \
     hipLaunchKernelGGL(softmax_regress_conf_reg_kernel<DT>, grid, dim3(64), 0, st, logits, depth, dds, dps, hw, out_depth, \
-                       out_conf, disp_range, n_range, out_depth_inv)
+                       out_conf, disp_range, n_range, out_depth_inv, out_conf_up, w, f)
     switch (D) {
         case 8: EFFI_SM(8); break;
         case 16: EFFI_SM(16); break;
@@ -569,11 +576,26 @@
         case 96: EFFI_SM(96); break;
         default:
             hipLaunchKernelGGL(softmax_regress_conf_kernel, grid, dim3(64), 0, st, logits, depth, dds, dps, D, hw, out_depth, out_conf,
-                               disp_range, n_range, out_depth_inv);
+                               disp_range, n_range, out_depth_inv, out_conf_up, w, f);
     }
 #undef EFFI_SM
     EFFI_LAUNCH_CHECK();
     return EFFI_OK;
+}
+
+extern "C" int effi_softmax_regress_conf_f32(const float* logits, const float* depth, long dds, long dps, int D,
+                                             int hw, float* out_depth, float* out_conf, const float* disp_range, int n_range,
+                                             float* out_depth_inv, effi_stream_t stream) {
+    return softmax_regress_conf_launch(logits, depth, dds, dps, D, hw, out_depth, out_conf, disp_range, n_range, out_depth_inv, nullptr, 0,
+                                       0, stream);
+}
+
+extern "C" int effi_softmax_regress_conf_up_f32(const float* logits, const float* depth, long dds, long dps, int D, int h, int w,
+                                                float* out_depth, float* out_conf, const float* disp_range, int n_range,
+                                                float* out_depth_inv, float* out_conf_up, int f, effi_stream_t stream) {
+    if (h < 1 || w < 1 || !out_conf_up) return EFFI_ERR_BADARG;
+    return softmax_regress_conf_launch(logits, depth, dds, dps, D, h * w, out_depth, out_conf, disp_range, n_range, out_depth_inv,
+                                       out_conf_up, w, f, stream);
 }
 
 extern "C" int effi_vol_lookup1d_f32(const float* vol, long vds, long vps, int Dp, const float* query, long qds,
@@ -717,17 +739,8 @@
     int planes[4], h[4], w[4], hp[4], wp[4];
     int first[5];
 };
-__global__ __launch_bounds__(TPB) void sr_clear_border_kernel(SrMaps a) {
-    int k = 0;
-#pragma unroll
-    for (int j = 1; j < 4; ++j) k += ((int)blockIdx.x >= a.first[j]) ? 1 : 0;
-    unsigned short* base = a.base[0];
-    int planes = a.planes[0], h = a.h[0], w = a.w[0], hp = a.hp[0], wp = a.wp[0], b0 = a.first[0];
-#pragma unroll
-    for (int j = 1; j < 4; ++j)
-        if (k == j) { base = a.base[j]; planes = a.planes[j]; h = a.h[j]; w = a.w[j]; hp = a.hp[j]; wp = a.wp[j]; b0 = a.first[j]; }
+__device__ __forceinline__ void sr_clear_border_unit(unsigned short* __restrict__ base, int planes, int h, int w, int hp, int wp, long i) {
     const int rowpart = (hp - h) * wp, per_plane = rowpart + h * (wp - w);
-    const long i = (long)(blockIdx.x - b0) * TPB + threadIdx.x;
     if (i >= (long)planes * per_plane) return;
     const int pl = (int)(i / per_plane), r = (int)(i - (long)pl * per_plane);
     int y, x;
@@ -742,6 +755,17 @@
     }
     *reinterpret_cast<float4*>(base + (((long)pl * hp + y) * wp + x) * 8) = make_float4(0.0f, 0.0f, 0.0f, 0.0f);
 }
+__global__ __launch_bounds__(TPB) void sr_clear_border_kernel(SrMaps a) {
+    int k = 0;
+#pragma unroll
+    for (int j = 1; j < 4; ++j) k += ((int)blockIdx.x >= a.first[j]) ? 1 : 0;
+    unsigned short* base = a.base[0];
+    int planes = a.planes[0], h = a.h[0], w = a.w[0], hp = a.hp[0], wp = a.wp[0], b0 = a.first[0];
+#pragma unroll
+    for (int j = 1; j < 4; ++j)
+        if (k == j) { base = a.base[j]; planes = a.planes[j]; h = a.h[j]; w = a.w[j]; hp = a.hp[j]; wp = a.wp[j]; b0 = a.first[j]; }
+    sr_clear_border_unit(base, planes, h, w, hp, wp, (long)(blockIdx.x - b0) * TPB + threadIdx.x);
+}
 
 __global__ __launch_bounds__(TPB) void sr_from_planar_kernel(const float* __restrict__ in, int C, int h, int w, unsigned short* __restrict__ sr,
                                                              int hp, int wp) {
@@ -763,6 +787,8 @@
     unsigned short* hidden_sr[4];
     int hd[4], cd[4], h[4], w[4], hp[4], wp[4], q4[4];
     int first[5];
+    unsigned short* clear_base[4];
+    int clear_planes[4], nsplit[4];
 };
 __global__ __launch_bounds__(TPB) void split_tanh_relu_stages_sr_kernel(SplitStagesSr a) {
     int k = 0;
@@ -779,6 +805,17 @@
             ctx = a.ctx[j]; hidden = a.hidden[j]; inp = a.inp[j]; hsr = a.hidden_sr[j];
             hd = a.hd[j]; cd = a.cd[j]; h = a.h[j]; w = a.w[j]; hp = a.hp[j]; wp = a.wp[j]; b0 = a.first[j]; q4 = a.q4[j];
         }
+    {
+        unsigned short* cbase = a.clear_base[0];
+        int cplanes = a.clear_planes[0], nsplit = a.nsplit[0];
+#pragma unroll
+        for (int j = 1; j < 4; ++j)
+            if (k == j) { cbase = a.clear_base[j]; cplanes = a.clear_planes[j]; nsplit = a.nsplit[j]; }
+        if ((int)blockIdx.x - b0 >= nsplit) {
+            sr_clear_border_unit(cbase, cplanes, h, w, hp, wp, (long)(blockIdx.x - b0 - nsplit) * TPB + threadIdx.x);
+            return;
+        }
+    }
     const long hw = (long)h * w, n_h = (long)(hd >> 3) * hw, n_i = (long)(cd >> 2) * hw;
     const long i = (long)(blockIdx.x - b0) * TPB + threadIdx.x;
     if (i < n_h) {
@@ -842,9 +879,10 @@
     return EFFI_OK;
 }
 
-extern "C" int effi_split_tanh_relu_stages_sr_f32(const float* const* ctx, const int* hd, const int* cd, const int* h, const int* w,
-                                                  float* const* hidden, void* const* hidden_sr, const int* hp, const int* wp,
-                                                  float* const* inp, const int* hidden_q4, int n_stages, effi_stream_t stream) {
+static int split_tanh_relu_stages_sr_launch(const float* const* ctx, const int* hd, const int* cd, const int* h, const int* w,
+                                            float* const* hidden, void* const* hidden_sr, const int* hp, const int* wp,
+                                            float* const* inp, const int* hidden_q4, void* const* clear_base, const int* clear_planes,
+                                            int n_stages, effi_stream_t stream) {
     if (!ctx || !hd || !cd || !h || !w || !hidden || !hidden_sr || !hp || !wp || !inp || n_stages < 1 || n_stages > 4) return EFFI_ERR_BADARG;
     SplitStagesSr a;
     int blocks = 0;
@@ -858,12 +896,32 @@
         a.q4[k] = hidden_q4 ? hidden_q4[j] : 0;
         if (a.q4[k] && (reinterpret_cast<uintptr_t>(hidden[j]) & 15)) return EFFI_ERR_BADARG;
         a.first[k] = blocks;
-        if (k < n_stages) blocks += effi_cdiv((long)h[j] * w[j] * ((hd[j] >> 3) + (cd[j] >> 2)), TPB);
+        a.nsplit[k] = effi_cdiv((long)h[j] * w[j] * ((hd[j] >> 3) + (cd[j] >> 2)), TPB);
+        a.clear_base[k] = clear_base ? reinterpret_cast<unsigned short*>(clear_base[j]) : nullptr;
+        a.clear_planes[k] = clear_base ? clear_planes[j] : 0;
+        if (clear_base && (!clear_base[j] || clear_planes[j] < 1 || (reinterpret_cast<uintptr_t>(clear_base[j]) & 15))) return EFFI_ERR_BADARG;
+        if (k < n_stages)
+            blocks += a.nsplit[k] + effi_cdiv((long)a.clear_planes[k] * ((long)(hp[j] - h[j]) * wp[j] + (long)h[j] * (wp[j] - w[j])), TPB);
     }
     a.first[4] = blocks;
     hipLaunchKernelGGL(split_tanh_relu_stages_sr_kernel, dim3(blocks), dim3(TPB), 0, effi_s(stream), a);
     EFFI_LAUNCH_CHECK();
     return EFFI_OK;
+}
+
+extern "C" int effi_split_tanh_relu_stages_sr_f32(const float* const* ctx, const int* hd, const int* cd, const int* h, const int* w,
+                                                  float* const* hidden, void* const* hidden_sr, const int* hp, const int* wp,
+                                                  float* const* inp, const int* hidden_q4, int n_stages, effi_stream_t stream) {
+    return split_tanh_relu_stages_sr_launch(ctx, hd, cd, h, w, hidden, hidden_sr, hp, wp, inp, hidden_q4, nullptr, nullptr, n_stages, stream);
+}
+
+extern "C" int effi_split_tanh_relu_stages_sr_clear_f32(const float* const* ctx, const int* hd, const int* cd, const int* h, const int* w,
+                                                        float* const* hidden, void* const* hidden_sr, const int* hp, const int* wp,
+                                                        float* const* inp, const int* hidden_q4, void* const* clear_base,
+                                                        const int* clear_planes, int n_stages, effi_stream_t stream) {
+    if (!clear_base || !clear_planes) return EFFI_ERR_BADARG;
+    return split_tanh_relu_stages_sr_launch(ctx, hd, cd, h, w, hidden, hidden_sr, hp, wp, inp, hidden_q4, clear_base, clear_planes, n_stages,
+                                            stream);
 }
 
 namespace {
diff --git a/effi_mvs_plus_amd/models/Effi_MVS_plus.py b/effi_mvs_plus_amd/models/Effi_MVS_plus.py
--- a/effi_mvs_plus_amd/models/Effi_MVS_plus.py
+++ b/effi_mvs_plus_amd/models/Effi_MVS_plus.py
@@ -274,18 +274,20 @@
     def _hot_single(self, feats, ctx, pairs, disp_range, want_intermediates=False):
         D1 = self.depth_stage_nums[0]
         ops.mark("begin")
-        hyp, misc = ops.stage1_hypotheses(disp_range, D1)
+        keys = ["stage{}".format(s + 1) for s in range(self.num_stage)]
+        if self.num_stage <= 4 and ops.option("setup_fused"):
+            (hyp, misc), rts = ops.cascade_setup(disp_range, D1, [pairs[k].contiguous() for k in keys])
+        else:
+            hyp, misc = ops.stage1_hypotheses(disp_range, D1)
+            if self.num_stage <= 4:
+                rts = ops.compose_rel_proj_stages([pairs[k].contiguous() for k in keys])
+            else:
+                rts = [ops.compose_rel_proj(pairs[k]) for k in keys]
         g_min, g_max = misc[3:4], misc[4:5]
         preds, inter = [], {}
         conf = None
         weights = reg_vol = cur_vol = None
         lo_prev, hi_prev = g_min, g_max
-
-        keys = ["stage{}".format(s + 1) for s in range(self.num_stage)]
-        if self.num_stage <= 4:
-            rts = ops.compose_rel_proj_stages([pairs[k].contiguous() for k in keys])
-        else:
-            rts = [ops.compose_rel_proj(pairs[k]) for k in keys]
 
         table = feats if isinstance(feats, ops.ViewTable) else None
 
@@ -309,11 +311,14 @@
                 nm = BasicUpdateBlock.N_SR_MAPS
                 sr_maps = [ops.sr_alloc(nm, self.hdim_stage[s], cs[s].shape[1], cs[s].shape[2], cs[s].device, clear=False)
                            for s in range(self.num_stage)]
-                ops.sr_clear_border(sr_maps)
+                clear_fused = bool(ops.option("clear_fused"))
+                if not clear_fused:
+                    ops.sr_clear_border(sr_maps)
                 state_q4 = [self.update_block[s].state_q4_ok(not want_intermediates) and ops.uses_sr(cs[s].shape[1] * cs[s].shape[2])
                             for s in range(self.num_stage)]
                 return dict(enumerate(ops.split_tanh_relu_stages_sr(cs, self.hdim_stage[:self.num_stage], self.cdim_stage[:self.num_stage],
-                                                                    [m[-1] for m in sr_maps], q4=state_q4)))
+                                                                    [m[-1] for m in sr_maps], q4=state_q4,
+                                                                    clear=sr_maps if clear_fused else None)))
             if self.num_stage <= 4:
                 return dict(enumerate(ops.split_tanh_relu_stages(cs, self.hdim_stage[:self.num_stage], self.cdim_stage[:self.num_stage])))
             return {s: ops.split_tanh_relu(cs[s], self.hdim_stage[s], self.cdim_stage[s]) for s in range(self.num_stage)}
@@ -338,9 +343,12 @@
                 weights = self.PixelwiseNet.run(entropy)
                 cur_vol = ops.view_aggregate(sim_views, weights)
                 reg_vol = self.cost_regularization.run(cur_vol.unsqueeze(0))[0][0]
-                depth, c, inv_next = ops.softmax_regress_conf(reg_vol, hyp, disp_range)
-                with ops.Branch() as tail_branch:
-                    conf = ops.upsample_nearest(c.unsqueeze(0), 4)[0]
+                if ops.option("conf_fused"):
+                    depth, c, inv_next, conf = ops.softmax_regress_conf(reg_vol, hyp, disp_range, conf_up=4)
+                else:
+                    depth, c, inv_next = ops.softmax_regress_conf(reg_vol, hyp, disp_range)
+                    with ops.Branch() as tail_branch:
+                        conf = ops.upsample_nearest(c.unsqueeze(0), 4)[0]
                 preds.append(depth)
                 lo_cur, hi_cur = g_min, g_max
             else:
diff --git a/effi_mvs_plus_amd/models/update.py b/effi_mvs_plus_amd/models/update.py
--- a/effi_mvs_plus_amd/models/update.py
+++ b/effi_mvs_plus_amd/models/update.py
@@ -243,6 +243,15 @@
         return (bool(ops.option("state_q4")) and fuse_upsample and self.UpMask and not ops.option("gru_fused")
                 and self._sr_structure_ok(self.depth_head.conv1.in_channels))
 
+    def head_fused_tile(self, hd, h, w):
+        mode = ops.option("head_fused")
+        if not mode or hd not in (16, 32, 48):
+            return 0
+        forced = ops.option("head_fused_tile")
+        if forced:
+            return forced
+        return 8 if -(-h // 14) * -(-w // 14) < 256 else 4
+
     def run_fused_sr(self, net, lookup, inv_depth, context, seq_len, disp_range, fuse_upsample=False, maps=None, net_sr_ready=False,
                      net_owned=False, net_q4=False):
         hd = net.shape[0]
@@ -276,6 +285,7 @@
         wh2, bh2 = dh._c2t.get([dh.conv2.weight], lambda: packing.pack_head_taps(dh.conv2.weight, hd))
         inv_list, mask_list, depth_list = [], [], []
         gen_pair = ops.option("enc_gen") != 0 and getattr(lookup, "encoder_pair_sr", None) is not None
+        head_tile = self.head_fused_tile(hd, h, w)
         H_first = Hm
         h_pp = [None, net if net_owned else None]
         for i in range(seq_len):
@@ -302,8 +312,11 @@
             if want_mask and not fused_up:
                 with ops.Branch() as br:
                     mask = self.run_mask(net)
-            part = ops.conv2d_k3_k1_sr([Hm], wh1.wx, bh1, hd, None, wh2, bh2, 9, relu=False, relu1=True, out=head_buf)
-            inv_depth, depth = ops.head_update(part, dh.conv2.bias, inv_depth, disp_range)
+            if head_tile:
+                inv_depth, depth = ops.depth_head_sr([Hm], wh1.wx, bh1, hd, wh2, bh2, dh.conv2.bias, inv_depth, disp_range, head_tile)
+            else:
+                part = ops.conv2d_k3_k1_sr([Hm], wh1.wx, bh1, hd, None, wh2, bh2, 9, relu=False, relu1=True, out=head_buf)
+                inv_depth, depth = ops.head_update(part, dh.conv2.bias, inv_depth, disp_range)
             if fused_up:
                 wm, bm = _pack(self._m0, self.mask[0])
                 c1 = self.mask[0].out_channels
diff --git a/effi_mvs_plus_amd/ops.py b/effi_mvs_plus_amd/ops.py
--- a/effi_mvs_plus_amd/ops.py
+++ b/effi_mvs_plus_amd/ops.py
@@ -77,7 +77,8 @@
 
 
 _PY_OPTION_DEFAULTS = {"warp_x3": 0, "state_q4": 1, "c1k7_mfma": 1, "k5s2_split": 1, "roll": 1, "conv3d_unaligned_split": 1, "conv3d_s2_split": 1, "fpn_conv0_fused": 1,
-                       "fpn_split_head": 1, "csp_pair": 1, "head_taps": 1, "enc_tail": 0, "enc_gen": 1, "reduce_chunk": 2048, "gru_fused": 0, "csp_gen": 0}
+                       "fpn_split_head": 1, "csp_pair": 1, "head_taps": 1, "enc_tail": 0, "enc_gen": 1, "reduce_chunk": 2048, "gru_fused": 0, "csp_gen": 0,
+                       "head_fused": 1, "head_fused_tile": 0, "clear_fused": 1, "setup_fused": 1, "conf_fused": 1}
 _PY_OPTS = {k: int(os.environ.get("EFFI_" + k.upper(), v)) for k, v in _PY_OPTION_DEFAULTS.items()}
 LIB_OPTIONS = ("warp_lds_kb", "dyn_form", "dyn_setup_exact", "dyn_xchg", "pixnet_mfma", "force_mr", "mr4_min", "mr4_nt2_max", "mr2_min",
                "wide_tiles", "roll_mr", "roll_zt", "roll_rp", "deconv_mr", "sr_waves", "enc_gen_mr3", "c3_lean", "dyn_win")
@@ -308,6 +309,22 @@
     check(_lib.lib().effi_compose_rel_proj_stages_f32(_ptr_array(pairs_list), len(pairs_list), n, _p(rt), _stream()),
           "effi_compose_rel_proj_stages_f32")
     return [rt[k] for k in range(len(pairs_list))]
+
+
+def cascade_setup(disp_range, D, pairs_list):
+    _t(disp_range, "disp_range")
+    for p_ in pairs_list:
+        _t(p_, "pairs")
+    n = pairs_list[0].shape[0]
+    if len(pairs_list) > 4 or any(p_.shape[0] != n for p_ in pairs_list):
+        raise ValueError("cascade_setup: up to 4 stages with the same number of views")
+    dev = disp_range.device
+    depths = torch.empty(D, device=dev, dtype=torch.float32)
+    intervals = torch.empty(5, device=dev, dtype=torch.float32)
+    rt = torch.empty(len(pairs_list), n - 1, 12, device=dev, dtype=torch.float32)
+    check(_lib.lib().effi_cascade_setup_f32(_p(disp_range), disp_range.numel(), D, _p(depths), _p(intervals), _ptr_array(pairs_list),
+                                            len(pairs_list), n, _p(rt), _stream()), "effi_cascade_setup_f32")
+    return (depths, intervals), [rt[k] for k in range(len(pairs_list))]
 
 
 def rel_proj(src_proj: torch.Tensor, ref_proj: torch.Tensor) -> torch.Tensor:
@@ -763,7 +780,7 @@
     return out
 
 
-def softmax_regress_conf(logits, depth, disp_range=None):
+def softmax_regress_conf(logits, depth, disp_range=None, conf_up=0):
     D, h, w = logits.shape
     _t(logits, "logits"), _t(depth, "depth", contiguous=False)
     depth, dds, dps = _depth_strides(depth, D, h, w)
@@ -773,6 +790,11 @@
     if disp_range is not None:
         _t(disp_range, "disp_range")
         oi, n_range = torch.empty(h, w, device=logits.device, dtype=torch.float32), disp_range.numel()
+    if conf_up:
+        ou = torch.empty(h * conf_up, w * conf_up, device=logits.device, dtype=torch.float32)
+        check(_lib.lib().effi_softmax_regress_conf_up_f32(_p(logits), _p(depth), dds, dps, D, h, w, _p(od), _p(oc), _p(disp_range), n_range,
+                                                           _p(oi), _p(ou), conf_up, _stream()), "effi_softmax_regress_conf_up_f32")
+        return (od, oc, ou) if disp_range is None else (od, oc, oi, ou)
     check(_lib.lib().effi_softmax_regress_conf_f32(_p(logits), _p(depth), dds, dps, D, h * w, _p(od), _p(oc), _p(disp_range), n_range,
                                                     _p(oi), _stream()), "effi_softmax_regress_conf_f32")
     return (od, oc) if disp_range is None else (od, oc, oi)
@@ -1119,15 +1141,20 @@
     return m
 
 
-def sr_clear_border(groups):
-    if not 1 <= len(groups) <= 4:
-        raise ValueError("sr_clear_border: 1..4 groups")
+def _sr_groups(groups, name):
     firsts = [_sr(g[0], "SR map") for g in groups]
     planes = [2 * (g[0].channels // 8) * len(g) for g in groups]
     for g in groups:
         step = g[0].t.numel() * 2
         if any(m.t.data_ptr() != g[0].t.data_ptr() + i * step for i, m in enumerate(g)):
-            raise ValueError("sr_clear_border: a group must be consecutive maps of one sr_alloc block")
+            raise ValueError(f"{name}: a group must be consecutive maps of one sr_alloc block")
+    return firsts, planes
+
+
+def sr_clear_border(groups):
+    if not 1 <= len(groups) <= 4:
+        raise ValueError("sr_clear_border: 1..4 groups")
+    firsts, planes = _sr_groups(groups, "sr_clear_border")
     check(_lib.lib().effi_sr_clear_border(_ptr_array([m.t for m in firsts]), _int_array(planes), _int_array([m.h for m in firsts]),
                                            _int_array([m.w for m in firsts]), _int_array([m.hp for m in firsts]),
                                            _int_array([m.wp for m in firsts]), len(groups), _stream()), "effi_sr_clear_border")
@@ -1142,7 +1169,7 @@
     return out
 
 
-def split_tanh_relu_stages_sr(ctxs, hds, cds, hidden_srs, q4=None):
+def split_tanh_relu_stages_sr(ctxs, hds, cds, hidden_srs, q4=None, clear=None):
     outs = []
     for c_, hd, cd, m in zip(ctxs, hds, cds, hidden_srs):
         _t(c_, "context"), _sr(m, "hidden SR map")
@@ -1153,6 +1180,17 @@
                      torch.empty(cd, h, w, device=c_.device, dtype=torch.float32)))
     if len(ctxs) > 4:
         raise ValueError("split_tanh_relu_stages_sr: up to 4 stages")
+    if clear is not None:
+        if len(clear) != len(ctxs) or any((g[0].h, g[0].w, g[0].hp, g[0].wp) != (m.h, m.w, m.hp, m.wp) for g, m in zip(clear, hidden_srs)):
+            raise ValueError("split_tanh_relu_stages_sr: one group of maps of the stage's geometry per stage")
+        firsts, planes = _sr_groups(clear, "split_tanh_relu_stages_sr")
+        check(_lib.lib().effi_split_tanh_relu_stages_sr_clear_f32(
+            _ptr_array(ctxs), _int_array(list(hds)), _int_array(list(cds)), _int_array([c_.shape[1] for c_ in ctxs]),
+            _int_array([c_.shape[2] for c_ in ctxs]), _ptr_array([o[0] for o in outs]), _ptr_array([m.t for m in hidden_srs]),
+            _int_array([m.hp for m in hidden_srs]), _int_array([m.wp for m in hidden_srs]), _ptr_array([o[1] for o in outs]),
+            _int_array([int(bool(v)) for v in (q4 if q4 is not None else [0] * len(ctxs))]), _ptr_array([m.t for m in firsts]),
+            _int_array(planes), len(ctxs), _stream()), "effi_split_tanh_relu_stages_sr_clear_f32")
+        return outs
     check(_lib.lib().effi_split_tanh_relu_stages_sr_f32(
         _ptr_array(ctxs), _int_array(list(hds)), _int_array(list(cds)), _int_array([c_.shape[1] for c_ in ctxs]),
         _int_array([c_.shape[2] for c_ in ctxs]), _ptr_array([o[0] for o in outs]), _ptr_array([m.t for m in hidden_srs]),
@@ -1302,6 +1340,23 @@
                 _p(w2pack), _p(bias2), cout2, int(relu), h, w, g.hp, g.wp, _p(None if out_sr is not None else out),
                 _p(out_sr.t if out_sr is not None else None), _stream()), "effi_conv2d_k3_k1_bf16x3_sr")
     return out_sr if out_sr is not None else out
+
+
+def depth_head_sr(srcs, wpack, bias, cout1, w2pack, bias2_taps, bias2, inv_depth, disp_range, tile):
+    g = _sr_srcs(srcs)
+    _t(inv_depth, "inv_depth"), _t(disp_range, "disp_range"), _t(bias2, "bias")
+    h, w = g.h, g.w
+    if inv_depth.numel() != h * w:
+        raise ValueError("depth_head_sr: inv_depth must hold h*w values")
+    out_inv = torch.empty(1, h, w, device=g.t.device, dtype=torch.float32)
+    out_depth = torch.empty(1, h, w, device=g.t.device, dtype=torch.float32)
+    cin = sum(m.channels for m in srcs)
+    work = lambda: {"flops": 2.0 * h * w * (cin * cout1 * 9 + cout1 * 9), "bytes": 4.0 * h * w * (cin + 3)}
+    check(_call(f"depth_head_nt{(cout1 + 15) // 16}", work, _x3("effi_depth_head_bf16x3_sr"), _ptr_array([m.t for m in srcs]),
+                _int_array([m.channels for m in srcs]), len(srcs), _p(wpack), _p(bias), cout1, _p(w2pack), _p(bias2_taps), _p(bias2),
+                _p(inv_depth), _p(disp_range), disp_range.numel(), h, w, g.hp, g.wp, int(tile), _p(out_inv), _p(out_depth), _stream()),
+          "effi_depth_head_bf16x3_sr")
+    return out_inv, out_depth
 
 
 def conv2d_k3_k1_up2x_sr(srcs, wpack, bias, cout1, w2pack, bias2, inv_depth, disp_range, want_depth_inv=True):
diff --git a/include/effi_mvs_hip.h b/include/effi_mvs_hip.h
--- a/include/effi_mvs_hip.h
+++ b/include/effi_mvs_hip.h
@@ -44,6 +44,8 @@
 int effi_compose_rel_proj_stages_f32(const float* const* pairs, int n_stages, int n_views, float* rt_out,
                                      effi_stream_t stream);
 int effi_rel_proj_f32(const float* src_proj, const float* ref_proj, float* rt_out, effi_stream_t stream);
+int effi_cascade_setup_f32(const float* disp_range, int n_range, int D, float* depths, float* intervals,
+                           const float* const* pairs, int n_stages, int n_views, float* rt_out, effi_stream_t stream);
 
 int effi_planar_to_nhwc_f32(const float* const* srcs, float* const* dsts, int n, int C, int HW,
                             effi_stream_t stream);
@@ -120,6 +122,9 @@
 int effi_softmax_regress_conf_f32(const float* logits, const float* depth, long depth_dstride,
                                   long depth_pstride, int D, int hw, float* out_depth, float* out_conf,
                                   const float* disp_range, int n_range, float* out_depth_inv, effi_stream_t stream);
+int effi_softmax_regress_conf_up_f32(const float* logits, const float* depth, long depth_dstride, long depth_pstride, int D, int h,
+                                     int w, float* out_depth, float* out_conf, const float* disp_range, int n_range,
+                                     float* out_depth_inv, float* out_conf_up, int f, effi_stream_t stream);
 
 int effi_vol_lookup1d_f32(const float* vol, long vol_dstride, long vol_pstride, int Dp,
                           const float* query, long q_dstride, long q_ystride, long q_xstride, int nq,
@@ -361,6 +366,10 @@
 int effi_split_tanh_relu_stages_sr_f32(const float* const* ctx, const int* hd, const int* cd, const int* h, const int* w,
                                        float* const* hidden, void* const* hidden_sr, const int* hp, const int* wp, float* const* inp,
                                        const int* hidden_q4, int n_stages, effi_stream_t stream);
+int effi_split_tanh_relu_stages_sr_clear_f32(const float* const* ctx, const int* hd, const int* cd, const int* h, const int* w,
+                                             float* const* hidden, void* const* hidden_sr, const int* hp, const int* wp,
+                                             float* const* inp, const int* hidden_q4, void* const* clear_base, const int* clear_planes,
+                                             int n_stages, effi_stream_t stream);
 int effi_encoder_inputs_bf16x3_sr(const float* inv_depth, const float* disp_range, int n_range, const float* interval,
                                   const float* cur_vol, long cds, long cps, int Dcur, const float* reg_vol, long rds, long rps,
                                   int Dreg, const float* dmin, const float* dmax, long range_ps, int nq, int h, int w,
@@ -382,6 +391,10 @@
 int effi_conv2d_k3_k1_bf16x3_sr(const void* const* srcs, const int* src_channels, int n_src, const void* wpack_bf16, const float* bias,
                                 int cout1, int relu1, const float* extra, int c_extra, const void* w2pack_bf16, const float* bias2,
                                 int cout2, int relu, int h, int w, int hp, int wp, float* out, void* out_sr, effi_stream_t stream);
+int effi_depth_head_bf16x3_sr(const void* const* srcs, const int* src_channels, int n_src, const void* wpack_bf16, const float* bias,
+                              int cout1, const void* w2pack_bf16, const float* bias2_taps, const float* bias2, const float* inv_depth,
+                              const float* disp_range, int n_range, int h, int w, int hp, int wp, int tile, float* out_inv,
+                              float* out_depth, effi_stream_t stream);
 int effi_conv2d_k3_k1_up2x_bf16x3_sr(const void* const* srcs, const int* src_channels, int n_src, const void* wpack_bf16,
                                      const float* bias, int cout1, const void* w2pack_bf16, const float* bias2, const float* inv_depth,
                                      const float* disp_range, int n_range, int h, int w, int hp, int wp, float* out_depth,
@@ -404,6 +417,10 @@
                                           const float* bias, int cout1, const void* w2pack_bf16, const float* bias2,
                                           const float* inv_depth, const float* disp_range, int n_range, int h, int w, int hp, int wp,
                                           float* out_depth, float* out_depth_inv, effi_stream_t stream);
+int effi_depth_head_bf16x3_sr_bf16(const void* const* srcs, const int* src_channels, int n_src, const void* wpack_bf16,
+                                   const float* bias, int cout1, const void* w2pack_bf16, const float* bias2_taps, const float* bias2,
+                                   const float* inv_depth, const float* disp_range, int n_range, int h, int w, int hp, int wp, int tile,
+                                   float* out_inv, float* out_depth, effi_stream_t stream);
 int effi_gru_zr_q_fused_bf16x3_sr_bf16(const void* H_in, const void* X, const float* h_in, const void* wzr_pack, const float* bias_zr,
                                        const void* wq_pack, const float* bias_q, int hd, int h, int w, int hp, int wp, float* h_out,
                                        void* H_out, effi_stream_t stream);
```

New measurement: 639.6 views/s (median of 6 runs). 1.01x the previous value.
